# yahoo/bftkv

Measured on AMD Instinct MI355X. Metric: pgp_rsa2048_signature_verifies_per_sec, higher is better.
Workload: dtype u32; 1 GPU; 64-replica quorum, 10000 RSA-2048 signed writes per GPU (cfg2 of BASELINE.json), 534164 signature packets per GPU, 1.0% corrupt / 0.5% unknown issuer / 0.5% duplicate / 1.0% one-short; parallelism=shard-by-write x1, RCCL all-gather of verdict bitmaps on the verifier's stream, replicas=64, writes_per_gpu=10000, sigs_per_gpu=534164, batches_in_flight=3

## Files before the change

### bftkv_amd/csrc/capi.hip

```cpp
#include "../../include/bftkv_gpu.h"

#include <hip/hip_runtime.h>
#include <stdio.h>
#include <stdlib.h>
#include <string.h>

#include <limits.h>
#include <linux/futex.h>
#include <sched.h>
#include <sys/syscall.h>
#include <unistd.h>

#include <algorithm>
#include <array>
#include <atomic>
#include <memory>
#include <functional>
#include <map>
#include <set>
#include <chrono>
#include <condition_variable>
#include <mutex>
#include <shared_mutex>
#include <system_error>
#include <thread>
#include <string>
#include <unordered_map>
#include <vector>

#include "host_bignum.h"
#include "host_sha256.h"
#include "kernels.hip"
#include "threshold_kernels.hip"
#include "ec_kernels.hip"
#include "dsa_verify_kernels.hip"

using namespace bftkv;

namespace {

inline void copy_out(void* dst, const void* src, size_t n) { if (n) memcpy(dst, src, n); }

struct DevBuf {
  void* p = nullptr;
  size_t cap = 0;
  hipError_t ensure(size_t bytes) {
    if (bytes <= cap) return hipSuccess;
    if (p) { hipError_t e = hipFree(p); if (e != hipSuccess) return e; p = nullptr; cap = 0; }
    size_t want = bytes + bytes / 4 + 256;
    hipError_t e = hipMalloc(&p, want);
    if (e == hipSuccess) cap = want;
    return e;
  }
  hipError_t ensure_exact(size_t bytes) {
    if (bytes <= cap) return hipSuccess;
    if (p) { hipError_t e = hipFree(p); if (e != hipSuccess) return e; p = nullptr; cap = 0; }
    hipError_t e = hipMalloc(&p, bytes);
    if (e == hipSuccess) cap = bytes;
    return e;
  }
  void release() { if (p) (void)hipFree(p); p = nullptr; cap = 0; }
  template <typename T> T* as() const { return (T*)p; }
};

struct KeyEntry {
  uint64_t key_id = 0, entity_id = 0;
  uint8_t algo = 0, flags = 0;
  uint32_t bits = 0, e = 0, n0 = 0, qbits = 0;
  std::vector<uint32_t> nl, r2, r2w, qw, dtab, qpow, qconst;
  std::string material;
  bool cert_only = false;
  int cert_group = -1;
  uint32_t entity_index = 0;
  std::string cert_digest;
  uint64_t last_used = 0;
  bool dsa_unslotted = false;
};

struct QuorumHost {
  bool live = false;
  int n_qcs = 0;
  int32_t f[MAX_QC], mn[MAX_QC], thr[MAX_QC], suff[MAX_QC];
  std::vector<std::vector<uint64_t>> nodes;
  DevBuf member;
  uint64_t keyring_gen = ~0ull;
  DevBuf ids;
  uint32_t ids_off[MAX_QC + 1];
};

struct EcKeySet {
  bool live = false;
  int curve_id = -1;
  uint32_t bits = 0, n_keys = 0, n_refused = 0;
  uint32_t w = 0, nwin = 0;
  size_t key_words = 0;
  std::vector<uint8_t> curve;
  DevBuf tab;
  DevBuf refused;
  DevBuf mod[4];
  void release() { tab.release(); refused.release(); for (DevBuf& b : mod) b.release(); }
};

}

using ctx_lock = std::lock_guard<std::recursive_mutex>;

struct bftkv_gpu_ctx {
  int device = 0;
  hipStream_t stream = nullptr;
  hipStream_t stream_h = nullptr;
  hipStream_t stream_d = nullptr;
  std::recursive_mutex mu;
  std::string err;

  uint64_t keyring_gen = 0;
  uint32_t n_keys = 0, n_entities = 0;
  bool have_dsa_keys = false, have_rsa3072 = false, have_rsa4096 = false, have_ambiguous = false;
  std::vector<uint64_t> h_key_id, h_entity_id;
  std::vector<uint32_t> h_key_entity;
  std::vector<uint8_t> h_key_flags;
  std::vector<KeyEntry> ring, certs;
  uint32_t n_ring_entities = 0;
  std::map<std::string, bool> cert_valid;
  DevBuf k_r2w;
  DevBuf k_id, k_entity, k_algo, k_flags, k_bits, k_e, k_n, k_r2, k_n0, k_q, k_qbits, k_dsatab, k_dsaslot, k_sorted_id, k_sorted_slot;
  DevBuf dsa_comb;
  uint32_t dsa_wbits = 8, dsa_wbits_pinned = 0;
  std::map<std::string, uint32_t> dsa_comb_slot;
  std::set<std::string> dsa_cert_materials;
  uint64_t ring_epoch = 0, dsa_ring_epoch_seen = ~0ull;
  uint32_t dsa_wbits_want = 0;
  uint32_t dsa_entry_limbs = DSA_N_SMALL;
  size_t dsa_budget_bytes = 0;
  bool have_dsa3072 = false, have_dsa2048 = false;
  DevBuf dsa_idx;
  uint64_t cert_clock = 0;
  struct CertFast { uint64_t issuer_id; int group; uint64_t epoch; };
  std::shared_mutex cert_fast_mu;
  std::unordered_map<std::string, CertFast> cert_fast;
  size_t cert_fast_bytes = 0;
  uint64_t cert_epoch = 0, kt_cert_epoch = 0;
  std::vector<uint32_t> kt_group_ent;
  KeyTableDev kt{};

  std::vector<QuorumHost> quorums;
  std::vector<EcKeySet> ec_keysets;

  DevBuf txt_mid32, txt_mid64, txt_tail, txt_len;
  DevBuf forced_iss;
  DevBuf counts, base, total, item_flags, walk_scratch, cert_ent, sig_class, mid, mid64, hash_mask, recs, digests, r, xr, pk_list, pk_list3072, pk_list4096, r3072, r4096, pk_count, dsa_list, dsa_u, ids_tmp;
  DevBuf o_err, o_nver, o_verdict, o_fenced;
  DevBuf in_tbs, in_tbs_off, in_ss, in_ss_off;
  hipEvent_t seg_ev = nullptr;
  DevBuf in_prefix, in_prefix_off, in_shared, in_shared_off, in_seg;
  DevBuf st_tmp, item_tmp, bits_tmp, plan_cut;
  DevBuf chunk_arena, chunk_ctr;
  uint32_t multiexp_parts = 0;
  uint32_t ec_split = 0;
  uint32_t ec_window = 0;
  DevBuf ec_fb_tab[4];
  uint32_t ec_fb_w[4] = {};
  uint32_t multiexp_block = 0;
  uint32_t multiexp_lanes = 0;
  uint32_t dsa_inv_mode = 0;
  uint32_t n_cus = 256;
  uint32_t lagrange_x_bound = 0;
  bool early_exit = true;
  std::vector<DevBuf*> scratch_pool;
  std::unordered_map<std::string, std::vector<uint32_t>> modrow_cache;
  std::map<std::string, std::array<DevBuf, 4>> modtab_cache;
  uint32_t* h_mail = nullptr;
  uint32_t* d_mail = nullptr;
  uint32_t last_total = 0, last_rsa = 0, last_items = 0;
  bool last_total_on_dev = false;
  hipEvent_t ev[10] = {};
  hipEvent_t ev_turn = nullptr;
  bool have_timing = false;
  void* rccl_comm = nullptr;
  int n_ranks = 1, rank = 0;

  bftkv_gpu_ctx* root = nullptr;
  std::shared_mutex kt_rw;
  std::atomic<int> kt_writers{0};
  std::atomic<int> n_forks{0};
  uint64_t quorum_gen = 0;
  uint64_t seen_keyring_gen = ~0ull, seen_quorum_gen = ~0ull;
  size_t n_dsa_slots = 0;
  int kt_read_depth = 0;
  DevBuf in_pack;
  uint8_t* h_out = nullptr; uint8_t* d_out = nullptr; size_t out_cap = 0;
  uint32_t out_seq = 0;
  std::vector<bftkv_gpu_ctx*> hb_workers;
  hipStream_t stream_c = nullptr;
  hipStream_t stream_c2 = nullptr;
  std::vector<hipEvent_t> hb_ev;
  uint8_t* hb_out = nullptr; size_t hb_out_cap = 0;
  uint32_t modexp_lds_pad = 0;
  uint32_t hb_pieces = 0;
  hipEvent_t hb_ev0 = nullptr;
  bool hb_tight = false;
  uint32_t hb_copy_mode = 0;
  void* hb_ring = nullptr;
  std::vector<float> hb_trace;
  uint32_t hb_last_pieces = 0;
  std::vector<uint32_t> hb_item0;
  void* small_pin = nullptr;
  uint32_t staged_spin_us = 50000;
};

void rccl_release(bftkv_gpu_ctx* c);
void release_small_pin(bftkv_gpu_ctx* c);
extern "C" int signature_verify_entities(bftkv_gpu_ctx* c, uint32_t n_items, const uint8_t* tbs, const uint64_t* tbs_off, const uint8_t* sig,
                                         const uint64_t* sig_off, const uint32_t* ent, uint8_t* err_out, const uint8_t* sig_class = nullptr,
                                         uint8_t* fenced_out = nullptr, const uint64_t* forced_issuer = nullptr);

namespace {

int fork_refresh(bftkv_gpu_ctx* c);

struct KtWrite {
  bftkv_gpu_ctx* c;
  explicit KtWrite(bftkv_gpu_ctx* c_) : c(c_) { c->kt_writers.fetch_add(1); c->kt_rw.lock(); }
  ~KtWrite() { c->kt_rw.unlock(); c->kt_writers.fetch_sub(1); }
};
struct KtRead {
  bftkv_gpu_ctx *c, *r;
  int rc = 0;
  explicit KtRead(bftkv_gpu_ctx* c_) : c(c_), r(c_->root) {
    if (!r || c->kt_read_depth++ > 0) return;
    while (r->kt_writers.load(std::memory_order_acquire) > 0) std::this_thread::yield();
    r->kt_rw.lock_shared();
    rc = fork_refresh(c);
  }
  ~KtRead() { if (r && --c->kt_read_depth == 0) r->kt_rw.unlock_shared(); }
};

struct Turnstile { std::mutex mu; hipEvent_t last = nullptr; const void* owner = nullptr; };
Turnstile g_turnstile[16];
constexpr uint64_t HB_PIPE_MIN_BYTES = 24ull << 20;
constexpr uint32_t HB_PIPE_MAX_PIECES = 8;
std::mutex g_hb_mu[16];
constexpr size_t HB_TR = 10;
struct HbRing {
  static constexpr size_t SLOT = 16u << 20;
  static constexpr int NSLOT = 6;
  static constexpr int THREADS = 4;
  uint8_t* base = nullptr;
  hipEvent_t ev[NSLOT] = {};
  bool used[NSLOT] = {};
  ~HbRing() { if (base) (void)hipHostFree(base); for (auto e : ev) if (e) (void)hipEventDestroy(e); }
  hipError_t init() {
    if (base) return hipSuccess;
    hipError_t e = hipHostMalloc((void**)&base, SLOT * NSLOT, hipHostMallocDefault);
    if (e != hipSuccess) { base = nullptr; return e; }
    for (auto& x : ev) if ((e = hipEventCreateWithFlags(&x, hipEventDisableTiming)) != hipSuccess) return e;
    return hipSuccess;
  }
};


constexpr uint32_t TURNSTILE_MIN_PACKETS = 98304;

std::mutex g_live_mu;
std::vector<bftkv_gpu_ctx*> g_live;
bool ctx_is_live(bftkv_gpu_ctx* c) {
  std::lock_guard<std::mutex> lk(g_live_mu);
  for (auto* p : g_live) if (p == c) return true;
  return false;
}

int fail(bftkv_gpu_ctx* c, int rc, const char* what, hipError_t e = hipSuccess) {
  char buf[512];
  if (e != hipSuccess) snprintf(buf, sizeof buf, "%s: %s", what, hipGetErrorString(e));
  else snprintf(buf, sizeof buf, "%s", what);
  c->err = buf;
  return rc;
}
// ... 96 lines not shown
                 const std::function<int(hipStream_t)>* upload_tbs = nullptr, const QuorumDev* plan_q = nullptr, uint64_t ss_len = 0,
                 const uint32_t* d_mid_in = nullptr, const uint64_t* d_tbs_prefix = nullptr, uint32_t staged_cap = 0,
                 hipEvent_t ev_input = nullptr, bool mid_prelaunched = false, const uint64_t* d_forced_issuer = nullptr) {
  const bool one_stream = staged_cap != 0 && !ev_input;
  hipStream_t s = c->stream, sh = one_stream ? c->stream : c->stream_h;
  auto rec = [&](int k, hipStream_t st) -> hipError_t { return one_stream ? hipSuccess : hipEventRecord(c->ev[k], st); };
  auto join = [&](hipStream_t st, int k) -> hipError_t { return one_stream ? hipSuccess : hipStreamWaitEvent(st, c->ev[k], 0); };
  if (!c->ev[0]) for (auto& e : c->ev) HIPCHK(c, hipEventCreate(&e));
  HIPCHK(c, c->counts.ensure(sizeof(uint32_t) * (n_items + 1)));
  HIPCHK(c, c->base.ensure(sizeof(uint32_t) * (n_items + 1)));
  HIPCHK(c, c->total.ensure(16));
  HIPCHK(c, c->item_flags.ensure(n_items + 16));
  const uint32_t walk_cap = ss_len ? (uint32_t)std::min<uint64_t>(WALK_CAP_MAX, std::max<uint64_t>(WALK_CAP_MIN, ss_len / n_items / 48)) : 96u;
  HIPCHK(c, c->walk_scratch.ensure(sizeof(WalkEnt) * walk_cap * (size_t)n_items + 16));
  HIPCHK(c, c->mid.ensure(sizeof(uint32_t) * 8 * N_MID32 * (size_t)n_items + 16));
  HIPCHK(c, c->mid64.ensure(sizeof(uint64_t) * 8 * 2 * (size_t)n_items + 16));
  HIPCHK(c, c->hash_mask.ensure(sizeof(uint32_t) * (size_t)n_items + 16));
  constexpr size_t CHUNK_ARENA_MIN = 64u << 10;
  if (!c->chunk_ctr.p) { HIPCHK(c, c->chunk_ctr.ensure(16)); HIPCHK(c, hipMemsetAsync(c->chunk_ctr.p, 0, 16, c->stream)); }
  HIPCHK(c, c->chunk_arena.ensure(CHUNK_ARENA_MIN + (staged_cap ? 2 * (size_t)ss_len : 0)));
  HIPCHK(c, c->pk_count.ensure(96));
  if (plan_q) HIPCHK(c, c->plan_cut.ensure(sizeof(uint32_t) * (size_t)n_items + 16));
  TextDev txt{nullptr, nullptr, nullptr, nullptr};
  if (!d_mid_in) {
    HIPCHK(c, c->txt_mid32.ensure(sizeof(uint32_t) * 8 * N_MID32 * (size_t)n_items + 16));
    HIPCHK(c, c->txt_mid64.ensure(sizeof(uint64_t) * 8 * N_MID64 * (size_t)n_items + 16));
    HIPCHK(c, c->txt_tail.ensure((size_t)128 * N_HASHES * n_items + 16));
    HIPCHK(c, c->txt_len.ensure(sizeof(uint64_t) * N_HASHES * (size_t)n_items + 16));
    txt = TextDev{c->txt_mid32.as<uint32_t>(), c->txt_mid64.as<uint64_t>(), c->txt_tail.as<uint8_t>(), c->txt_len.as<uint64_t>()};
  }
  if (ev_input) HIPCHK(c, hipStreamWaitEvent(s, ev_input, 0));
  HIPCHK(c, rec(0, s));
  HIPCHK(c, join(sh, 0));
  HIPCHK(c, rec(5, sh));
  if (!upload_tbs && !d_mid_in)
    hipLaunchKernelGGL(k_sha256_mid, dim3((n_items + 63) / 64), dim3(64), 0, sh, d_tbs, d_tbs_off, n_items, c->mid.as<uint32_t>());
  hipLaunchKernelGGL(k_walk<false>, dim3(n_items), dim3(64), 0, s, d_ss, d_ss_off, n_items, c->counts.as<uint32_t>(),
                     (const uint32_t*)nullptr, (SigRec*)nullptr, c->item_flags.as<uint8_t>(), c->walk_scratch.as<WalkEnt>(), walk_cap,
                     c->chunk_ctr.as<uint32_t>());
  constexpr uint32_t MAIL_EMPTY = 0xFFFFFFFFu;
  if (c->h_mail && !staged_cap) __atomic_store_n(&c->h_mail[0], MAIL_EMPTY, __ATOMIC_RELEASE);
  hipLaunchKernelGGL(k_scan_counts, dim3(1), dim3(1024), 0, s, c->counts.as<uint32_t>(), n_items, c->base.as<uint32_t>(),
                     c->total.as<uint32_t>(), staged_cap ? (uint32_t*)nullptr : c->d_mail, c->pk_count.as<uint32_t>(), c->hash_mask.as<uint32_t>(),
                     staged_cap, c->chunk_ctr.as<uint32_t>());
  uint32_t total = staged_cap ? staged_cap : MAIL_EMPTY;
  const uint32_t* const n_recs_dev = staged_cap ? c->total.as<uint32_t>() : nullptr;
  if (c->h_mail && !staged_cap) {
    const auto t_spin = std::chrono::steady_clock::now();
    for (uint32_t it = 0;; ++it) {
      total = __atomic_load_n(&c->h_mail[0], __ATOMIC_ACQUIRE);
      if (total != MAIL_EMPTY) break;
      if ((it & 1023u) == 1023u && std::chrono::steady_clock::now() - t_spin > std::chrono::milliseconds(20)) break;
      __builtin_ia32_pause();
    }
  }
  uint32_t chunk_units = (c->h_mail && !staged_cap && total != MAIL_EMPTY) ? c->h_mail[2] : 0u;
  if (total == MAIL_EMPTY) {
    HIPCHK(c, hipMemcpyAsync(&total, c->total.p, sizeof(uint32_t), hipMemcpyDeviceToHost, s));
    HIPCHK(c, hipMemcpyAsync(&chunk_units, c->chunk_ctr.as<uint32_t>() + 2, sizeof(uint32_t), hipMemcpyDeviceToHost, s));
    HIPCHK(c, hipStreamSynchronize(s));
  }
  if (!staged_cap && (size_t)chunk_units * 16 > c->chunk_arena.cap) HIPCHK(c, c->chunk_arena.ensure((size_t)chunk_units * 16));
  c->last_total = staged_cap ? 0u : total;
  c->last_total_on_dev = staged_cap != 0 && ev_input != nullptr;
  c->last_items = n_items;
  c->hb_last_pieces = 0;
  const size_t tr = total ? total : 1;
  HIPCHK(c, c->recs.ensure(sizeof(SigRec) * tr));
  HIPCHK(c, c->digests.ensure(sizeof(uint32_t) * 16 * tr));
  HIPCHK(c, c->r.ensure(sizeof(uint32_t) * EM_LOW_LIMBS * tr));
  HIPCHK(c, c->xr.ensure(sizeof(uint32_t) * (c->have_rsa4096 ? MONT_NMAX : c->have_rsa3072 ? MONT_TPI_BIG * MONT_L3072 : 80) * tr));
  HIPCHK(c, c->pk_list.ensure(sizeof(uint32_t) * tr));
  HIPCHK(c, c->pk_list3072.ensure(c->have_rsa3072 ? sizeof(uint32_t) * tr : 16));
  HIPCHK(c, c->pk_list4096.ensure(c->have_rsa4096 ? sizeof(uint32_t) * tr : 16));
  if (c->have_rsa3072) HIPCHK(c, c->r3072.ensure(sizeof(uint32_t) * EM_LOW_LIMBS * tr));
  if (c->have_rsa4096) HIPCHK(c, c->r4096.ensure(sizeof(uint32_t) * EM_LOW_LIMBS * tr));
  HIPCHK(c, c->dsa_list.ensure(sizeof(uint32_t) * tr));
  if (c->have_dsa_keys) HIPCHK(c, c->dsa_u.ensure(sizeof(uint32_t) * DSA_U_WORDS * tr));
  if (c->have_dsa3072 && c->have_dsa2048) HIPCHK(c, c->dsa_idx.ensure(sizeof(uint32_t) * 4 * (size_t)tr + 16));
  hipLaunchKernelGGL(k_walk<true>, dim3(n_items), dim3(64), 0, s, d_ss, d_ss_off, n_items, c->counts.as<uint32_t>(),
                     c->base.as<uint32_t>(), c->recs.as<SigRec>(), c->item_flags.as<uint8_t>(), (WalkEnt*)nullptr, walk_cap, (uint32_t*)nullptr);
  if (total) {
    ParseArgs pa;
    pa.sig_blob = d_ss; pa.sig_off = d_ss_off; pa.rec_base = c->base.as<uint32_t>(); pa.counts = c->counts.as<uint32_t>(); pa.n_items = n_items;
    pa.scratch = c->walk_scratch.as<WalkEnt>(); pa.walk_cap = walk_cap; pa.recs = c->recs.as<SigRec>(); pa.n_recs = total; pa.cert_ent = d_cert_ent;
    pa.pk_list = c->pk_list.as<uint32_t>(); pa.pk_list3072 = c->pk_list3072.as<uint32_t>(); pa.pk_list4096 = c->pk_list4096.as<uint32_t>();
    pa.pk_count = c->pk_count.as<uint32_t>(); pa.dsa_list = c->dsa_list.as<uint32_t>(); pa.item_hash_mask = c->hash_mask.as<uint32_t>();
    pa.sig_class = d_sig_class; pa.forced_issuer = d_forced_issuer; pa.msg_slot = d_msg_slot; pa.msg_hash = d_msg_hash; pa.item_flags = c->item_flags.as<uint8_t>();
    pa.defer_queue = plan_q ? 1u : 0u;
    pa.n_recs_dev = n_recs_dev;
    pa.chunk_arena = c->chunk_arena.as<uint8_t>(); pa.chunk_cap_units = (uint32_t)std::min<size_t>(c->chunk_arena.cap / 16, 0xFFFFFFF0u);
    pa.chunk_bump = c->chunk_ctr.as<uint32_t>() + 1;
    if (!staged_cap && (uint64_t)total >= 128ull * n_items)
      hipLaunchKernelGGL(k_parse_body_items, dim3(n_items), dim3(PARSE_ITEM_BLOCK), 0, s, pa, c->kt);
    else
      hipLaunchKernelGGL(k_parse_body, dim3((total + 255) / 256), dim3(256), 0, s, pa, c->kt);
  }
  uint32_t* const cnt_p = c->pk_count.as<uint32_t>();
  const uint32_t* const start0 = cnt_p + 12;
  PlanArgs pl{};
  if (total && plan_q) {
    pl.recs = c->recs.as<SigRec>(); pl.rec_base = c->base.as<uint32_t>(); pl.counts = c->counts.as<uint32_t>(); pl.n_items = n_items;
    pl.pk_list = c->pk_list.as<uint32_t>(); pl.dsa_list = c->dsa_list.as<uint32_t>(); pl.pk_list3072 = c->pk_list3072.as<uint32_t>();
    pl.pk_list4096 = c->pk_list4096.as<uint32_t>(); pl.pk_count = cnt_p; pl.plan_cut = c->plan_cut.as<uint32_t>(); pl.verdict = nullptr;
    int min_suff = 0;
    for (int i = 0; i < plan_q->n_qcs; ++i) if (plan_q->suff[i] > 0 && (min_suff == 0 || plan_q->suff[i] < min_suff)) min_suff = plan_q->suff[i];
    pl.margin = 1u + (uint32_t)min_suff / 64u;
    pl.mail = c->d_mail ? c->d_mail + 3 : nullptr;
    if (c->h_mail) __atomic_store_n(&c->h_mail[3], 0u, __ATOMIC_RELEASE);
    hipLaunchKernelGGL(k_plan<1>, dim3((n_items + PLAN_ITEMS - 1) / PLAN_ITEMS), dim3(PLAN_BLOCK), 0, s, pl, c->kt, *plan_q);
  }
  const bool dsa_side = total && c->have_dsa_keys;
  if (one_stream && dsa_side) HIPCHK(c, hipEventRecord(c->ev[1], s)); else HIPCHK(c, rec(1, s));
  const size_t n_slots = c->root ? c->n_dsa_slots : c->dsa_comb_slot.size();
  const uint32_t inv_batch_min = c->dsa_inv_mode == 1 || n_slots > (c->dsa_inv_mode == 2 ? (size_t)INV_MAX_SLOTS : 256) ? 0xFFFFFFFFu
                                 : c->dsa_inv_mode == 2 ? 0u : (uint32_t)std::max<size_t>(4096, 64 * n_slots);
  auto launch_dsa_inv = [&](hipStream_t st, const uint32_t* start) {
    if (inv_batch_min != 0xFFFFFFFFu)
      hipLaunchKernelGGL(k_dsa_inv_batched, dim3((total + INV_TILE - 1) / INV_TILE), dim3(INV_BLOCK), 0, st, d_ss, c->recs.as<SigRec>(),
                         c->dsa_list.as<uint32_t>(), c->pk_count.as<uint32_t>(), start, c->kt, c->dsa_u.as<uint32_t>(), inv_batch_min);
    if (inv_batch_min != 0u)
      hipLaunchKernelGGL(k_dsa_inv, dim3((total + 63) / 64), dim3(64), 0, st, d_ss, c->recs.as<SigRec>(), c->dsa_list.as<uint32_t>(),
                         c->pk_count.as<uint32_t>(), start, c->kt, c->dsa_u.as<uint32_t>(), inv_batch_min);
  };
  if (total && c->have_dsa_keys) {
    HIPCHK(c, hipStreamWaitEvent(c->stream_d, c->ev[1], 0));
    launch_dsa_inv(c->stream_d, start0);
    HIPCHK(c, hipEventRecord(c->ev[7], c->stream_d));
  }
  auto hash_stream_work = [&]() -> int {
    HIPCHK(c, join(sh, 1));
    if (total) {
      if (!d_mid_in) {
        hipLaunchKernelGGL(k_hash_mid_other, dim3((n_items + 63) / 64, N_HASHES - 1), dim3(64), 0, sh, d_tbs, d_tbs_off, n_items,
                           c->hash_mask.as<uint32_t>(), c->mid.as<uint32_t>(), c->mid64.as<uint64_t>());
        hipLaunchKernelGGL(k_hash_mid_text, dim3((n_items + 63) / 64, N_HASHES), dim3(64), 0, sh, d_tbs, d_tbs_off, n_items, c->hash_mask.as<uint32_t>(), txt);
      }
      hipLaunchKernelGGL(k_digest_sha256, dim3((total + 255) / 256), dim3(256), 0, sh, d_tbs, d_tbs_off, d_ss,
                         d_mid_in ? d_mid_in : c->mid.as<uint32_t>(), c->mid64.as<uint64_t>(), n_items, c->recs.as<SigRec>(), total,
                         c->digests.as<uint32_t>(), d_tbs_prefix, n_recs_dev);
    }
    HIPCHK(c, rec(6, sh));
    return 0;
  };
  if (!upload_tbs) { int hrc = hash_stream_work(); if (hrc) return hrc; }
  const dim3 qg((total + MODEXP_BLOCK / MONT_TPI - 1) / (MODEXP_BLOCK / MONT_TPI));
  const dim3 qg8((total + MODEXP_BLOCK / MONT_TPI_BIG - 1) / (MODEXP_BLOCK / MONT_TPI_BIG));
  static const bool wide8_off = getenv("BFTKV_NO_WIDE8") != nullptr;
  const bool wide8 = staged_cap != 0 && ss_len / 256 <= 8192 && !wide8_off;
  auto launch_modexp = [&](const uint32_t* start) {
    if (wide8)
      hipLaunchKernelGGL((k_rsa_modexp<10, MONT_TPI_BIG>), qg8, dim3(MODEXP_BLOCK), 0, s, d_ss, c->recs.as<SigRec>(), c->pk_list.as<uint32_t>(),
                         cnt_p, start, c->kt, c->r.as<uint32_t>(), c->xr.as<uint32_t>(), (uint64_t*)(cnt_p + 16));
    else
    hipLaunchKernelGGL((k_rsa_modexp<MONT_L, MONT_TPI>), qg, dim3(MODEXP_BLOCK), c->modexp_lds_pad, s, d_ss, c->recs.as<SigRec>(), c->pk_list.as<uint32_t>(),
                       cnt_p, start, c->kt, c->r.as<uint32_t>(), c->xr.as<uint32_t>(), (uint64_t*)(cnt_p + 16));
    if (c->have_rsa3072)
      hipLaunchKernelGGL((k_rsa_modexp<MONT_L3072, MONT_TPI_BIG>), qg8, dim3(MODEXP_BLOCK), 0, s, d_ss, c->recs.as<SigRec>(), c->pk_list3072.as<uint32_t>(),
                         cnt_p + 2, start + 2, c->kt, c->r3072.as<uint32_t>(), c->xr.as<uint32_t>(), (uint64_t*)nullptr);
    if (c->have_rsa4096)
      hipLaunchKernelGGL((k_rsa_modexp<MONT_L4096, MONT_TPI_BIG>), qg8, dim3(MODEXP_BLOCK), 0, s, d_ss, c->recs.as<SigRec>(), c->pk_list4096.as<uint32_t>(),
                         cnt_p + 3, start + 3, c->kt, c->r4096.as<uint32_t>(), c->xr.as<uint32_t>(), (uint64_t*)nullptr);
  };
  static const bool turnstile_off = getenv("BFTKV_NO_TURNSTILE") != nullptr;
  const bool big = staged_cap ? (ev_input != nullptr && ss_len / 320 >= TURNSTILE_MIN_PACKETS) : total >= TURNSTILE_MIN_PACKETS;
  if (big && !turnstile_off) {
    Turnstile& g = g_turnstile[(unsigned)c->device & 15u];
    std::lock_guard<std::mutex> tl(g.mu);
    if (g.last && g.owner != c) HIPCHK(c, hipStreamWaitEvent(s, g.last, 0));
    HIPCHK(c, rec(9, s));
    launch_modexp(start0);
    if (!c->ev_turn) HIPCHK(c, hipEventCreateWithFlags(&c->ev_turn, hipEventDisableTiming));
    HIPCHK(c, hipEventRecord(c->ev_turn, s));
    g.last = c->ev_turn; g.owner = c;
  } else {
    HIPCHK(c, rec(9, s));
    if (total) launch_modexp(start0);
  }
  HIPCHK(c, rec(2, s));
  if (upload_tbs) {
    int hrc = (*upload_tbs)(sh);
    if (hrc) return hrc;
    if (!mid_prelaunched)
      hipLaunchKernelGGL(k_sha256_mid, dim3((n_items + 63) / 64), dim3(64), 0, sh, d_tbs, d_tbs_off, n_items, c->mid.as<uint32_t>());
    if ((hrc = hash_stream_work())) return hrc;
  }
  HIPCHK(c, join(s, 6));
  bool other_hashes = true;
  if (total && !d_mid_in && plan_q && big && c->h_mail) {
    const auto t_spin = std::chrono::steady_clock::now();
    for (uint32_t it = 0;; ++it) {
      const uint32_t v = __atomic_load_n(&c->h_mail[3], __ATOMIC_ACQUIRE);
      if (v) { other_hashes = (v & 1u) != 0; break; }
      if ((it & 255u) == 255u && std::chrono::steady_clock::now() - t_spin > std::chrono::microseconds(300) + std::chrono::nanoseconds((uint64_t)total / 2)) break;
      __builtin_ia32_pause();
    }
  }
  if (total && !d_mid_in && other_hashes)
    hipLaunchKernelGGL(k_digest_other, dim3(std::min<uint32_t>((total + 255) / 256, DIGEST_OTHER_MAX_BLOCKS)), dim3(256), 0, s,
                       d_tbs, d_tbs_off, d_ss, c->mid.as<uint32_t>(), c->mid64.as<uint64_t>(), n_items, c->recs.as<SigRec>(), total,
                       c->digests.as<uint32_t>(), c->pk_count.as<uint32_t>() + 4, txt, n_recs_dev);
  const dim3 cg(((uint64_t)total * CMP_LANES + 255) / 256);
  auto launch_compare = [&](const uint32_t* start) {
    hipLaunchKernelGGL(k_rsa_compare, cg, dim3(256), 0, s, c->recs.as<SigRec>(), c->pk_list.as<uint32_t>(),
                       cnt_p, start, c->kt, c->r.as<uint32_t>(), c->digests.as<uint32_t>());
    if (c->have_rsa3072)
      hipLaunchKernelGGL(k_rsa_compare, cg, dim3(256), 0, s, c->recs.as<SigRec>(), c->pk_list3072.as<uint32_t>(),
                         cnt_p + 2, start + 2, c->kt, c->r3072.as<uint32_t>(), c->digests.as<uint32_t>());
    if (c->have_rsa4096)
      hipLaunchKernelGGL(k_rsa_compare, cg, dim3(256), 0, s, c->recs.as<SigRec>(), c->pk_list4096.as<uint32_t>(),
                         cnt_p + 3, start + 3, c->kt, c->r4096.as<uint32_t>(), c->digests.as<uint32_t>());
  };
  auto launch_dsa = [&](const uint32_t* start) {
    hipLaunchKernelGGL(k_dsa_mul, dim3((total + 63) / 64), dim3(64), 0, s, c->recs.as<SigRec>(), c->dsa_list.as<uint32_t>(),
                       cnt_p, start, c->kt, c->digests.as<uint32_t>(), c->dsa_u.as<uint32_t>());
    const uint32_t* idx_s = nullptr; const uint32_t* idx_b = nullptr; const uint32_t* cnt_cls = nullptr;
    if (c->have_dsa3072 && c->have_dsa2048) {
      uint32_t* cc = cnt_p + (start == start0 ? 20 : 22);
      uint32_t* is = c->dsa_idx.as<uint32_t>() + (start == start0 ? 0 : 2 * (size_t)total);
      hipLaunchKernelGGL(k_dsa_split, dim3((total + 255) / 256), dim3(256), 0, s, c->recs.as<SigRec>(), c->dsa_list.as<uint32_t>(), cnt_p, start, c->kt,
                         is, is + total, cc);
      idx_s = is; idx_b = is + total; cnt_cls = cc;
    }
    if (c->have_dsa2048)
      hipLaunchKernelGGL((k_dsa_modexp<MONT_L, MONT_TPI>), dim3((total + QUADS_PER_BLOCK - 1) / QUADS_PER_BLOCK), dim3(RSA_BLOCK), 0, s,
                         c->recs.as<SigRec>(), c->dsa_list.as<uint32_t>(), cnt_p, start, c->kt, c->dsa_u.as<uint32_t>(), idx_s, cnt_cls);
    if (c->have_dsa3072)
      hipLaunchKernelGGL((k_dsa_modexp<MONT_L3072, MONT_TPI_BIG>), dim3((total + RSA_BLOCK / MONT_TPI_BIG - 1) / (RSA_BLOCK / MONT_TPI_BIG)), dim3(RSA_BLOCK), 0, s,
                         c->recs.as<SigRec>(), c->dsa_list.as<uint32_t>(), cnt_p, start, c->kt, c->dsa_u.as<uint32_t>(), idx_b, cnt_cls ? cnt_cls + 1 : nullptr);
  };
  if (total) launch_compare(start0);
  HIPCHK(c, rec(8, s));
  if (total && c->have_dsa_keys) {
    HIPCHK(c, hipStreamWaitEvent(s, c->ev[7], 0));
    launch_dsa(start0);
  }
  if (total && plan_q) {
    HIPCHK(c, c->o_nver.ensure(sizeof(uint32_t) * n_items));
    HIPCHK(c, c->o_verdict.ensure(n_items));
    hipLaunchKernelGGL(k_tally, dim3((n_items + 3) / 4), dim3(256), 0, s, c->recs.as<SigRec>(), c->base.as<uint32_t>(), c->counts.as<uint32_t>(),
                       n_items, c->kt, *plan_q, c->o_verdict.as<uint8_t>(), c->o_nver.as<uint32_t>(), (uint32_t*)nullptr);
    hipLaunchKernelGGL(k_plan_snapshot, dim3(1), dim3(64), 0, s, cnt_p);
    pl.verdict = c->o_verdict.as<uint8_t>();
    hipLaunchKernelGGL(k_plan<2>, dim3((n_items + PLAN_ITEMS - 1) / PLAN_ITEMS), dim3(PLAN_BLOCK), 0, s, pl, c->kt, *plan_q);
    const uint32_t* const start1 = cnt_p + 8;
    if (c->have_dsa_keys) launch_dsa_inv(s, start1);
    launch_modexp(start1);
    launch_compare(start1);
    if (c->have_dsa_keys) launch_dsa(start1);
  }
  if (total && c->have_ambiguous && !d_msg_slot)
    hipLaunchKernelGGL(k_candidates, dim3((total + 63) / 64), dim3(64), 0, s, d_tbs, d_tbs_off, d_ss, d_mid_in ? d_mid_in : c->mid.as<uint32_t>(),
                       c->mid64.as<uint64_t>(), n_items, c->recs.as<SigRec>(), total, n_recs_dev, d_tbs_prefix, c->kt, d_cert_ent, d_sig_class, txt,
                       c->hash_mask.as<uint32_t>());
  HIPCHK(c, rec(3, s));
  HIPCHK(c, hipGetLastError());
  return 0;
}

int make_key_entry(bftkv_gpu_ctx* c, const bftkv_gpu_pubkey& k, bool cert_only, KeyEntry* out) {
  KeyEntry& e = *out;
  e.key_id = k.key_id; e.entity_id = k.entity_id; e.algo = k.pk_algo; e.cert_only = cert_only;
  e.material.clear();
  e.material.push_back((char)k.pk_algo);
  e.material.push_back((char)k.usable_sign);
  auto app = [&](const uint8_t* p, uint32_t l) {
    uint32_t z = 0;
    while (z < l && p[z] == 0) ++z;
    if (l > z) e.material.append((const char*)p + z, l - z);
    e.material.push_back('|');
  };
  app(k.n, k.n_len); app(k.e, k.e_len); app(k.g, k.g_len); app(k.y, k.y_len);
  e.flags = 0;
  if (k.usable_sign) e.flags |= KEYF_USABLE_SIGN;
  if (k.pk_algo != PK_RSA_ENCRYPT_ONLY && k.pk_algo != PK_ELGAMAL) e.flags |= KEYF_CAN_SIGN;
  if (k.key_id == k.entity_id) e.flags |= KEYF_PRIMARY;
  if (cert_only) e.flags |= KEYF_CERT_ONLY;
  e.bits = (uint32_t)hostbn::bit_length(k.n, k.n_len);
  e.e = 0; e.n0 = 0; e.qbits = 0;
  e.r2w.clear();
  e.nl.assign(MONT_NMAX, 0); e.r2.assign(MONT_NMAX, 0); e.qw.assign(8, 0); e.dtab.assign(2 * DSA_N_BIG, 0); e.qpow.clear(); e.qconst.clear();
  if (k.pk_algo == PK_RSA || k.pk_algo == PK_RSA_SIGN_ONLY) {
    if (hostbn::bit_length(k.e, k.e_len) > 32) return fail(c, BFTKV_E_UNSUPPORTED, "RSA public exponent wider than 32 bits");
    for (uint32_t j = 0; j < k.e_len; ++j) e.e = (e.e << 8) | k.e[j];
    const int nlimbs = e.bits <= 2048 ? MONT_N : (e.bits <= 3072 ? MONT_TPI_BIG * MONT_L3072 : MONT_TPI_BIG * MONT_L4096);
    if (e.bits > 4096) e.bits = 0xFFFFFFFFu;
    else if (!hostbn::mont_setup(k.n, k.n_len, nlimbs, e.nl.data(), e.r2.data(), &e.n0)) e.bits = 0xFFFFFFFFu;
    else if (e.bits <= 2048) {
      std::vector<uint32_t> nl80(80);
      uint32_t n0b = 0;
      e.r2w.assign(80, 0);
      (void)hostbn::mont_setup(k.n, k.n_len, 80, nl80.data(), e.r2w.data(), &n0b);
    }
  } else if (k.pk_algo == PK_DSA) {
    e.qbits = (uint32_t)hostbn::bit_length(k.e, k.e_len);
    const int NLp = e.bits <= 2048 ? (int)DSA_N_SMALL : (int)DSA_N_BIG;
    const uint32_t cap_bits = e.bits <= 2048 ? 2048u : 3072u;
    const int nwords = (28 * NLp + 31) / 32 + 1;
    std::vector<uint32_t> p(nwords), g(nwords), y(nwords), q(nwords);
    hostbn::from_be(k.e, k.e_len, q.data(), nwords);
    bool ok = e.bits >= 2 && e.bits <= 3072 && e.qbits >= 32 && e.qbits <= 256 && (q[0] & 1u) &&
              hostbn::mont_setup(k.n, k.n_len, NLp, e.nl.data(), e.r2.data(), &e.n0);
    if (ok && (hostbn::bit_length(k.g, k.g_len) > cap_bits || hostbn::bit_length(k.y, k.y_len) > cap_bits)) ok = false;
    if (ok) {
      hostbn::from_be(k.n, k.n_len, p.data(), nwords);
      hostbn::from_be(k.g, k.g_len, g.data(), nwords);
      hostbn::from_be(k.y, k.y_len, y.data(), nwords);
      hostbn::reduce(g.data(), p.data(), nwords);
      hostbn::reduce(y.data(), p.data(), nwords);
      hostbn::to_mont_limbs(g.data(), p.data(), nwords, NLp, &e.dtab[0]);
      hostbn::to_mont_limbs(y.data(), p.data(), nwords, NLp, &e.dtab[DSA_N_BIG]);
      for (int j = 0; j < 8; ++j) e.qw[j] = q[j];
      e.qpow.assign((size_t)NLp * 10, 0);
      uint32_t x[9] = {1, 0, 0, 0, 0, 0, 0, 0, 0}, q9[9];
      for (int j = 0; j < 9; ++j) q9[j] = j < 8 ? q[j] : 0;
      for (int j = 0; j < NLp; ++j) {
        hostbn::to_limbs28(x, 9, &e.qpow[(size_t)j * 10], 10);
        for (int b = 0; b < MONT_W; ++b) hostbn::dbl_mod(x, q9, 9);
      }
      e.qconst.assign(12, 0);
      uint32_t r2q[9] = {1, 0, 0, 0, 0, 0, 0, 0, 0};
      for (int b = 0; b < 512; ++b) hostbn::dbl_mod(r2q, q9, 9);
      for (int j = 0; j < 8; ++j) e.qconst[j] = r2q[j];
      uint32_t inv = 1;
      for (int it = 0; it < 5; ++it) inv *= 2u - q[0] * inv;
      e.qconst[8] = 0u - inv;
    } else {
      e.bits = 0xFFFFFFFFu;
    }
  }
  return 0;
}

int sync_dsa_tables(bftkv_gpu_ctx* c, const std::vector<const KeyEntry*>& rows, const std::vector<uint8_t>& algo,
                    std::vector<uint32_t>& bits, bool* bits_changed) {
  std::vector<uint32_t> slot(rows.size() ? rows.size() : 1, 0xFFFFFFFFu);
  *bits_changed = false;
  auto stride_bytes = [&](uint32_t w, uint32_t E) -> size_t { return (size_t)dsa_slot_stride(w, E) * sizeof(uint32_t); };
  size_t ring_dsa = 0;
  bool ring_big = false;
  for (size_t i = 0; i < rows.size(); ++i)
    if (algo[i] == PK_DSA && bits[i] != 0xFFFFFFFFu && !rows[i]->cert_only) { ++ring_dsa; ring_big = ring_big || bits[i] > 2048; }
  auto assign = [&](std::vector<uint32_t>& new_slots, std::vector<uint32_t>& new_rows) {
    new_slots.clear(); new_rows.clear();
    size_t cert_cap = c->dsa_wbits > 8 ? 8 : 1024;
    if (c->dsa_budget_bytes) {
      const size_t per = stride_bytes(c->dsa_wbits, c->dsa_entry_limbs), ring_need = per * ring_dsa;
      cert_cap = std::min(cert_cap, c->dsa_budget_bytes > ring_need ? (c->dsa_budget_bytes - ring_need) / per : 0);
    }
    for (size_t i = 0; i < rows.size(); ++i) {
      if (algo[i] != PK_DSA || bits[i] == 0xFFFFFFFFu) continue;
      if (bits[i] > 2048 && c->dsa_entry_limbs != DSA_N_BIG) {
        bits[i] = 0xFFFFFFFFu; *bits_changed = true;
        const_cast<KeyEntry*>(rows[i])->dsa_unslotted = true;
        continue;
      }
      auto it = c->dsa_comb_slot.find(rows[i]->material);
      if (it == c->dsa_comb_slot.end()) {
        uint32_t id = (uint32_t)c->dsa_comb_slot.size();
        if (rows[i]->cert_only && c->dsa_cert_materials.size() >= cert_cap) {
          std::string victim;
          if (rows[i]->last_used == c->cert_clock) {
            for (const std::string& m : c->dsa_cert_materials) {
              bool in_use = false;
              for (size_t j = 0; j < rows.size() && !in_use; ++j)
                in_use = algo[j] == PK_DSA && rows[j]->material == m && (!rows[j]->cert_only || rows[j]->last_used == c->cert_clock);
              if (!in_use) { victim = m; break; }
            }
          }
          if (victim.empty()) {
            bits[i] = 0xFFFFFFFFu; *bits_changed = true;
            const_cast<KeyEntry*>(rows[i])->dsa_unslotted = true;
            continue;
          }
          for (size_t j = 0; j < rows.size(); ++j)
            if (algo[j] == PK_DSA && rows[j]->material == victim) {
              bits[j] = 0xFFFFFFFFu; slot[j] = 0xFFFFFFFFu; *bits_changed = true;
              const_cast<KeyEntry*>(rows[j])->dsa_unslotted = true;
            }
          id = c->dsa_comb_slot[victim];
          c->dsa_comb_slot.erase(victim);
          c->dsa_cert_materials.erase(victim);
        }
        it = c->dsa_comb_slot.emplace(rows[i]->material, id).first;
        if (rows[i]->cert_only) c->dsa_cert_materials.insert(rows[i]->material);
        const_cast<KeyEntry*>(rows[i])->dsa_unslotted = false;
        new_slots.push_back(it->second); new_rows.push_back((uint32_t)i);
      } else if (!rows[i]->cert_only) c->dsa_cert_materials.erase(rows[i]->material);
      slot[i] = it->second;
    }
  };
  auto policy = [&](size_t n_keys, uint32_t E) -> uint32_t {
    if (c->dsa_wbits_pinned) return c->dsa_wbits_pinned;
    if (const char* e = getenv("BFTKV_DSA_WBITS")) {
      const uint32_t b = (uint32_t)atoi(e);
      if (b == 4 || (b >= 8 && b <= 20)) return b;
    }
    if (n_keys > 4096) return 4u;
    static const uint32_t widths[] = {18, 16, 15, 14, 13, 12, 10};
    if (c->dsa_budget_bytes) {
      for (uint32_t w : widths)
        if (std::max<size_t>(n_keys, 1) * stride_bytes(w, E) <= c->dsa_budget_bytes) return w;
      return std::max<size_t>(n_keys, 1) * stride_bytes(8, E) <= c->dsa_budget_bytes ? 8u : 4u;
    }
    size_t free_b = 0, total_b = 0;
    if (hipMemGetInfo(&free_b, &total_b) == hipSuccess) {
      const size_t room = free_b + c->dsa_comb.cap;
      for (uint32_t w : widths) {
        const size_t need = (n_keys + 1) * stride_bytes(w, E) * 3 / 2;
        if (need < (w == 18 ? room / 100 * 45 : room / 4)) return w;
      }
    }
    return 8u;
  };
  uint32_t want_E = c->dsa_entry_limbs;
  if (c->dsa_ring_epoch_seen != c->ring_epoch || c->dsa_wbits_want == 0) {
    want_E = ring_big ? DSA_N_BIG : DSA_N_SMALL;
    c->dsa_wbits_want = policy(ring_dsa, want_E);
    c->dsa_ring_epoch_seen = c->ring_epoch;
  }
  const uint32_t want_wbits = c->dsa_wbits_pinned ? c->dsa_wbits_pinned : c->dsa_wbits_want;
  std::vector<uint32_t> new_slots, new_rows;
  bool restart = false;
  if (want_wbits != c->dsa_wbits || want_E != c->dsa_entry_limbs) {
    restart = true;
    c->dsa_comb_slot.clear();
    c->dsa_cert_materials.clear();
    c->dsa_wbits = want_wbits;
    c->dsa_entry_limbs = want_E;
  }
  assign(new_slots, new_rows);
  const size_t live = [&] { size_t n = 0; for (uint32_t v : slot) n += v != 0xFFFFFFFFu; return n; }();
  bool crowded = false;
  if (!restart && c->dsa_comb_slot.size() > live) {
    const size_t held = c->dsa_comb_slot.size() * stride_bytes(c->dsa_wbits, c->dsa_entry_limbs);
    size_t free_b = 0, total_b = 0;
    if (c->dsa_budget_bytes) crowded = held > c->dsa_budget_bytes;
    else if (c->dsa_wbits >= 12 && hipMemGetInfo(&free_b, &total_b) == hipSuccess) crowded = held * 3 / 2 > (free_b + c->dsa_comb.cap) / 100 * 45;
  }
  if (!restart && (c->dsa_comb_slot.size() > 2 * live + 256 || crowded)) {
    restart = true;
    c->dsa_comb_slot.clear();
    c->dsa_cert_materials.clear();
    for (size_t i = 0; i < rows.size(); ++i) slot[i] = 0xFFFFFFFFu;
    assign(new_slots, new_rows);
  }
  if (getenv("BFTKV_DEBUG_DSA")) {
    size_t n_cert_rows = 0, n_dsa = 0, n_fenced = 0;
    for (size_t i = 0; i < rows.size(); ++i) { n_cert_rows += rows[i]->cert_only; n_dsa += algo[i] == PK_DSA; n_fenced += algo[i] == PK_DSA && bits[i] == 0xFFFFFFFFu; }
    fprintf(stderr, "[dsa tables] rows %zu (cert %zu, dsa %zu, dsa without slot %zu) width %u want %u entry limbs %u slots %zu cert-slots %zu new %zu restart %d clock %llu budget %zu\n", rows.size(),
            n_cert_rows, n_dsa, n_fenced, c->dsa_wbits, want_wbits, c->dsa_entry_limbs, c->dsa_comb_slot.size(), c->dsa_cert_materials.size(), new_slots.size(), (int)restart,
            (unsigned long long)c->cert_clock, c->dsa_budget_bytes);
  }
  int rc;
  if ((rc = upload(c, c->k_dsaslot, slot))) return rc;
  c->kt.dsa_slot = c->k_dsaslot.as<uint32_t>();
  c->kt.dsa_wbits = c->dsa_wbits;
  c->kt.dsa_entry_limbs = c->dsa_entry_limbs;
  if (new_slots.empty()) return 0;
  const uint32_t E = c->dsa_entry_limbs;
  const size_t per_key = stride_bytes(c->dsa_wbits, E);
  const size_t need = per_key * c->dsa_comb_slot.size();
  if (restart && (c->dsa_comb.cap > 2 * need + (64u << 20) || (c->dsa_budget_bytes && c->dsa_comb.cap > c->dsa_budget_bytes))) c->dsa_comb.release();
  if (need > c->dsa_comb.cap) {
    DevBuf bigger;
    size_t want = need + (c->dsa_wbits > 18 ? std::min(need / 2, 2 * per_key) : need / 2);
    if (c->dsa_budget_bytes) want = std::max(need, std::min(want, c->dsa_budget_bytes));
    if (restart) c->dsa_comb.release();
    HIPCHK(c, bigger.ensure_exact(want));
    const size_t keep = restart ? 0 : std::min(need, (c->dsa_comb.cap / per_key) * per_key);
    if (keep && c->dsa_comb.p) HIPCHK(c, hipMemcpyAsync(bigger.p, c->dsa_comb.p, keep, hipMemcpyDeviceToDevice, c->stream));
    HIPCHK(c, hipStreamSynchronize(c->stream));
    c->dsa_comb.release();
    c->dsa_comb = bigger;
  }
  c->kt.dsa_comb = c->dsa_comb.as<uint32_t>();
  for (size_t k = 0; k < new_slots.size(); ++k) {
    char* tail = (char*)c->dsa_comb.p + per_key * new_slots[k] + dsa_comb_limbs_per_key(c->dsa_wbits, E) * sizeof(uint32_t);
    const KeyEntry* ke = rows[new_rows[k]];
    HIPCHK(c, hipMemcpyAsync(tail, ke->qpow.data(), ke->qpow.size() * sizeof(uint32_t), hipMemcpyHostToDevice, c->stream));
    HIPCHK(c, hipMemcpyAsync(tail + dsa_qpow_words(E) * sizeof(uint32_t), ke->qconst.data(), ke->qconst.size() * sizeof(uint32_t), hipMemcpyHostToDevice, c->stream));
  }
  hipError_t e = hipSuccess;
  for (int big = 0; big < 2 && e == hipSuccess; ++big) {
    std::vector<uint32_t> cs, cr;
    for (size_t k = 0; k < new_slots.size(); ++k)
      if ((bits[new_rows[k]] > 2048) == (big == 1)) { cs.push_back(new_slots[k]); cr.push_back(new_rows[k]); }
    if (cs.empty()) continue;
    DevBuf d_slots, d_rows;
    if ((rc = upload(c, d_slots, cs)) || (rc = upload(c, d_rows, cr))) { d_slots.release(); d_rows.release(); return rc; }
    const uint32_t parts = c->dsa_wbits > 12 ? 1u << (c->dsa_wbits - 12u) : 1u;
    const uint32_t n_groups = (uint32_t)cs.size() * 2u * dsa_nwin(c->dsa_wbits) * parts;
    if (big)
      hipLaunchKernelGGL((k_dsa_build_comb<MONT_L3072, MONT_TPI_BIG>), dim3((n_groups + RSA_BLOCK / MONT_TPI_BIG - 1) / (RSA_BLOCK / MONT_TPI_BIG)), dim3(RSA_BLOCK), 0, c->stream,
                         (uint32_t)cs.size(), d_slots.as<uint32_t>(), d_rows.as<uint32_t>(), c->kt, c->dsa_comb.as<uint32_t>(), parts);
    else
      hipLaunchKernelGGL((k_dsa_build_comb<MONT_L, MONT_TPI>), dim3((n_groups + QUADS_PER_BLOCK - 1) / QUADS_PER_BLOCK), dim3(RSA_BLOCK), 0, c->stream,
                         (uint32_t)cs.size(), d_slots.as<uint32_t>(), d_rows.as<uint32_t>(), c->kt, c->dsa_comb.as<uint32_t>(), parts);
    e = hipStreamSynchronize(c->stream);
    d_slots.release(); d_rows.release();
  }
  if (e != hipSuccess) return fail(c, BFTKV_E_DEVICE, "k_dsa_build_comb", e);
  return 0;
}

int upload_key_table(bftkv_gpu_ctx* c) {
  if (c->root) return fail(c, BFTKV_E_STATE, "a forked context cannot change the key table (use its root)");
  KtWrite kw(c);
  std::vector<uint64_t> key_id, entity_ids;
  std::vector<uint32_t> entity, bits, e32, nl, r2, r2w, n0, qw, qbits, dtab;
  std::vector<uint8_t> algo, flags;
  std::vector<const KeyEntry*> rows;
  auto add = [&](const KeyEntry& e, bool own_entity) {
    uint32_t ent = 0;
    if (own_entity) { ent = (uint32_t)entity_ids.size(); entity_ids.push_back(e.entity_id); }
    else {
      for (; ent < entity_ids.size(); ++ent) if (entity_ids[ent] == e.entity_id) break;
      if (ent == entity_ids.size()) entity_ids.push_back(e.entity_id);
    }
    key_id.push_back(e.key_id); entity.push_back(ent); algo.push_back(e.algo); flags.push_back(e.flags);
    bits.push_back(e.bits); e32.push_back(e.e); n0.push_back(e.n0); qbits.push_back(e.qbits);
    nl.insert(nl.end(), e.nl.begin(), e.nl.end()); r2.insert(r2.end(), e.r2.begin(), e.r2.end());
    r2w.insert(r2w.end(), e.r2w.begin(), e.r2w.end()); r2w.resize(key_id.size() * 80, 0);
    qw.insert(qw.end(), e.qw.begin(), e.qw.end()); dtab.insert(dtab.end(), e.dtab.begin(), e.dtab.end());
    rows.push_back(&e);
    return ent;
  };
  for (auto& e : c->ring) add(e, false);
  c->n_ring_entities = (uint32_t)entity_ids.size();
  int last_group = -1;
  uint32_t group_ent = 0;
  std::vector<uint32_t> group_ents;
  for (auto& e : c->certs) {
    if (e.cert_group != last_group) { group_ent = add(e, true); last_group = e.cert_group; }
    else {
      key_id.push_back(e.key_id); entity.push_back(group_ent); algo.push_back(e.algo); flags.push_back(e.flags);
      bits.push_back(e.bits); e32.push_back(e.e); n0.push_back(e.n0); qbits.push_back(e.qbits);
      nl.insert(nl.end(), e.nl.begin(), e.nl.end()); r2.insert(r2.end(), e.r2.begin(), e.r2.end());
      r2w.insert(r2w.end(), e.r2w.begin(), e.r2w.end()); r2w.resize(key_id.size() * 80, 0);
      qw.insert(qw.end(), e.qw.begin(), e.qw.end()); dtab.insert(dtab.end(), e.dtab.begin(), e.dtab.end());
      rows.push_back(&e);
    }
    const_cast<KeyEntry&>(e).entity_index = group_ent;
    if (e.cert_group >= 0) {
      if (group_ents.size() <= (size_t)e.cert_group) group_ents.resize((size_t)e.cert_group + 1, 0xFFFFFFFEu);
      group_ents[(size_t)e.cert_group] = group_ent;
    }
  }
  std::vector<uint32_t> sorted_slot(key_id.size());
  for (size_t i = 0; i < sorted_slot.size(); ++i) sorted_slot[i] = (uint32_t)i;
  std::stable_sort(sorted_slot.begin(), sorted_slot.end(), [&](uint32_t a, uint32_t b) { return key_id[a] < key_id[b]; });
  std::vector<uint64_t> sorted_id(key_id.size());
  for (size_t i = 0; i < sorted_slot.size(); ++i) sorted_id[i] = key_id[sorted_slot[i]];
  int rc;
  if ((rc = upload(c, c->k_sorted_id, sorted_id)) || (rc = upload(c, c->k_sorted_slot, sorted_slot))) return rc;
  if ((rc = upload(c, c->k_id, key_id)) || (rc = upload(c, c->k_entity, entity)) || (rc = upload(c, c->k_algo, algo)) ||
      (rc = upload(c, c->k_flags, flags)) || (rc = upload(c, c->k_bits, bits)) || (rc = upload(c, c->k_e, e32)) ||
      (rc = upload(c, c->k_n, nl)) || (rc = upload(c, c->k_r2, r2)) || (rc = upload(c, c->k_n0, n0)) ||
      (rc = upload(c, c->k_q, qw)) || (rc = upload(c, c->k_qbits, qbits)) || (rc = upload(c, c->k_dsatab, dtab)) || (rc = upload(c, c->k_r2w, r2w)))
    return rc;
  c->kt.r2_limbs80 = c->k_r2w.as<uint32_t>();
  c->n_keys = (uint32_t)key_id.size();
  c->kt.n_keys = c->n_keys;
  c->kt.n_limbs = c->k_n.as<uint32_t>();
  c->kt.r2_limbs = c->k_r2.as<uint32_t>();
  c->kt.n0inv = c->k_n0.as<uint32_t>();
  c->kt.dsa_tab = c->k_dsatab.as<uint32_t>();
  bool bits_changed = false;
  if ((rc = sync_dsa_tables(c, rows, algo, bits, &bits_changed))) return rc;
  if (bits_changed && (rc = upload(c, c->k_bits, bits))) return rc;
  HIPCHK(c, hipStreamSynchronize(c->stream));
  c->have_dsa_keys = c->have_dsa3072 = c->have_dsa2048 = c->have_rsa3072 = c->have_rsa4096 = c->have_ambiguous = false;
  for (size_t i = 0; i < algo.size(); ++i) {
    if (flags[i] & KEYF_AMBIGUOUS) c->have_ambiguous = true;
    if (algo[i] == PK_DSA) c->have_dsa_keys = true;
    if (algo[i] == PK_DSA && bits[i] != 0xFFFFFFFFu && bits[i] > 2048) c->have_dsa3072 = true;
    if (algo[i] == PK_DSA && (bits[i] == 0xFFFFFFFFu || bits[i] <= 2048)) c->have_dsa2048 = true;
    if ((algo[i] == PK_RSA || algo[i] == PK_RSA_SIGN_ONLY) && bits[i] != 0xFFFFFFFFu) {
      if (bits[i] > 3072) c->have_rsa4096 = true; else if (bits[i] > 2048) c->have_rsa3072 = true;
    }
  }
  c->n_entities = (uint32_t)entity_ids.size();
  c->h_key_id = key_id;
  c->h_entity_id = entity_ids;
  c->h_key_entity = entity;
  c->h_key_flags = flags;
  c->kt.n_keys = c->n_keys;
  c->kt.key_id = c->k_id.as<uint64_t>();
  c->kt.sorted_id = c->k_sorted_id.as<uint64_t>();
  c->kt.sorted_slot = c->k_sorted_slot.as<uint32_t>();
  c->kt.entity = c->k_entity.as<uint32_t>();
  c->kt.pk_algo = c->k_algo.as<uint8_t>();
  c->kt.flags = c->k_flags.as<uint8_t>();
  c->kt.mod_bits = c->k_bits.as<uint32_t>();
  c->kt.rsa_e = c->k_e.as<uint32_t>();
  c->kt.n_limbs = c->k_n.as<uint32_t>();
  c->kt.r2_limbs = c->k_r2.as<uint32_t>();
  c->kt.n0inv = c->k_n0.as<uint32_t>();
  c->kt.q_words = c->k_q.as<uint32_t>();
  c->kt.q_bits = c->k_qbits.as<uint32_t>();
  c->kt.dsa_tab = c->k_dsatab.as<uint32_t>();
  c->kt.dsa_slot = c->k_dsaslot.as<uint32_t>();
  c->kt.dsa_comb = c->dsa_comb.as<uint32_t>();
  c->kt.dsa_wbits = c->dsa_wbits;
  c->kt.dsa_entry_limbs = c->dsa_entry_limbs;
  c->kt_group_ent = std::move(group_ents);
  c->kt_cert_epoch = c->cert_epoch;
  ++c->keyring_gen;
  return 0;
}

int fork_refresh(bftkv_gpu_ctx* c) {
  bftkv_gpu_ctx* r = c->root;
  if (c->seen_keyring_gen != r->keyring_gen) {
    c->kt = r->kt;
    c->n_keys = r->n_keys; c->n_entities = r->n_entities; c->n_ring_entities = r->n_ring_entities;
    c->have_dsa_keys = r->have_dsa_keys; c->have_dsa3072 = r->have_dsa3072; c->have_dsa2048 = r->have_dsa2048; c->have_rsa3072 = r->have_rsa3072; c->have_rsa4096 = r->have_rsa4096; c->have_ambiguous = r->have_ambiguous;
    c->h_key_id = r->h_key_id; c->h_entity_id = r->h_entity_id; c->h_key_entity = r->h_key_entity; c->h_key_flags = r->h_key_flags;
    c->n_dsa_slots = r->dsa_comb_slot.size(); c->dsa_wbits = r->dsa_wbits; c->dsa_entry_limbs = r->dsa_entry_limbs;
    c->keyring_gen = r->keyring_gen;
    c->seen_keyring_gen = r->keyring_gen;
  }
  c->early_exit = r->early_exit;
  if (c->seen_quorum_gen != r->quorum_gen) {
    for (auto& q : c->quorums) { q.member.release(); q.ids.release(); }
    c->quorums.clear();
    c->quorums.resize(r->quorums.size());
    for (size_t i = 0; i < r->quorums.size(); ++i) {
      const QuorumHost& s = r->quorums[i];
      QuorumHost& d = c->quorums[i];
      d.live = s.live; d.n_qcs = s.n_qcs; d.nodes = s.nodes;
      for (int k = 0; k < MAX_QC; ++k) { d.f[k] = s.f[k]; d.mn[k] = s.mn[k]; d.thr[k] = s.thr[k]; d.suff[k] = s.suff[k]; }
      d.keyring_gen = ~0ull;
    }
    c->seen_quorum_gen = r->quorum_gen;
  }
  return 0;
}

int check_offsets(bftkv_gpu_ctx* c, const uint64_t* off, uint32_t n, const char* what) {
  if (off[0] != 0) return fail(c, BFTKV_E_INVALID, what);
  for (uint32_t i = 0; i < n; ++i) if (off[i + 1] < off[i]) return fail(c, BFTKV_E_INVALID, what);
  return 0;
}

int check_quorum(bftkv_gpu_ctx* c, int quorum) {
  if (quorum < 0 || (size_t)quorum >= c->quorums.size() || !c->quorums[quorum].live) return fail(c, BFTKV_E_INVALID, "bad quorum handle");
  return 0;
}

}

extern "C" {

int bftkv_gpu_init(int device_ordinal, bftkv_gpu_ctx** out) {
  if (!out) return BFTKV_E_INVALID;
  int n = 0;
  if (hipGetDeviceCount(&n) != hipSuccess || n <= 0) return BFTKV_E_DEVICE;
  if (device_ordinal < 0 || device_ordinal >= n) return BFTKV_E_INVALID;
  if (hipSetDevice(device_ordinal) != hipSuccess) return BFTKV_E_DEVICE;
  bftkv_gpu_ctx* c = new bftkv_gpu_ctx();
  c->device = device_ordinal;
  if (hipHostMalloc((void**)&c->h_mail, 64, hipHostMallocMapped) == hipSuccess) {
    if (hipHostGetDevicePointer((void**)&c->d_mail, c->h_mail, 0) != hipSuccess) { (void)hipHostFree(c->h_mail); c->h_mail = nullptr; c->d_mail = nullptr; }
    else memset(c->h_mail, 0, 64);
  } else c->h_mail = nullptr;
  if (hipStreamCreateWithFlags(&c->stream, hipStreamNonBlocking) != hipSuccess ||
      hipStreamCreateWithFlags(&c->stream_h, hipStreamNonBlocking) != hipSuccess ||
      hipStreamCreateWithFlags(&c->stream_d, hipStreamNonBlocking) != hipSuccess) { delete c; return BFTKV_E_DEVICE; }
  { std::lock_guard<std::mutex> lk(g_live_mu); g_live.push_back(c); }
  if (const char* e = getenv("BFTKV_STAGED_SPIN_US")) c->staged_spin_us = (uint32_t)atoi(e);
  if (const char* e = getenv("BFTKV_MODEXP_LDS_PAD")) c->modexp_lds_pad = (uint32_t)atoi(e);
  if (const char* e = getenv("BFTKV_MULTIEXP_PARTS")) c->multiexp_parts = (uint32_t)atoi(e);
  if (const char* e = getenv("BFTKV_EC_SPLIT")) c->ec_split = (uint32_t)atoi(e);
  if (const char* e = getenv("BFTKV_EC_WINDOW")) c->ec_window = (uint32_t)atoi(e);
  if (const char* e = getenv("BFTKV_MULTIEXP_LANES")) c->multiexp_lanes = (uint32_t)atoi(e);
  if (const char* e = getenv("BFTKV_MULTIEXP_BLOCK")) c->multiexp_block = (uint32_t)atoi(e);
  if (const char* e = getenv("BFTKV_DSA_INV")) c->dsa_inv_mode = !strcmp(e, "batched") ? 2u : !strcmp(e, "single") ? 1u : 0u;
  { int cus = 0; if (hipDeviceGetAttribute(&cus, hipDeviceAttributeMultiprocessorCount, device_ordinal) == hipSuccess && cus > 0) c->n_cus = (uint32_t)cus; }
  *out = c;
  return BFTKV_OK;
}

int bftkv_gpu_ctx_fork(bftkv_gpu_ctx* root, bftkv_gpu_ctx** out) {
  if (!root || !out) return BFTKV_E_INVALID;
  if (root->root) return fail(root, BFTKV_E_INVALID, "fork of a fork");
  bftkv_gpu_ctx* c = nullptr;
  int rc = bftkv_gpu_init(root->device, &c);
  if (rc) return rc;
  c->root = root;
  c->early_exit = root->early_exit;
  c->dsa_inv_mode = root->dsa_inv_mode;
  root->n_forks.fetch_add(1);
  *out = c;
  return 0;
}

void bftkv_gpu_destroy(bftkv_gpu_ctx* c) {
  if (!c) return;
  for (bftkv_gpu_ctx* w : c->hb_workers) bftkv_gpu_destroy(w);
  c->hb_workers.clear();
  if (!c->root && c->n_forks.load() > 0) {
    fprintf(stderr, "bftkv_gpu_destroy: context still has %d forked context(s); not destroyed\n", c->n_forks.load());
    return;
  }
  {
    std::lock_guard<std::mutex> lk(g_live_mu);
    for (size_t i = 0; i < g_live.size(); ++i) if (g_live[i] == c) { g_live.erase(g_live.begin() + i); break; }
  }
  (void)hipSetDevice(c->device);
  (void)hipStreamSynchronize(c->stream);
  (void)hipStreamSynchronize(c->stream_h);
  (void)hipStreamSynchronize(c->stream_d);
  for (DevBuf* b : {&c->k_id, &c->k_entity, &c->k_algo, &c->k_flags, &c->k_bits, &c->k_e, &c->k_n, &c->k_r2, &c->k_n0, &c->k_q, &c->k_qbits, &c->k_dsatab, &c->k_dsaslot, &c->dsa_comb, &c->k_sorted_id, &c->k_sorted_slot, &c->k_r2w,
                    &c->chunk_arena, &c->chunk_ctr, &c->counts, &c->base, &c->total, &c->item_flags, &c->walk_scratch, &c->cert_ent, &c->sig_class, &c->mid, &c->mid64, &c->hash_mask, &c->recs, &c->digests, &c->r, &c->xr,
                    &c->pk_list, &c->pk_list3072, &c->pk_list4096, &c->r3072, &c->r4096, &c->pk_count, &c->dsa_list, &c->dsa_u, &c->dsa_idx, &c->ids_tmp, &c->o_err, &c->o_nver, &c->o_verdict, &c->o_fenced, &c->in_tbs, &c->in_tbs_off,
                    &c->in_ss, &c->in_ss_off, &c->in_prefix, &c->in_prefix_off, &c->in_shared, &c->in_shared_off, &c->in_seg, &c->st_tmp, &c->item_tmp, &c->bits_tmp, &c->plan_cut, &c->txt_mid32, &c->txt_mid64, &c->txt_tail, &c->txt_len})
    b->release();
  for (auto& q : c->quorums) { q.member.release(); q.ids.release(); }
  for (EcKeySet& ks : c->ec_keysets) ks.release();
  c->in_pack.release();
  c->forced_iss.release();
  release_small_pin(c);
  if (c->h_out) (void)hipHostFree(c->h_out);
  if (c->root) c->root->n_forks.fetch_sub(1);
  for (DevBuf* b : c->scratch_pool) { b->release(); delete b; }
  for (auto& kv : c->modtab_cache) for (DevBuf& b : kv.second) b.release();
  for (DevBuf& b : c->ec_fb_tab) b.release();
  if (c->h_mail) (void)hipHostFree(c->h_mail);
  if (c->hb_out) (void)hipHostFree(c->hb_out);
  if (c->hb_ring) { if (c->stream_c) (void)hipStreamSynchronize(c->stream_c); delete (HbRing*)c->hb_ring; }
  for (hipEvent_t e : c->hb_ev) (void)hipEventDestroy(e);
  if (c->hb_ev0) (void)hipEventDestroy(c->hb_ev0);
  if (c->seg_ev) (void)hipEventDestroy(c->seg_ev);
  if (c->stream_c) { (void)hipStreamSynchronize(c->stream_c); (void)hipStreamDestroy(c->stream_c); }
  if (c->stream_c2) { (void)hipStreamSynchronize(c->stream_c2); (void)hipStreamDestroy(c->stream_c2); }
  rccl_release(c);
  for (auto& e : c->ev) if (e) (void)hipEventDestroy(e);
  if (c->ev_turn) {
    Turnstile& g = g_turnstile[(unsigned)c->device & 15u];
    std::lock_guard<std::mutex> tl(g.mu);
    if (g.owner == c) { g.last = nullptr; g.owner = nullptr; }
    (void)hipEventDestroy(c->ev_turn);
  }
  (void)hipStreamDestroy(c->stream);
  (void)hipStreamDestroy(c->stream_h);
  (void)hipStreamDestroy(c->stream_d);
  delete c;
}

const char* bftkv_gpu_last_error(const bftkv_gpu_ctx* c) { return c ? c->err.c_str() : "null context"; }

const char* bftkv_gpu_error_string(int e) {
  switch (e) {
    case BFTKV_ERR_NONE: return "";
    case BFTKV_ERR_INVALID_SIGNATURE: return "crypto: invalid signature";
    case BFTKV_ERR_INSUFFICIENT_SIGNATURES: return "crypto: insufficient number of signatures";
    default: return "unknown";
  }
}

void* bftkv_gpu_stream(bftkv_gpu_ctx* c) { return c ? (void*)c->stream : nullptr; }

int bftkv_gpu_sync(bftkv_gpu_ctx* c) {
  if (!c) return BFTKV_E_INVALID;
  HIPCHK(c, hipStreamSynchronize(c->stream));
  return 0;
}

int bftkv_gpu_set_host_pipeline(bftkv_gpu_ctx* c, uint32_t pieces) {
  const uint32_t mode = (pieces >> 8) & 3u, tight = (pieces >> 10) & 1u;
  if (!c || (pieces & 0xFFu) > HB_PIPE_MAX_PIECES || mode > 2 || (pieces >> 11)) return BFTKV_E_INVALID;
  pieces &= 0xFFu;
  ctx_lock lk(c->mu);
  c->hb_pieces = pieces;
  c->hb_copy_mode = mode;
  c->hb_tight = tight != 0;
  return 0;
}

int bftkv_gpu_host_pipeline_trace(bftkv_gpu_ctx* c, float* out, uint32_t cap, uint32_t* n_out) {
  if (!c || !n_out) return BFTKV_E_INVALID;
  ctx_lock lk(c->mu);
  *n_out = (uint32_t)c->hb_trace.size();
  if (out) copy_out(out, c->hb_trace.data(), sizeof(float) * std::min<size_t>(cap, c->hb_trace.size()));
  return 0;
}

int bftkv_gpu_set_early_exit(bftkv_gpu_ctx* c, int on) {
  if (!c) return BFTKV_E_INVALID;
  ctx_lock lk(c->mu);
  if (c->root) return fail(c, BFTKV_E_STATE, "set on the root context; its forks follow");
  KtWrite kw(c);
  c->early_exit = on != 0;
  return 0;
}

int bftkv_gpu_set_hash_policy(bftkv_gpu_ctx* c, int hash_id, int state) {
  if (!c || (hash_id != HASH_MD5 && hash_id != HASH_RIPEMD160) || state < 0 || state > 2) return BFTKV_E_INVALID;
  ctx_lock lk(c->mu);
  if (c->root) return fail(c, BFTKV_E_STATE, "set on the root context; its forks follow");
  KtWrite kw(c);
  const int sh = hash_id == HASH_MD5 ? 0 : 2;
  c->kt.hash_policy = (c->kt.hash_policy & ~(3u << sh)) | ((uint32_t)state << sh);
  ++c->keyring_gen;
  return 0;
}

static bool dsa_width_ok(uint32_t bits) { return bits == 4 || (bits >= 8 && bits <= 20); }

int bftkv_gpu_set_dsa_window_bits(bftkv_gpu_ctx* c, uint32_t bits) {
  if (!c || (bits != 0 && !dsa_width_ok(bits))) return BFTKV_E_INVALID;
  ctx_lock lk(c->mu);
  c->dsa_wbits_pinned = bits;
  return 0;
}

int bftkv_gpu_set_dsa_table_budget(bftkv_gpu_ctx* c, uint64_t bytes) {
  if (!c) return BFTKV_E_INVALID;
  ctx_lock lk(c->mu);
  if (c->root) return fail(c, BFTKV_E_STATE, "a forked context cannot change the key table (use its root)");
  c->dsa_budget_bytes = (size_t)bytes;
  c->dsa_wbits_want = 0;
  return 0;
}

int bftkv_gpu_dsa_table_bytes(bftkv_gpu_ctx* c, uint64_t* bytes_out, uint32_t* entry_limbs_out) {
  if (!c) return BFTKV_E_INVALID;
  ctx_lock lk(c->mu);
  const bftkv_gpu_ctx* r = c->root ? c->root : c;
  if (bytes_out) *bytes_out = (uint64_t)r->dsa_comb.cap;
  if (entry_limbs_out) *entry_limbs_out = r->dsa_entry_limbs;
  return 0;
}

int bftkv_gpu_dsa_window_bits(bftkv_gpu_ctx* c, uint32_t* bits_out) {
  if (!c || !bits_out) return BFTKV_E_INVALID;
  ctx_lock lk(c->mu);
  const bftkv_gpu_ctx* r = c->root ? c->root : c;
  *bits_out = r->dsa_comb_slot.empty() ? 0u : r->dsa_wbits;
  return 0;
}

int bftkv_gpu_keyring_set(bftkv_gpu_ctx* c, const bftkv_gpu_pubkey* keys, uint32_t n_keys) {
  if (!c || (!keys && n_keys)) return BFTKV_E_INVALID;
  ctx_lock lk(c->mu);
  if (c->root) return fail(c, BFTKV_E_STATE, "a forked context cannot change the key table (use its root)");
  HIPCHK(c, hipSetDevice(c->device));
  std::vector<KeyEntry> ring;
  for (uint32_t i = 0; i < n_keys; ++i) {
    KeyEntry e;
    int rc = make_key_entry(c, keys[i], false, &e);
    if (rc) return rc;
    bool dup = false;
    for (auto& o : ring) {
      if (o.key_id == e.key_id) {
        if (o.material == e.material) { dup = true; break; }
        o.flags |= KEYF_AMBIGUOUS; e.flags |= KEYF_AMBIGUOUS;
      }
    }
    if (!dup) ring.push_back(std::move(e));
  }
  c->ring = std::move(ring);
  c->certs.clear();
  c->cert_valid.clear();
  ++c->cert_epoch;
  { std::unique_lock<std::shared_mutex> fl(c->cert_fast_mu); c->cert_fast.clear(); c->cert_fast_bytes = 0; }
// ... 817 lines not shown
```

### bftkv_amd/csrc/device_types.h

```cpp
#pragma once
#include <stdint.h>

namespace bftkv {

enum SigStatus : uint8_t {
  ST_OK = 0,
  ST_UNKNOWN_ISSUER = 1,
  ST_PARSE_ERROR = 2,
  ST_NOT_SIGNATURE = 3,
  ST_NO_ISSUER = 4,
  ST_HASH_UNSUPPORTED = 5,
  ST_HASH_TAG = 6,
  ST_ALGO_MISMATCH = 7,
  ST_BAD_SIG = 8,
  ST_KEY_CANNOT_SIGN = 9,
  ST_UNSUPPORTED = 10,
  ST_NOT_EXAMINED = 11,
  ST_PENDING_CHUNKED = 98,
  ST_PENDING_PARSE = 99,
  ST_PENDING_HASH = 100,
  ST_PENDING_RSA = 101,
  ST_PENDING_DSA = 102,
};

constexpr int PK_RSA = 1, PK_RSA_ENCRYPT_ONLY = 2, PK_RSA_SIGN_ONLY = 3, PK_ELGAMAL = 16, PK_DSA = 17, PK_ECDSA = 19;
constexpr int HASH_MD5 = 1, HASH_SHA1 = 2, HASH_RIPEMD160 = 3, HASH_SHA256 = 8, HASH_SHA384 = 9,
              HASH_SHA512 = 10, HASH_SHA224 = 11;

struct SigRec {
  uint64_t body_off;
  uint32_t body_len;
  uint32_t item;
  int32_t key_slot;
  uint32_t mpi_off[2];
  uint16_t mpi_bits[2];
  uint16_t hashed_len;
  uint8_t hash_tag[2];
  uint8_t pk_algo, hash_id, sig_type, status;
  uint8_t after_tag;
  uint8_t flags;
  uint8_t q_kind1;
  uint8_t queued;
  uint32_t pk_idx;
};
constexpr uint8_t AFTER_TAG_PUBKEY = 0xFF;

struct KeyTableDev {
  uint32_t n_keys;
  const uint64_t* key_id;
  const uint64_t* sorted_id;
  const uint32_t* sorted_slot;
  const uint32_t* entity;
  const uint8_t* pk_algo;
  const uint8_t* flags;
  const uint32_t* mod_bits;
  const uint32_t* rsa_e;
  const uint32_t* n_limbs;
  const uint32_t* r2_limbs;
  const uint32_t* r2_limbs80;
  const uint32_t* n0inv;
  const uint32_t* q_words;
  const uint32_t* q_bits;
  const uint32_t* dsa_tab;
  const uint32_t* dsa_slot;
  const uint32_t* dsa_comb;
  uint32_t dsa_wbits;
  uint32_t dsa_entry_limbs;
  uint32_t hash_policy;
};
constexpr uint32_t dsa_nwin(uint32_t wbits) { return (256u + wbits - 1u) / wbits; }
constexpr uint32_t DSA_N_SMALL = 76, DSA_N_BIG = 112;
constexpr uint64_t dsa_comb_limbs_per_key(uint32_t wbits, uint32_t entry_limbs) {
  return 2ull * dsa_nwin(wbits) * ((1u << wbits) - 1u) * entry_limbs;
}
constexpr uint32_t dsa_qpow_words(uint32_t entry_limbs) { return entry_limbs * 10u; }
constexpr uint32_t dsa_qtail_words(uint32_t entry_limbs) { return dsa_qpow_words(entry_limbs) + 12u; }
constexpr bool dsa_plain_window(uint32_t base, uint32_t w, uint32_t nwin) { return base == 1u && w == nwin - 1u; }
constexpr uint64_t dsa_slot_stride(uint32_t wbits, uint32_t entry_limbs) { return dsa_comb_limbs_per_key(wbits, entry_limbs) + dsa_qtail_words(entry_limbs); }

constexpr uint8_t KEYF_USABLE_SIGN = 1, KEYF_CAN_SIGN = 2, KEYF_PRIMARY = 4;
constexpr uint8_t KEYF_CERT_ONLY = 8;
constexpr uint8_t KEYF_CERT_CHECK_ONLY = 16;
constexpr uint8_t KEYF_AMBIGUOUS = 32;
constexpr uint32_t ITEM_FENCED = 0x80000000u;
constexpr uint32_t ITEM_TEXT_SHIFT = 8, ITEM_NEEDS_PAYLOAD = 0x7F7Eu;

struct TextDev {
  uint32_t* mid32;
  uint64_t* mid64;
  uint8_t* tail;
  uint64_t* len;
};

constexpr int MAX_QC = 8;
struct QuorumDev {
  int32_t n_qcs;
  int32_t f[MAX_QC], min[MAX_QC], threshold[MAX_QC], suff[MAX_QC];
  const uint8_t* member;
  uint32_t n_entities;
};

constexpr uint8_t V_IS_QUORUM = 1, V_IS_THRESHOLD = 2, V_IS_SUFFICIENT = 4, V_REJECT = 8;

}
```

### bftkv_amd/csrc/host_bignum.h

```cpp
#pragma once
#include <stdint.h>
#include <string.h>

#include <vector>

namespace bftkv {
namespace hostbn {

constexpr int W28 = 28;
constexpr uint32_t MASK28 = (1u << W28) - 1;

inline void from_be(const uint8_t* be, uint32_t len, uint32_t* w, int nwords) {
  memset(w, 0, sizeof(uint32_t) * nwords);
  for (uint32_t i = 0; i < len; ++i) {
    uint32_t k = len - 1 - i;
    if ((int)(k >> 2) < nwords) w[k >> 2] |= (uint32_t)be[i] << (8 * (k & 3));
  }
}

inline int bit_length(const uint8_t* be, uint32_t len) {
  uint32_t i = 0;
  while (i < len && be[i] == 0) ++i;
  if (i == len) return 0;
  int top = 8;
  while (!((be[i] >> (top - 1)) & 1)) --top;
  return (int)(len - i - 1) * 8 + top;
}

inline int cmp(const uint32_t* a, const uint32_t* b, int n) {
  for (int i = n - 1; i >= 0; --i) {
    if (a[i] != b[i]) return a[i] < b[i] ? -1 : 1;
  }
  return 0;
}
inline void sub(uint32_t* a, const uint32_t* b, int n) {
  uint64_t borrow = 0;
  for (int i = 0; i < n; ++i) {
    uint64_t d = (uint64_t)a[i] - b[i] - borrow;
    a[i] = (uint32_t)d;
    borrow = (d >> 63) & 1;
  }
}
inline void dbl_mod(uint32_t* a, const uint32_t* m, int n) {
  uint32_t c = 0;
  for (int i = 0; i < n; ++i) {
    uint32_t nc = a[i] >> 31;
    a[i] = (a[i] << 1) | c;
    c = nc;
  }
  if (cmp(a, m, n) >= 0) sub(a, m, n);
}

inline void to_limbs28(const uint32_t* w, int nwords, uint32_t* limbs, int nlimbs) {
  for (int j = 0; j < nlimbs; ++j) {
    uint32_t bit = 28u * j, wi = bit >> 5, sh = bit & 31;
    uint64_t v = 0;
    if ((int)wi < nwords) v = w[wi];
    if ((int)wi + 1 < nwords) v |= (uint64_t)w[wi + 1] << 32;
    limbs[j] = (uint32_t)(v >> sh) & MASK28;
  }
}

inline bool mont_setup_by_doubling(const uint8_t* n_be, uint32_t n_len, int nlimbs, uint32_t* n_limbs, uint32_t* r2_limbs,
                                   uint32_t* n0inv) {
  const int nwords = (28 * nlimbs + 31) / 32 + 1;
  std::vector<uint32_t> n(nwords), r(nwords);
  from_be(n_be, n_len, n.data(), nwords);
  if ((n[0] & 1) == 0) return false;
  r.assign(nwords, 0);
  r[0] = 1;
  if (cmp(r.data(), n.data(), nwords) >= 0) { r[0] = 0; }
  for (int i = 0; i < 2 * 28 * nlimbs; ++i) dbl_mod(r.data(), n.data(), nwords);
  to_limbs28(n.data(), nwords, n_limbs, nlimbs);
  to_limbs28(r.data(), nwords, r2_limbs, nlimbs);
  uint32_t n0 = n[0], inv = n0;
  for (int i = 0; i < 5; ++i) inv *= 2u - n0 * inv;
  *n0inv = (0u - inv) & MASK28;
  return true;
}

inline void dbl_mod64(uint64_t* a, const uint64_t* m, int k) {
  uint64_t c = 0;
  for (int i = 0; i < k; ++i) { const uint64_t nc = a[i] >> 63; a[i] = (a[i] << 1) | c; c = nc; }
  bool ge = true;
  for (int i = k - 1; i >= 0; --i) if (a[i] != m[i]) { ge = a[i] > m[i]; break; }
  if (ge) {
    uint64_t borrow = 0;
    for (int i = 0; i < k; ++i) {
      const unsigned __int128 d = (unsigned __int128)a[i] - m[i] - borrow;
      a[i] = (uint64_t)d;
      borrow = (uint64_t)(d >> 64) & 1;
    }
  }
}
inline void montmul64(const uint64_t* a, const uint64_t* b, const uint64_t* m, uint64_t m0inv, int k, uint64_t* out) {
  std::vector<uint64_t> t((size_t)k + 2, 0);
  for (int i = 0; i < k; ++i) {
    unsigned __int128 c = 0;
    for (int j = 0; j < k; ++j) { c += (unsigned __int128)a[j] * b[i] + t[j]; t[j] = (uint64_t)c; c >>= 64; }
    c += t[k]; t[k] = (uint64_t)c; t[k + 1] = (uint64_t)(c >> 64);
    const uint64_t u = t[0] * m0inv;
    c = (unsigned __int128)u * m[0] + t[0];
    c >>= 64;
    for (int j = 1; j < k; ++j) { c += (unsigned __int128)u * m[j] + t[j]; t[j - 1] = (uint64_t)c; c >>= 64; }
    c += t[k]; t[k - 1] = (uint64_t)c; c >>= 64;
    t[k] = t[k + 1] + (uint64_t)c;
  }
  bool ge = t[k] != 0;
  if (!ge) { ge = true; for (int i = k - 1; i >= 0; --i) if (t[i] != m[i]) { ge = t[i] > m[i]; break; } }
  if (ge) {
    uint64_t borrow = 0;
    for (int i = 0; i < k; ++i) {
      const unsigned __int128 d = (unsigned __int128)t[i] - m[i] - borrow;
      t[i] = (uint64_t)d;
      borrow = (uint64_t)(d >> 64) & 1;
    }
  }
  memcpy(out, t.data(), sizeof(uint64_t) * (size_t)k);
}

inline bool mont_setup(const uint8_t* n_be, uint32_t n_len, int nlimbs, uint32_t* n_limbs, uint32_t* r2_limbs, uint32_t* n0inv) {
  const int nwords = (28 * nlimbs + 31) / 32 + 1;
  std::vector<uint32_t> n(nwords);
  from_be(n_be, n_len, n.data(), nwords);
  if ((n[0] & 1) == 0) return false;
  to_limbs28(n.data(), nwords, n_limbs, nlimbs);
  uint32_t n0 = n[0], inv = n0;
  for (int i = 0; i < 5; ++i) inv *= 2u - n0 * inv;
  *n0inv = (0u - inv) & MASK28;
  int top = nwords - 1;
  while (top > 0 && n[top] == 0) --top;
  int bits = 32 * top + 32;
  while (!((n[top] >> ((bits - 1) & 31)) & 1u)) --bits;
  const int k = (bits + 64) / 64;
  if (bits == 1) { for (int j = 0; j < nlimbs; ++j) r2_limbs[j] = 0; return true; }
  if (bits > 28 * nlimbs - 2) return mont_setup_by_doubling(n_be, n_len, nlimbs, n_limbs, r2_limbs, n0inv);
  std::vector<uint64_t> m(k, 0), acc(k, 0), one(k, 0);
  for (int i = 0; i < nwords && i < 2 * k; ++i) m[i >> 1] |= (uint64_t)n[i] << (32 * (i & 1));
  uint64_t m0inv = m[0];
  for (int i = 0; i < 6; ++i) m0inv *= 2ull - m[0] * m0inv;
  m0inv = 0ull - m0inv;
  acc[(bits - 1) >> 6] = 1ull << ((bits - 1) & 63);
  for (int i = bits - 1; i < 64 * k; ++i) dbl_mod64(acc.data(), m.data(), k);
  dbl_mod64(acc.data(), m.data(), k);
  const uint32_t e = 2u * 28u * (uint32_t)nlimbs;
  int hb = 31;
  while (!((e >> hb) & 1u)) --hb;
  for (int b = hb - 1; b >= 0; --b) {
    montmul64(acc.data(), acc.data(), m.data(), m0inv, k, acc.data());
    if ((e >> b) & 1u) dbl_mod64(acc.data(), m.data(), k);
  }
  one[0] = 1;
  montmul64(acc.data(), one.data(), m.data(), m0inv, k, acc.data());
  std::vector<uint32_t> r(nwords, 0);
  for (int i = 0; i < nwords && i < 2 * k; ++i) r[i] = (uint32_t)(acc[i >> 1] >> (32 * (i & 1)));
  to_limbs28(r.data(), nwords, r2_limbs, nlimbs);
  return true;
}

inline void add_mod(uint32_t* a, const uint32_t* b, const uint32_t* m, int n) {
  uint64_t c = 0;
  for (int i = 0; i < n; ++i) { c += (uint64_t)a[i] + b[i]; a[i] = (uint32_t)c; c >>= 32; }
  if (c || cmp(a, m, n) >= 0) sub(a, m, n);
}
inline void mul_mod(const uint32_t* a, const uint32_t* b, const uint32_t* m, uint32_t* r, int n) {
  std::vector<uint32_t> acc(n, 0);
  for (int i = 32 * n - 1; i >= 0; --i) {
    dbl_mod(acc.data(), m, n);
    if ((b[i >> 5] >> (i & 31)) & 1u) add_mod(acc.data(), a, m, n);
  }
  memcpy(r, acc.data(), sizeof(uint32_t) * n);
}
inline void reduce(uint32_t* a, const uint32_t* m, int n) {
  std::vector<uint32_t> r(n, 0);
  for (int i = 32 * n - 1; i >= 0; --i) {
    dbl_mod(r.data(), m, n);
    if ((a[i >> 5] >> (i & 31)) & 1u) {
      uint64_t c = 1;
      for (int k = 0; k < n && c; ++k) { c += r[k]; r[k] = (uint32_t)c; c >>= 32; }
      if (cmp(r.data(), m, n) >= 0) sub(r.data(), m, n);
    }
  }
  memcpy(a, r.data(), sizeof(uint32_t) * n);
}
inline void to_mont_limbs(const uint32_t* x_words, const uint32_t* m, int nwords, int nlimbs, uint32_t* out_limbs) {
  std::vector<uint32_t> t(x_words, x_words + nwords);
  for (int i = 0; i < 28 * nlimbs; ++i) dbl_mod(t.data(), m, nwords);
  to_limbs28(t.data(), nwords, out_limbs, nlimbs);
}

}
}
```

### bftkv_amd/csrc/kernels.hip

```cpp
#include <hip/hip_runtime.h>
#include <stdint.h>

#include "device_types.h"
#include "mont28.h"
#include "u256.h"
#include "hashes.h"

namespace bftkv {

struct ParsedPacket {
  uint64_t next;
  bool event;
  SigRec rec;
};

__host__ __device__ __forceinline__ bool known_tag(uint32_t tag) {
  return tag < 32 && ((0x00066BFEu >> tag) & 1u);
}

struct SubpacketState {
  bool have_ctime = false, have_issuer = false, have_embedded = false;
  bool too_deep = false;
  uint64_t issuer = 0;
};
constexpr uint32_t PARSE_WIN = 64;
constexpr uint32_t PARSE_WIN_STRIDE = 68;
typedef const __attribute__((address_space(3))) uint8_t* lds_bytes_t;
struct WinBytes {
  const uint8_t* g;
  lds_bytes_t l;
  uint32_t n;
  __device__ __forceinline__ uint8_t operator[](uint32_t i) const { return i < n ? l[i] : g[i]; }
  __device__ __forceinline__ WinBytes operator+(uint32_t d) const {
    return d < n ? WinBytes{g + d, l + d, n - d} : WinBytes{g + d, l, 0u};
  }
};

__host__ __device__ __forceinline__ const uint8_t* raw_bytes(const uint8_t* p) { return p; }
__device__ __forceinline__ const uint8_t* raw_bytes(const WinBytes& w) { return w.g; }
struct ChainBytes;
__host__ __device__ inline ChainBytes raw_bytes(const ChainBytes& c);

template <int DEPTH, class B = const uint8_t*>
__host__ __device__ __forceinline__ bool parse_subpackets_t(B p, uint32_t len, bool hashed, SubpacketState& st);

template <int DEPTH, class B = const uint8_t*>
__host__ __device__ __forceinline__ bool parse_sig_body_t(B body, uint32_t blen, SigRec& rec, SubpacketState& st) {
  if (blen < 1) return false;
  if (body[0] != 4) return false;
  if (blen < 6) return false;
  rec.sig_type = body[1];
  rec.pk_algo = body[2];
  rec.hash_id = body[3];
  if (!(rec.pk_algo == PK_RSA || rec.pk_algo == PK_RSA_SIGN_ONLY || rec.pk_algo == PK_DSA || rec.pk_algo == PK_ECDSA))
    return false;
  uint32_t h = rec.hash_id;
  if (!(h == 1 || h == 2 || h == 3 || (h >= 8 && h <= 11))) return false;
  uint32_t hl = ((uint32_t)body[4] << 8) | body[5];
  if (6 + hl > blen) return false;
  rec.hashed_len = (uint16_t)hl;
  if (!parse_subpackets_t<DEPTH, B>(body + 6u, hl, true, st)) return false;
  if (!st.have_ctime) return false;
  uint32_t p = 6 + hl;
  if (p + 2 > blen) return false;
  uint32_t ul = ((uint32_t)body[p] << 8) | body[p + 1];
  p += 2;
  if (p + ul > blen) return false;
  if (!parse_subpackets_t<DEPTH, B>(body + p, ul, false, st)) return false;
  p += ul;
  if (p + 2 > blen) return false;
  rec.hash_tag[0] = body[p];
  rec.hash_tag[1] = body[p + 1];
  p += 2;
  int n_mpi = (rec.pk_algo == PK_RSA || rec.pk_algo == PK_RSA_SIGN_ONLY) ? 1 : 2;
  rec.mpi_off[1] = 0;
  rec.mpi_bits[1] = 0;
  for (int i = 0; i < n_mpi; ++i) {
    if (p + 2 > blen) return false;
    uint32_t bits = ((uint32_t)body[p] << 8) | body[p + 1];
    uint32_t nb = (bits + 7) >> 3;
    p += 2;
    if (p + nb > blen) return false;
    rec.mpi_off[i] = p;
    rec.mpi_bits[i] = (uint16_t)bits;
    p += nb;
  }
  return true;
}

template <int DEPTH, class B>
__host__ __device__ __forceinline__ bool parse_subpackets_t(B a, uint32_t len, bool hashed, SubpacketState& st) {
  uint32_t p = 0;
  while (p < len) {
    uint32_t b = a[p], ln;
    if (b < 192) { ln = b; p += 1; }
    else if (b < 255) {
      if (p + 2 > len) return false;
      ln = ((b - 192) << 8) + a[p + 1] + 192; p += 2;
    } else {
      if (p + 5 > len) return false;
      ln = ((uint32_t)a[p + 1] << 24) | ((uint32_t)a[p + 2] << 16) | ((uint32_t)a[p + 3] << 8) | a[p + 4]; p += 5;
    }
    if (ln > len - p) return false;
    if (ln == 0) return false;
    uint32_t typ = a[p] & 0x7F;
    bool critical = (a[p] & 0x80) != 0;
    const B body = a + (p + 1);
    uint32_t bl = ln - 1;
    p += ln;
    switch (typ) {
      case 2:
        if (!hashed) return false;
        if (bl != 4) return false;
        st.have_ctime = true;
        break;
      case 3: case 9:
        if (!hashed) break;
        if (bl != 4) return false;
        break;
      case 11: case 21: case 22: case 30:
        break;
      case 16:
        if (bl != 8) return false;
        st.issuer = 0;
        for (int i = 0; i < 8; ++i) st.issuer = (st.issuer << 8) | body[i];
        st.have_issuer = true;
        break;
      case 25:
        if (!hashed) break;
        if (bl != 1) return false;
        break;
      case 27: case 29:
        if (!hashed) break;
        if (bl == 0) return false;
        break;
      case 32: {
        if (st.have_embedded) return false;
        st.have_embedded = true;
        if constexpr (DEPTH >= 2) { st.too_deep = true; return false; }
        else {
          SigRec tmp; SubpacketState inner;
          const bool ok = parse_sig_body_t<DEPTH + 1>(raw_bytes(body), bl, tmp, inner);
          if (inner.too_deep) st.too_deep = true;
          if (!ok) return false;
          if (tmp.sig_type != 0x19) return false;
        }
        break;
      }
      default:
        if (critical) return false;
    }
  }
  return true;
}

template <class B = const uint8_t*>
__host__ __device__ __forceinline__ bool parse_sig_body(B body, uint32_t blen, SigRec& rec, bool& have_issuer,
                                                        uint64_t& issuer, bool* too_deep = nullptr) {
  SubpacketState st;
  const bool ok = parse_sig_body_t<0, B>(body, blen, rec, st);
  have_issuer = st.have_issuer;
  issuer = st.issuer;
  if (too_deep) *too_deep = st.too_deep;
  return ok;
}

constexpr uint8_t SIGF_LONG_VALUE = 1, SIGF_V3 = 2, SIGF_MORE_CANDIDATES = 4, SIGF_TEXT = 8;
template <class B = const uint8_t*>
__host__ __device__ __forceinline__ bool parse_sig_body_v3(B body, uint32_t blen, SigRec& rec, uint64_t& issuer) {
  if (blen < 1 || body[0] < 2 || body[0] > 3) return false;
  if (blen < 19) return false;
  if (body[1] != 5) return false;
  rec.sig_type = body[2];
  issuer = 0;
  for (int i = 0; i < 8; ++i) issuer = (issuer << 8) | body[7 + i];
  rec.pk_algo = body[15];
  rec.hash_id = body[16];
  if (!(rec.pk_algo == PK_RSA || rec.pk_algo == PK_RSA_SIGN_ONLY || rec.pk_algo == PK_DSA)) return false;
  const uint32_t h = rec.hash_id;
  if (!(h == 1 || h == 2 || h == 3 || (h >= 8 && h <= 11))) return false;
  rec.hashed_len = 0;
  rec.hash_tag[0] = body[17];
  rec.hash_tag[1] = body[18];
  uint32_t p = 19;
  const int n_mpi = (rec.pk_algo == PK_DSA) ? 2 : 1;
  rec.mpi_off[1] = 0;
  rec.mpi_bits[1] = 0;
  for (int i = 0; i < n_mpi; ++i) {
    if (p + 2 > blen) return false;
    const uint32_t bits = ((uint32_t)body[p] << 8) | body[p + 1];
    const uint32_t nb = (bits + 7) >> 3;
    p += 2;
    if (p + nb > blen) return false;
    rec.mpi_off[i] = p;
    rec.mpi_bits[i] = (uint16_t)bits;
    p += nb;
  }
  return true;
}

constexpr uint8_t BODY_DEFINITE = 0, BODY_PARTIAL = 1, BODY_INDETERMINATE = 2;
constexpr uint32_t BUFIO_SIZE = 4096;
constexpr uint32_t CHAIN_MAX_HOPS = 1024;
constexpr uint32_t CHUNKED_SIG_MAX_BODY = 16384;

struct ChunkCursor { uint64_t pos; uint64_t rem; bool partial; };

__host__ __device__ inline bool cursor_next_chunk(const uint8_t* base, ChunkCursor& c, uint64_t end) {
  while (c.rem == 0) {
    if (!c.partial) return true;
    if (c.pos >= end) return false;
    const uint32_t b = base[c.pos];
    if (b < 192) { c.rem = b; c.pos += 1; c.partial = false; }
    else if (b < 224) {
      if (c.pos + 2 > end) { c.pos = end; return false; }
      c.rem = ((uint64_t)(b - 192) << 8) + base[c.pos + 1] + 192; c.pos += 2; c.partial = false;
    } else if (b == 255) {
      if (c.pos + 5 > end) { c.pos = end; return false; }
      c.rem = ((uint64_t)base[c.pos + 1] << 24) | ((uint64_t)base[c.pos + 2] << 16) | ((uint64_t)base[c.pos + 3] << 8) | base[c.pos + 4];
      c.pos += 5; c.partial = false;
    } else { c.rem = 1ull << (b & 31u); c.pos += 1; }
  }
  return true;
}

struct BodyExtent { uint64_t next, avail; bool truncated, gave_up; };
__host__ __device__ inline BodyExtent chain_extent(const uint8_t* base, ChunkCursor c, uint64_t end, uint32_t max_hops) {
  BodyExtent e{end, 0, false, false};
  for (uint32_t hop = 0;; ++hop) {
    const uint64_t room = end - c.pos, take = c.rem < room ? c.rem : room;
    e.avail += take; c.pos += take;
    if (take < c.rem) { e.truncated = true; return e; }
    c.rem = 0;
    if (!c.partial) { e.next = c.pos; return e; }
    if (hop >= max_hops) { e.gave_up = true; return e; }
    if (!cursor_next_chunk(base, c, end)) { e.truncated = true; return e; }
  }
}

__host__ __device__ inline void chain_copy(const uint8_t* base, ChunkCursor c, uint64_t end, uint8_t* dst, uint64_t n) {
  uint64_t done = 0;
  while (done < n) {
    if (c.rem == 0 && !cursor_next_chunk(base, c, end)) return;
    if (c.rem == 0) return;
    uint64_t take = c.rem < end - c.pos ? c.rem : end - c.pos;
    if (take > n - done) take = n - done;
    if (take == 0) return;
    for (uint64_t i = 0; i < take; ++i) dst[done + i] = base[c.pos + i];
    done += take; c.pos += take; c.rem -= take;
  }
}

struct ChainBytes {
  const uint8_t* base; ChunkCursor c0; uint64_t end; uint32_t skip;
  mutable ChunkCursor cur; mutable uint64_t cur_at; mutable bool cur_ok;
  __host__ __device__ inline ChainBytes(const uint8_t* b, ChunkCursor c, uint64_t e, uint32_t s)
      : base(b), c0(c), end(e), skip(s), cur(c), cur_at(0), cur_ok(true) {}
  __host__ __device__ inline uint8_t operator[](uint32_t i) const {
    const uint64_t want = (uint64_t)skip + i;
    if (!cur_ok || want < cur_at) { cur = c0; cur_at = 0; cur_ok = true; }
    for (;;) {
      if (cur.rem == 0 && (!cursor_next_chunk(base, cur, end) || cur.rem == 0)) { cur_ok = false; return 0; }
      const uint64_t off = want - cur_at;
      if (off < cur.rem) return cur.pos + off < end ? base[cur.pos + off] : 0;
      cur_at += cur.rem; cur.pos += cur.rem; cur.rem = 0;
      if (cur.pos >= end) { cur_ok = false; return 0; }
    }
  }
  __host__ __device__ inline ChainBytes operator+(uint32_t d) const { ChainBytes r(*this); r.skip = skip + d; return r; }
};
__host__ __device__ inline ChainBytes raw_bytes(const ChainBytes& c) { return c; }

struct FetchSim {
  ChunkCursor c; uint64_t end; uint64_t buffered; bool dry;
  __host__ __device__ inline uint64_t fetch(const uint8_t* base, uint64_t req) {
    if (c.rem == 0 && !cursor_next_chunk(base, c, end)) { dry = true; return 0; }
    uint64_t take = c.rem < end - c.pos ? c.rem : end - c.pos;
    if (take > req) take = req;
    if (take == 0) { dry = true; return 0; }
    c.pos += take; c.rem -= take;
    return take;
  }
  __host__ __device__ inline void read_full(const uint8_t* base, uint64_t n) {
    while (n > 0 && !dry) {
      if (buffered == 0) {
        if (n >= BUFIO_SIZE) { n -= fetch(base, n); continue; }
        buffered = fetch(base, BUFIO_SIZE);
        if (buffered == 0) return;
      }
      const uint64_t take = n < buffered ? n : buffered;
      n -= take; buffered -= take;
    }
  }
};

__host__ __device__ inline uint64_t reader_position_after_parse(const uint8_t* base, ChunkCursor body, uint64_t end, const SigRec& rec, bool v3) {
  FetchSim f{body, end, 0, false};
  f.buffered = f.fetch(base, BUFIO_SIZE);
  const int n_mpi = rec.mpi_bits[1] || rec.mpi_off[1] ? 2 : 1;
  if (v3) f.read_full(base, 19);
  else {
    const uint64_t hl = rec.hashed_len, ul = (uint64_t)rec.mpi_off[0] - hl - 12;
    f.read_full(base, 6); f.read_full(base, hl); f.read_full(base, 2); f.read_full(base, ul); f.read_full(base, 2);
  }
  f.read_full(base, 2); f.read_full(base, ((uint64_t)rec.mpi_bits[0] + 7) >> 3);
  if (n_mpi == 2) { f.read_full(base, 2); f.read_full(base, ((uint64_t)rec.mpi_bits[1] + 7) >> 3); }
  return f.dry ? ~0ull : f.c.pos;
}

struct WalkStep {
  uint64_t next;
  uint64_t body_off;
  uint32_t body_len;
  bool event;
  bool reads_to_end;
  bool gave_up;
  uint8_t status;
  uint8_t kind;
};

// ... 182 lines not shown
  const bool usable = (kt.flags[k] & KEYF_USABLE_SIGN) || (cls != 0 && (kt.flags[k] & KEYF_CERT_CHECK_ONLY));
  return usable && (only_ent == 0xFFFFFFFFu ? !(kt.flags[k] & KEYF_CERT_ONLY) : kt.entity[k] == only_ent);
}

struct ParseArgs {
  const uint8_t* sig_blob; const uint64_t* sig_off; const uint32_t* rec_base; const uint32_t* counts; uint32_t n_items;
  const WalkEnt* scratch; uint32_t walk_cap; SigRec* recs; uint32_t n_recs; const uint32_t* cert_ent;
  uint32_t *pk_list, *pk_list3072, *pk_list4096;
  uint32_t* pk_count;
  uint32_t* dsa_list; uint32_t* item_hash_mask;
  const uint8_t* sig_class;
  const uint64_t* forced_issuer;
  const uint32_t* msg_slot;
  const uint8_t* msg_hash;
  const uint8_t* item_flags;
  uint32_t defer_queue;
  const uint32_t* n_recs_dev;
  uint8_t* chunk_arena; uint32_t chunk_cap_units; uint32_t* chunk_bump;
};

__device__ __forceinline__ void parse_one(const ParseArgs& a, const KeyTableDev& kt, uint32_t ri, uint32_t item, uint32_t* win) {
  const uint8_t* __restrict__ sig_blob = a.sig_blob; const uint64_t* __restrict__ sig_off = a.sig_off;
  const uint32_t* __restrict__ rec_base = a.rec_base; const uint32_t* __restrict__ counts = a.counts;
  const WalkEnt* __restrict__ scratch = a.scratch; SigRec* __restrict__ recs = a.recs;
  const uint32_t* __restrict__ cert_ent = a.cert_ent;
  uint32_t* __restrict__ pk_list = a.pk_list; uint32_t* __restrict__ pk_list3072 = a.pk_list3072; uint32_t* __restrict__ pk_list4096 = a.pk_list4096;
  uint32_t* __restrict__ pk_count = a.pk_count; uint32_t* __restrict__ dsa_list = a.dsa_list; uint32_t* __restrict__ item_hash_mask = a.item_hash_mask;
  const uint8_t* __restrict__ sig_class = a.sig_class; const uint32_t* __restrict__ msg_slot = a.msg_slot;
  const uint8_t* __restrict__ msg_hash = a.msg_hash; const uint8_t* __restrict__ item_flags = a.item_flags;
  SigRec rec;
  const uint32_t WALK_CAP = a.walk_cap;
  if (counts[item] <= WALK_CAP && !(item_flags[item] & 2)) {
    const WalkEnt e = scratch[(uint64_t)item * WALK_CAP + (ri - rec_base[item])];
    rec.body_off = sig_off[item] + e.body_rel; rec.body_len = e.body_len_status & 0xFFFFFFu; rec.item = item; rec.key_slot = -1;
    rec.mpi_off[0] = rec.mpi_off[1] = 0; rec.mpi_bits[0] = rec.mpi_bits[1] = 0;
    rec.hashed_len = 0; rec.hash_tag[0] = rec.hash_tag[1] = 0;
    rec.pk_algo = rec.hash_id = rec.sig_type = 0; rec.status = (uint8_t)(e.body_len_status >> 24);
    rec.after_tag = 0; rec.flags = 0; rec.q_kind1 = rec.queued = 0; rec.pk_idx = 0xFFFFFFFFu;
    if (rec.status != ST_PENDING_PARSE && rec.status != ST_PENDING_CHUNKED) { recs[ri] = rec; return; }
  } else {
    rec = recs[ri];
    if (rec.status != ST_PENDING_PARSE && rec.status != ST_PENDING_CHUNKED) return;
  }
  const uint64_t item_end = sig_off[item + 1];
  const bool chunked = rec.status == ST_PENDING_CHUNKED;
  ChunkCursor body_cur{rec.body_off, rec.body_len, false};
  uint64_t body_next = rec.body_off + rec.body_len;
  if (chunked) {
    body_cur = ChunkCursor{rec.body_off, 1ull << (sig_blob[rec.body_off - 1] & 31u), true};
    body_next = chain_extent(sig_blob, body_cur, item_end, 0xFFFFFFFFu).next;
    const uint32_t units = chunk_arena_units(rec.body_len);
    const uint32_t at = a.chunk_arena ? atomicAdd(a.chunk_bump, units) : 0xFFFFFFFFu;
    if (!a.chunk_arena || at > a.chunk_cap_units || units > a.chunk_cap_units - at) {
      rec.status = ST_UNSUPPORTED;
      atomicOr(&item_hash_mask[item], ITEM_FENCED);
      recs[ri] = rec;
      return;
    }
    uint8_t* const lin = a.chunk_arena + 16ull * at;
    chain_copy(sig_blob, body_cur, item_end, lin, rec.body_len);
    rec.body_off = (uint64_t)((uintptr_t)lin - (uintptr_t)sig_blob);
    rec.status = ST_PENDING_PARSE;
  }
  const uint8_t* gbody = sig_blob + rec.body_off;
  const uint64_t room = chunked ? PARSE_WIN : sig_off[a.n_items] - rec.body_off;
  const uint32_t nwin = (room < PARSE_WIN ? (uint32_t)room : PARSE_WIN) & ~15u;
#pragma unroll
  for (uint32_t j = 0; j < PARSE_WIN / 16; ++j) {
    if (16 * j < nwin) {
      uint32_t v[4];
      __builtin_memcpy(v, gbody + 16 * j, 16);
      win[4 * j] = v[0]; win[4 * j + 1] = v[1]; win[4 * j + 2] = v[2]; win[4 * j + 3] = v[3];
    }
  }
  const WinBytes body{gbody, (lds_bytes_t)win, nwin};
  uint8_t st;
  int q_kind = -1;
  bool fence = false;
  const bool v3 = rec.body_len >= 1 && body[0] < 4;
  if (v3 && msg_slot) { st = ST_UNSUPPORTED; fence = true; }
  else {
    bool have_issuer = false, too_deep = false;
    uint64_t issuer = 0;
    bool parsed;
    if (v3) { parsed = parse_sig_body_v3(body, rec.body_len, rec, issuer); have_issuer = parsed; }
    else parsed = parse_sig_body(body, rec.body_len, rec, have_issuer, issuer, &too_deep);
    if (parsed && (chunked || rec.body_len > BUFIO_SIZE) && reader_position_after_parse(sig_blob, body_cur, item_end, rec, v3) != body_next)
      fence = true;
    if (parsed && a.forced_issuer && sig_class && sig_class[rec.item] != 0 && a.forced_issuer[rec.item] != 0) {
      issuer = a.forced_issuer[rec.item];
      have_issuer = true;
    }
    if (!parsed) { st = ST_PARSE_ERROR; fence = too_deep; }
    else if (!have_issuer && !msg_slot) st = ST_NO_ISSUER;
    else {
      const uint32_t only_ent = cert_ent ? cert_ent[rec.item] : 0xFFFFFFFFu;
      int32_t slot = -1;
      const uint32_t cls = sig_class ? sig_class[rec.item] : 0;
      const uint8_t sig_hash_id = rec.hash_id;
      if (msg_slot) { slot = (int32_t)msg_slot[rec.item]; rec.hash_id = msg_hash[rec.item]; }
      if (!msg_slot) {
        uint32_t lo_i = 0, hi_i = kt.n_keys;
        while (lo_i < hi_i) {
          const uint32_t mid = (lo_i + hi_i) >> 1;
          if (kt.sorted_id[mid] < issuer) lo_i = mid + 1; else hi_i = mid;
        }
        int32_t first_any = -1;
        for (uint32_t i = lo_i; i < kt.n_keys && kt.sorted_id[i] == issuer; ++i) {
          const uint32_t k = kt.sorted_slot[i];
          if (!key_is_candidate(kt, k, only_ent, cls)) continue;
          if (first_any < 0) first_any = (int32_t)k;
          if (kt.flags[k] & KEYF_CAN_SIGN) { slot = (int32_t)k; break; }
        }
        if (slot < 0) slot = first_any;
      }
      rec.key_slot = slot;
      const HashInfo hi = hash_info(rec.hash_id);
      const uint32_t hlen = hi.dlen, plen = hi.plen;
      if (slot >= 0 && !msg_slot && (kt.flags[slot] & KEYF_AMBIGUOUS)) rec.flags |= SIGF_MORE_CANDIDATES;
      if (slot < 0) st = ST_UNKNOWN_ISSUER;
      else if (!msg_slot && !sig_class_ok(cls, rec.sig_type) && !(cls == 0 && rec.sig_type == 0x01)) st = ST_HASH_UNSUPPORTED;
      else if (hi.family == 0) st = ST_HASH_UNSUPPORTED;
      else if (hi.le && ((kt.hash_policy >> (hi.idx == 5 ? 0 : 2)) & 3u) != 1u) {
        st = ST_HASH_UNSUPPORTED;
        fence = ((kt.hash_policy >> (hi.idx == 5 ? 0 : 2)) & 3u) == 0u;
      }
      else if (!(kt.flags[slot] & KEYF_CAN_SIGN)) st = ST_KEY_CANNOT_SIGN;
      else {
        st = ST_PENDING_HASH;
        if (!msg_slot && cls == 0 && rec.sig_type == 0x01) {
          rec.flags |= SIGF_TEXT;
          atomicOr(&item_hash_mask[rec.item], 1u << (ITEM_TEXT_SHIFT + hi.idx));
          pk_count[4] = 1u;
        } else if (rec.hash_id != HASH_SHA256) { atomicOr(&item_hash_mask[rec.item], 1u << hi.idx); pk_count[4] = 1u; }
        if (kt.pk_algo[slot] != rec.pk_algo) rec.after_tag = ST_ALGO_MISMATCH;
        else if ((rec.pk_algo == PK_RSA || rec.pk_algo == PK_RSA_SIGN_ONLY) && sig_hash_id != rec.hash_id)
          rec.after_tag = ST_BAD_SIG;
        else if (rec.pk_algo == PK_RSA || rec.pk_algo == PK_RSA_SIGN_ONLY) {
          const uint32_t mod_bits = kt.mod_bits[slot];
          const uint32_t kbytes = (mod_bits + 7) >> 3;
          const uint32_t nb = (rec.mpi_bits[0] + 7u) >> 3;
          const WinBytes mp = body + (uint32_t)rec.mpi_off[0];
          uint32_t lead = 0;
          while (lead < nb && mp[lead] == 0) ++lead;
          const uint32_t vbytes = nb - lead;
          const uint32_t cls_sz = mod_bits <= 2048 ? 0u : (mod_bits <= 3072 ? 1u : 2u);
          const uint32_t cap_bytes = (cls_sz == 0 ? MONT_N : cls_sz == 1 ? MONT_TPI_BIG * MONT_L3072 : MONT_TPI_BIG * MONT_L4096) * MONT_W / 8;
          if (mod_bits == 0xFFFFFFFFu) { rec.after_tag = ST_UNSUPPORTED; fence = true; }
          else if (kbytes < hlen + plen + 11) rec.after_tag = ST_BAD_SIG;
          else if (vbytes > cap_bytes) { rec.after_tag = ST_BAD_SIG; fence = true; }
          else {
            rec.after_tag = AFTER_TAG_PUBKEY;
            rec.flags |= (vbytes > kbytes) ? SIGF_LONG_VALUE : 0;
            q_kind = cls_sz == 0 ? 0 : (int)cls_sz + 1;
          }
        } else if (rec.pk_algo == PK_DSA) {
          if (kt.mod_bits[slot] == 0xFFFFFFFFu) { rec.after_tag = ST_UNSUPPORTED; fence = true; }
          else {
            rec.after_tag = AFTER_TAG_PUBKEY;
            q_kind = 1;
          }
        } else { rec.after_tag = ST_UNSUPPORTED; fence = true; }
      }
    }
  }
  if (fence) atomicOr(&item_hash_mask[rec.item], ITEM_FENCED);
  if (v3) rec.flags |= SIGF_V3;
  rec.q_kind1 = (uint8_t)(q_kind + 1);
  if (!a.defer_queue) {
    uint32_t* const lists[4] = {pk_list, dsa_list, pk_list3072, pk_list4096};
#pragma unroll
    for (int k = 0; k < 4; ++k) {
      const uint32_t idx = wave_alloc(pk_count + k, q_kind == k);
      if (q_kind == k) { rec.pk_idx = idx; rec.queued = 1; lists[k][idx] = ri; }
    }
  }
  rec.status = st;
  recs[ri] = rec;
}

__global__ void __launch_bounds__(256) k_parse_body(ParseArgs a, KeyTableDev kt) {
  const uint32_t ri = blockIdx.x * blockDim.x + threadIdx.x;
  if (ri >= (a.n_recs_dev ? *a.n_recs_dev : a.n_recs)) return;
  uint32_t lo = 0, hi = a.n_items;
  while (hi - lo > 1) {
    const uint32_t mid = (lo + hi) >> 1;
    if (a.rec_base[mid] <= ri) lo = mid; else hi = mid;
  }
  __shared__ uint32_t win_sh[256 * (PARSE_WIN_STRIDE / 4)];
  parse_one(a, kt, ri, lo, win_sh + threadIdx.x * (PARSE_WIN_STRIDE / 4));
}

constexpr int PARSE_ITEM_BLOCK = 128;
__global__ void __launch_bounds__(PARSE_ITEM_BLOCK) k_parse_body_items(ParseArgs a, KeyTableDev kt) {
  const uint32_t item = blockIdx.x;
  const uint32_t cnt = a.counts[item], base = a.rec_base[item];
  __shared__ uint32_t win_sh[PARSE_ITEM_BLOCK * (PARSE_WIN_STRIDE / 4)];
  for (uint32_t j = threadIdx.x; j < cnt; j += PARSE_ITEM_BLOCK) parse_one(a, kt, base + j, item, win_sh + threadIdx.x * (PARSE_WIN_STRIDE / 4));
}

template <bool FILL>
__global__ void __launch_bounds__(64) k_signers(const uint8_t* __restrict__ sig_blob, const uint64_t* __restrict__ sig_off,
                                                uint32_t n_items, uint32_t* __restrict__ counts,
                                                const uint32_t* __restrict__ out_base, uint64_t* __restrict__ ids_out,
                                                KeyTableDev kt, uint8_t* __restrict__ fenced ) {
  uint32_t item = blockIdx.x * blockDim.x + threadIdx.x;
  if (item >= n_items) return;
  uint64_t pos = sig_off[item], end = sig_off[item + 1];
  uint32_t n = 0;
  uint32_t base = FILL ? out_base[item] : 0;
  bool fence = false;
  while (pos < end) {
    WalkStep w = walk_next_dev(sig_blob, pos, end);
    pos = w.next;
    if (!w.event) continue;
    if (w.status == ST_UNSUPPORTED || (w.status == ST_NOT_SIGNATURE && !w.reads_to_end)) fence = true;
    if (w.status == ST_NOT_SIGNATURE) continue;
    if (w.status != ST_PENDING_PARSE && w.status != ST_PENDING_CHUNKED) break;
    SigRec tmp;
    bool have_issuer = false, too_deep = false, parsed, v3;
    uint64_t issuer = 0;
    ChunkCursor cur{w.body_off, w.body_len, false};
    if (w.status == ST_PENDING_CHUNKED) {
      cur = ChunkCursor{w.body_off, 1ull << (sig_blob[w.body_off - 1] & 31u), true};
      const ChainBytes body(sig_blob, cur, end, 0u);
      v3 = w.body_len >= 1 && body[0] < 4;
      parsed = v3 ? parse_sig_body_v3(body, w.body_len, tmp, issuer) : parse_sig_body(body, w.body_len, tmp, have_issuer, issuer, &too_deep);
    } else {
      const uint8_t* body = sig_blob + w.body_off;
      v3 = w.body_len >= 1 && body[0] < 4;
      parsed = v3 ? parse_sig_body_v3(body, w.body_len, tmp, issuer) : parse_sig_body(body, w.body_len, tmp, have_issuer, issuer, &too_deep);
    }
    if (!parsed) { fence |= too_deep; break; }
    if ((w.status == ST_PENDING_CHUNKED || w.body_len > BUFIO_SIZE) && reader_position_after_parse(sig_blob, cur, end, tmp, v3) != w.next)
      fence = true;
    if (v3) continue;
    if (!have_issuer) { fence = true; break; }
    for (uint32_t k = 0; k < kt.n_keys; ++k) {
      if (kt.key_id[k] == issuer && (kt.flags[k] & KEYF_PRIMARY) && !(kt.flags[k] & KEYF_CERT_ONLY)) {
        if (FILL) ids_out[base + n] = issuer;
        ++n;
        break;
      }
    }
  }
  if (!FILL) { counts[item] = n; if (fenced) fenced[item] = fence ? 1 : 0; }
}

__global__ void __launch_bounds__(1024) k_scan_counts(uint32_t* __restrict__ counts, uint32_t n,
                                                      uint32_t* __restrict__ base, uint32_t* __restrict__ total,
                                                      uint32_t* __restrict__ host_total, uint32_t* __restrict__ pk_count ,
                                                      uint32_t* __restrict__ item_hash_mask , uint32_t cap,
                                                      uint32_t* __restrict__ chunk_ctr ) {
  __shared__ uint32_t part[1024];
  uint32_t t = threadIdx.x;
  uint32_t chunk = (n + 1023) / 1024;
  uint32_t lo = t * chunk, hi = min(n, lo + chunk);
  uint32_t s = 0;
  for (uint32_t i = lo; i < hi; ++i) s += counts[i];
  part[t] = s;
  if (pk_count && t < 24) pk_count[t] = 0;
  if (item_hash_mask) for (uint32_t i = lo; i < hi; ++i) item_hash_mask[i] = 0;
  __syncthreads();
  for (uint32_t off = 1; off < 1024; off <<= 1) {
    uint32_t v = (t >= off) ? part[t - off] : 0;
    __syncthreads();
    part[t] += v;
    __syncthreads();
  }
  const uint32_t all = part[1023];
  if (cap && all > cap) {
    for (uint32_t i = lo; i < hi; ++i) { base[i] = 0; counts[i] = 0; }
    if (t == 1023) { total[0] = 0; total[1] = all; if (chunk_ctr) { chunk_ctr[0] = 0; chunk_ctr[1] = 0; chunk_ctr[2] = 0; } }
    return;
  }
  uint32_t run = (t == 0) ? 0 : part[t - 1];
  for (uint32_t i = lo; i < hi; ++i) { base[i] = run; run += counts[i]; }
  if (t == 1023) {
    total[0] = all; total[1] = 0;
    uint32_t units = 0;
    if (chunk_ctr) { units = chunk_ctr[0]; chunk_ctr[0] = 0; chunk_ctr[1] = 0; chunk_ctr[2] = units; }
    if (host_total) {
      host_total[2] = units;
      __hip_atomic_store(host_total, all, __ATOMIC_RELEASE, __HIP_MEMORY_SCOPE_SYSTEM);
    }
  }
}

__device__ __forceinline__ void load_block_raw(const uint8_t* p, uint32_t (&t)[17]) {
  const uint32_t mis = (uint32_t)((uintptr_t)p & 3);
  const uint32_t* ap = (const uint32_t*)((uintptr_t)p & ~(uintptr_t)3);
#pragma unroll
  for (int i = 0; i < 16; ++i) t[i] = ap[i];
  t[16] = mis ? ap[16] : 0;
}
__device__ __forceinline__ void block_raw_to_be(const uint8_t* p, const uint32_t (&t)[17], uint32_t (&w)[16]) {
  const uint32_t mis = (uint32_t)((uintptr_t)p & 3);
#pragma unroll
  for (int i = 0; i < 16; ++i) w[i] = __builtin_bswap32(__builtin_amdgcn_alignbyte(t[i + 1], t[i], mis));
}
__device__ __forceinline__ void load_block_be(const uint8_t* p, uint32_t (&w)[16]) {
  uint32_t t[17];
  load_block_raw(p, t);
  block_raw_to_be(p, t, w);
}

// ... 2 lines not shown
  uint32_t item = blockIdx.x * blockDim.x + threadIdx.x;
  if (item >= n_items) return;
  const uint8_t* p = tbs_blob + tbs_off[item];
  const uint64_t nblk = (tbs_off[item + 1] - tbs_off[item]) >> 6;
  uint32_t s[8];
  sha256_init(s);
  uint32_t ta[17], tb[17], w[16];
  if (nblk) load_block_raw(p, ta);
  uint64_t blk = 0;
  for (; blk + 1 < nblk; blk += 2) {
    load_block_raw(p + (blk + 1) * 64, tb);
    block_raw_to_be(p + blk * 64, ta, w);
    sha256_compress(s, w);
    if (blk + 2 < nblk) load_block_raw(p + (blk + 2) * 64, ta);
    block_raw_to_be(p + (blk + 1) * 64, tb, w);
    sha256_compress(s, w);
  }
  if (blk < nblk) {
    block_raw_to_be(p + blk * 64, ta, w);
    sha256_compress(s, w);
  }
#pragma unroll
  for (int i = 0; i < 8; ++i) mid[(uint64_t)item * 8 + i] = s[i];
}

__device__ __forceinline__ void load_block_le(const uint8_t* p, uint32_t (&w)[16]) {
  uint32_t t[17];
  load_block_raw(p, t);
  const uint32_t mis = (uint32_t)((uintptr_t)p & 3);
#pragma unroll
  for (int i = 0; i < 16; ++i) w[i] = __builtin_amdgcn_alignbyte(t[i + 1], t[i], mis);
}
__global__ void __launch_bounds__(64) k_hash_mid_other(const uint8_t* __restrict__ tbs_blob, const uint64_t* __restrict__ tbs_off,
                                                       uint32_t n_items, const uint32_t* __restrict__ item_hash_mask,
                                                       uint32_t* __restrict__ mid32 , uint64_t* __restrict__ mid64 ) {
  const uint32_t item = blockIdx.x * blockDim.x + threadIdx.x;
  const uint32_t which = blockIdx.y;
  if (item >= n_items) return;
  if (!((item_hash_mask[item] >> (which + 1)) & 1u)) return;
  const uint8_t* p = tbs_blob + tbs_off[item];
  const uint64_t len = tbs_off[item + 1] - tbs_off[item];
  if (which < 2 || which >= 4) {
    uint32_t s[8];
    if (which == 0) sha224_init(s); else if (which == 1) sha1_init(s); else if (which == 4) md5_init(s); else ripemd160_init(s);
    for (uint64_t blk = 0; blk < (len >> 6); ++blk) {
      uint32_t w[16];
      if (which >= 4) { load_block_le(p + blk * 64, w); if (which == 4) md5_compress(s, w); else ripemd160_compress(s, w); }
      else { load_block_be(p + blk * 64, w); if (which == 0) sha256_compress(s, w); else sha1_compress(s, w); }
    }
    const uint32_t slot32 = which < 2 ? which + 1 : which - 1;
    uint32_t* o = mid32 + ((uint64_t)slot32 * n_items + item) * 8;
#pragma unroll
    for (int i = 0; i < 8; ++i) o[i] = s[i];
  } else {
    uint64_t s[8];
    if (which == 2) sha512_init(s); else sha384_init(s);
    for (uint64_t blk = 0; blk < (len >> 7); ++blk) {
      uint32_t lo[16], hi[16];
      load_block_be(p + blk * 128, lo);
      load_block_be(p + blk * 128 + 64, hi);
      uint64_t w[16];
#pragma unroll
      for (int i = 0; i < 8; ++i) { w[i] = ((uint64_t)lo[2 * i] << 32) | lo[2 * i + 1]; w[8 + i] = ((uint64_t)hi[2 * i] << 32) | hi[2 * i + 1]; }
      sha512_compress(s, w);
    }
    uint64_t* o = mid64 + ((uint64_t)(which - 2) * n_items + item) * 8;
#pragma unroll
    for (int i = 0; i < 8; ++i) o[i] = s[i];
  }
}

__global__ void __launch_bounds__(64) k_hash_mid_text(const uint8_t* __restrict__ tbs_blob, const uint64_t* __restrict__ tbs_off,
                                                      uint32_t n_items, const uint32_t* __restrict__ item_hash_mask, TextDev txt) {
  const uint32_t item = blockIdx.x * blockDim.x + threadIdx.x;
  const uint32_t which = blockIdx.y;
  if (item >= n_items) return;
  if (!((item_hash_mask[item] >> (ITEM_TEXT_SHIFT + which)) & 1u)) return;
  const uint8_t* p = tbs_blob + tbs_off[item];
  const uint64_t len = tbs_off[item + 1] - tbs_off[item];
  const bool wide = which == 3 || which == 4;
  const uint32_t B = wide ? 128u : 64u;
  uint32_t s32[8];
  uint64_t s64[8];
  if (which == 0) sha256_init(s32); else if (which == 1) sha224_init(s32); else if (which == 2) sha1_init(s32);
  else if (which == 3) sha512_init(s64); else if (which == 4) sha384_init(s64); else if (which == 5) md5_init(s32); else ripemd160_init(s32);
  uint8_t buf[128];
  uint32_t fill = 0;
  uint64_t total = 0;
  auto put = [&](uint8_t c) {
    buf[fill++] = c;
    ++total;
    if (fill == B) {
      if (which >= 5) {
        uint32_t w[16];
#pragma unroll
        for (int i = 0; i < 16; ++i) w[i] = (uint32_t)buf[4 * i] | ((uint32_t)buf[4 * i + 1] << 8) | ((uint32_t)buf[4 * i + 2] << 16) | ((uint32_t)buf[4 * i + 3] << 24);
        if (which == 5) md5_compress(s32, w); else ripemd160_compress(s32, w);
      } else if (!wide) {
        uint32_t w[16];
#pragma unroll
        for (int i = 0; i < 16; ++i) w[i] = ((uint32_t)buf[4 * i] << 24) | ((uint32_t)buf[4 * i + 1] << 16) | ((uint32_t)buf[4 * i + 2] << 8) | buf[4 * i + 3];
        if (which == 2) sha1_compress(s32, w); else sha256_compress(s32, w);
      } else {
        uint64_t w[16];
#pragma unroll
        for (int i = 0; i < 16; ++i) {
          uint64_t v = 0;
#pragma unroll
          for (int t = 0; t < 8; ++t) v = (v << 8) | buf[8 * i + t];
          w[i] = v;
        }
        sha512_compress(s64, w);
      }
      fill = 0;
    }
  };
  int st = 0;
  for (uint64_t i = 0; i < len; ++i) {
    const uint8_t c = p[i];
    if (st == 0) {
      if (c == 0x0D) { st = 1; put(c); }
      else if (c == 0x0A) { put(0x0D); put(0x0A); }
      else put(c);
    } else { st = 0; put(c); }
  }
  const uint64_t slot = (uint64_t)which * n_items + item;
  if (!wide) {
    const uint32_t slot32 = which < 3 ? which : which - 2;
    for (int i = 0; i < 8; ++i) txt.mid32[((uint64_t)slot32 * n_items + item) * 8 + i] = s32[i];
  } else { for (int i = 0; i < 8; ++i) txt.mid64[((uint64_t)(which - 3) * n_items + item) * 8 + i] = s64[i]; }
  for (uint32_t i = 0; i < fill; ++i) txt.tail[slot * 128 + i] = buf[i];
  txt.len[slot] = total;
}

struct TailSrc {
  const uint8_t* tail; uint32_t tail_len;
  const uint8_t* body; uint32_t pre_len;
  uint32_t tr_len;
  uint32_t rep;
};
__device__ __forceinline__ uint32_t tail_byte(const TailSrc& t, uint32_t j) {
  if (j < t.tail_len) return t.tail[j];
  j -= t.tail_len;
  const uint32_t unit = t.pre_len + t.tr_len;
  if (j >= unit * t.rep) return (j == unit * t.rep) ? 0x80 : 0;
  if (t.rep > 1) j %= unit;
  if (j < t.pre_len) return t.body[j];
  j -= t.pre_len;
  if (j == 0) return 0x04;
  if (j == 1) return 0xFF;
  return (t.pre_len >> (8 * (5 - j))) & 0xFF;
}

template <typename F>
__device__ __forceinline__ uint32_t limb28(F byte_from_lsb, int j) {
  uint32_t bit = 28u * (uint32_t)j;
  uint32_t b0 = bit >> 3, sh = bit & 7;
  uint64_t v = 0;
#pragma unroll
  for (int t = 0; t < 5; ++t) v |= (uint64_t)byte_from_lsb(b0 + t) << (8 * t);
  return (uint32_t)(v >> sh) & MONT_MASK;
}

template <bool OTHERS>
__device__ __forceinline__ void digest_body(const uint8_t* __restrict__ tbs_blob, const uint64_t* __restrict__ tbs_off,
                                            const uint8_t* __restrict__ sig_blob, const uint32_t* __restrict__ mid32,
                                            const uint64_t* __restrict__ mid64, uint32_t n_items,
                                            SigRec* __restrict__ recs, uint32_t n_recs, uint32_t* __restrict__ digests ,
                                            uint32_t ri_in, const uint64_t* __restrict__ tbs_prefix = nullptr, uint32_t rep = 1,
                                            uint32_t* __restrict__ tag_only = nullptr, TextDev txt = TextDev{nullptr, nullptr, nullptr, nullptr}) {
  const uint32_t ri = ri_in;
  if (ri >= n_recs) return;
  const SigRec rec = recs[ri];
  if (!tag_only && rec.status != ST_PENDING_HASH) return;
  const bool text = OTHERS && (rec.flags & SIGF_TEXT) != 0;
  if (!tag_only && ((rec.hash_id != HASH_SHA256) || (rec.flags & SIGF_TEXT) != 0) != OTHERS) return;
  if (OTHERS && text && !txt.len) return;
  const HashInfo hi = OTHERS ? hash_info(rec.hash_id) : HashInfo{32, 0, 32, 19};
  const uint64_t seg = tbs_off[rec.item + 1] - tbs_off[rec.item];
  const uint32_t bmask = (OTHERS && hi.family == 64) ? 127u : 63u;
  const uint64_t tslot = (uint64_t)hi.idx * n_items + rec.item;
  const uint64_t tlen = text ? txt.len[tslot] : (tbs_prefix ? tbs_prefix[rec.item] + seg : seg);
  TailSrc ts;
  ts.tail_len = text ? (uint32_t)(tlen & bmask) : (tbs_prefix ? (uint32_t)seg : (uint32_t)(tlen & bmask));
  ts.tail = text ? txt.tail + tslot * 128 : tbs_blob + tbs_off[rec.item] + (seg - ts.tail_len);
  const bool v3 = (rec.flags & SIGF_V3) != 0;
  ts.body = sig_blob + rec.body_off + (v3 ? 2 : 0);
  ts.pre_len = v3 ? 5u : 6u + rec.hashed_len;
  ts.tr_len = v3 ? 0u : 6u;
  ts.rep = rep;
  const uint32_t rem = ts.tail_len + (ts.pre_len + ts.tr_len) * rep;
  const uint64_t bits = (tlen + (uint64_t)(ts.pre_len + ts.tr_len) * rep) * 8;
  uint32_t dg_dummy[16];
  uint32_t* dg = tag_only ? dg_dummy : digests + (uint64_t)ri * 16;
  uint32_t tag_hi;
  if (!OTHERS || hi.family == 32) {
    const uint32_t nblk = (rem + 9 + 63) >> 6;
    uint32_t s[8];
    const uint32_t* m = (text ? txt.mid32 : mid32) + ((uint64_t)hi.slot * n_items + rec.item) * 8;
#pragma unroll
    for (int i = 0; i < 8; ++i) s[i] = m[i];
    const bool le = OTHERS && hi.le;
    for (uint32_t blk = 0; blk < nblk; ++blk) {
      uint32_t w[16];
#pragma unroll
      for (int i = 0; i < 16; ++i) {
        uint32_t j = blk * 64 + i * 4;
        const uint32_t be = (tail_byte(ts, j) << 24) | (tail_byte(ts, j + 1) << 16) | (tail_byte(ts, j + 2) << 8) | tail_byte(ts, j + 3);
        w[i] = le ? __builtin_bswap32(be) : be;
      }
      if (blk == nblk - 1) { w[14] = le ? (uint32_t)bits : (uint32_t)(bits >> 32); w[15] = le ? (uint32_t)(bits >> 32) : (uint32_t)bits; }
      if (OTHERS && hi.slot == 2) sha1_compress(s, w);
      else if (OTHERS && hi.slot == 3) md5_compress(s, w);
      else if (OTHERS && hi.slot == 4) ripemd160_compress(s, w);
      else sha256_compress(s, w);
    }
#pragma unroll
    for (int i = 0; i < 8; ++i) dg[i] = le ? s[i] : __builtin_bswap32(s[i]);
    tag_hi = le ? __builtin_bswap32(s[0]) : s[0];
  } else if (OTHERS) {
    const uint32_t nblk = (rem + 17 + 127) >> 7;
    uint64_t s[8];
    const uint64_t* m = (text ? txt.mid64 : mid64) + ((uint64_t)hi.slot * n_items + rec.item) * 8;
#pragma unroll
    for (int i = 0; i < 8; ++i) s[i] = m[i];
    for (uint32_t blk = 0; blk < nblk; ++blk) {
      uint64_t w[16];
#pragma unroll
      for (int i = 0; i < 16; ++i) {
        uint32_t j = blk * 128 + i * 8;
        uint64_t v = 0;
#pragma unroll
        for (int t = 0; t < 8; ++t) v = (v << 8) | tail_byte(ts, j + t);
        w[i] = v;
      }
      if (blk == nblk - 1) { w[14] = 0; w[15] = bits; }
      sha512_compress(s, w);
    }
#pragma unroll
    for (int i = 0; i < 8; ++i) { dg[2 * i] = __builtin_bswap32((uint32_t)(s[i] >> 32)); dg[2 * i + 1] = __builtin_bswap32((uint32_t)s[i]); }
    tag_hi = (uint32_t)(s[0] >> 32);
  } else {
    tag_hi = 0;
  }
  if (tag_only) { *tag_only = tag_hi >> 16; return; }
  uint8_t st;
  if ((uint8_t)(tag_hi >> 24) != rec.hash_tag[0] || (uint8_t)(tag_hi >> 16) != rec.hash_tag[1]) st = ST_HASH_TAG;
  else st = (rec.after_tag == AFTER_TAG_PUBKEY) ? (uint8_t)ST_PENDING_RSA : rec.after_tag;
  recs[ri].status = st;
}

__global__ void __launch_bounds__(256) k_digest_sha256(const uint8_t* __restrict__ tbs_blob, const uint64_t* __restrict__ tbs_off,
                                                       const uint8_t* __restrict__ sig_blob, const uint32_t* __restrict__ mid32,
                                                       const uint64_t* __restrict__ mid64, uint32_t n_items, SigRec* __restrict__ recs,
                                                       uint32_t n_recs, uint32_t* __restrict__ digests,
                                                       const uint64_t* __restrict__ tbs_prefix, const uint32_t* __restrict__ n_recs_dev) {
  digest_body<false>(tbs_blob, tbs_off, sig_blob, mid32, mid64, n_items, recs, n_recs_dev ? *n_recs_dev : n_recs, digests,
                     blockIdx.x * blockDim.x + threadIdx.x, tbs_prefix);
}
__global__ void __launch_bounds__(256) k_digest_other(const uint8_t* __restrict__ tbs_blob, const uint64_t* __restrict__ tbs_off,
                                                         const uint8_t* __restrict__ sig_blob, const uint32_t* __restrict__ mid32,
                                                         const uint64_t* __restrict__ mid64, uint32_t n_items, SigRec* __restrict__ recs,
                                                         uint32_t n_recs, uint32_t* __restrict__ digests,
                                                         const uint32_t* __restrict__ any_other , TextDev txt,
                                                         const uint32_t* __restrict__ n_recs_dev ) {
  if (*any_other == 0) return;
  if (n_recs_dev) n_recs = *n_recs_dev;
  for (uint64_t ri = (uint64_t)blockIdx.x * blockDim.x + threadIdx.x; ri < n_recs; ri += (uint64_t)gridDim.x * blockDim.x)
    digest_body<true>(tbs_blob, tbs_off, sig_blob, mid32, mid64, n_items, recs, n_recs, digests, (uint32_t)ri, nullptr, 1, nullptr, txt);
}

__global__ void __launch_bounds__(64) k_candidates(const uint8_t* __restrict__ tbs_blob, const uint64_t* __restrict__ tbs_off,
                                                   const uint8_t* __restrict__ sig_blob, const uint32_t* __restrict__ mid32,
                                                   const uint64_t* __restrict__ mid64, uint32_t n_items, SigRec* __restrict__ recs,
                                                   uint32_t n_recs, const uint32_t* __restrict__ n_recs_dev, const uint64_t* __restrict__ tbs_prefix,
                                                   KeyTableDev kt, const uint32_t* __restrict__ cert_ent, const uint8_t* __restrict__ sig_class,
                                                   TextDev txt, uint32_t* __restrict__ item_hash_mask) {
  const uint32_t ri = blockIdx.x * blockDim.x + threadIdx.x;
  const uint32_t nr = n_recs_dev ? *n_recs_dev : n_recs;
  if (ri >= nr) return;
  const SigRec rec = recs[ri];
  if (!(rec.flags & SIGF_MORE_CANDIDATES)) return;
  uint8_t st = rec.status;
  if (!(st == ST_KEY_CANNOT_SIGN || st == ST_HASH_TAG || st == ST_ALGO_MISMATCH || st == ST_BAD_SIG)) return;
  if (tbs_prefix && (rec.hash_id != HASH_SHA256 || (rec.flags & SIGF_TEXT))) return;
  const uint32_t slot = (uint32_t)rec.key_slot;
  const uint64_t issuer = kt.key_id[slot];
  const uint32_t only_ent = cert_ent ? cert_ent[rec.item] : 0xFFFFFFFFu;
  const uint32_t cls = sig_class ? sig_class[rec.item] : 0;
  uint32_t lo_i = 0, hi_i = kt.n_keys;
  while (lo_i < hi_i) {
    const uint32_t mid = (lo_i + hi_i) >> 1;
    if (kt.sorted_id[mid] < issuer) lo_i = mid + 1; else hi_i = mid;
  }
  bool behind = false;
  uint32_t writes = (kt.flags[slot] & KEYF_CAN_SIGN) ? 1u : 0u;
  for (uint32_t i = lo_i; i < kt.n_keys && kt.sorted_id[i] == issuer; ++i) {
    const uint32_t k = kt.sorted_slot[i];
    if (!key_is_candidate(kt, k, only_ent, cls)) continue;
    if (k == slot) { behind = true; continue; }
    if (!behind) continue;
    if (!(kt.flags[k] & KEYF_CAN_SIGN)) { st = ST_KEY_CANNOT_SIGN; continue; }
    ++writes;
    uint32_t tag = 0;
    if (rec.hash_id == HASH_SHA256 && !(rec.flags & SIGF_TEXT))
      digest_body<false>(tbs_blob, tbs_off, sig_blob, mid32, mid64, n_items, recs, nr, nullptr, ri, tbs_prefix, writes, &tag);
    else digest_body<true>(tbs_blob, tbs_off, sig_blob, mid32, mid64, n_items, recs, nr, nullptr, ri, tbs_prefix, writes, &tag, txt);
    if ((uint8_t)(tag >> 8) != rec.hash_tag[0] || (uint8_t)tag != rec.hash_tag[1]) st = ST_HASH_TAG;
    else if (kt.pk_algo[k] != rec.pk_algo) st = ST_ALGO_MISMATCH;
    else {
      st = ST_BAD_SIG;
      atomicOr(&item_hash_mask[rec.item], ITEM_FENCED);
    }
  }
  recs[ri].status = st;
}

constexpr int RSA_BLOCK = 256;
constexpr int QUADS_PER_BLOCK = RSA_BLOCK / MONT_TPI;
#ifndef BFTKV_MODEXP_BLOCK
#define BFTKV_MODEXP_BLOCK 256
#endif
constexpr int MODEXP_BLOCK = BFTKV_MODEXP_BLOCK;

enum : int { OP_TO_MONT = 0, OP_SQR = 1, OP_MULX = 2, OP_MULP = 3, OP_MUL1 = 4 };

constexpr int EM_LOW_BYTES = 84;
constexpr int EM_LOW_LIMBS = EM_LOW_BYTES * 8 / MONT_W;
static_assert(EM_LOW_LIMBS * MONT_W == EM_LOW_BYTES * 8, "the EM split must fall on a limb boundary");
constexpr uint32_t EM_HEAD_BAD = 0xFFFFFFFFu;

__device__ __forceinline__ uint32_t em_head_limb(uint32_t gi, uint32_t kbytes) {
  const int32_t top = 8 * ((int32_t)kbytes - 2), lo = (int32_t)gi * MONT_W;
  if (top < lo) return 0u;
  if (top >= lo + MONT_W - 1) return MONT_MASK;
  return (1u << (top - lo + 1)) - 1u;
}

template <int L, int TPI>
__global__ void __launch_bounds__(MODEXP_BLOCK, 3) k_rsa_modexp(const uint8_t* __restrict__ sig_blob, const SigRec* __restrict__ recs,
                                                          const uint32_t* __restrict__ pk_list, const uint32_t* __restrict__ pk_count_ptr,
                                                          const uint32_t* __restrict__ pk_start_ptr,
                                                          KeyTableDev kt, uint32_t* __restrict__ r_low,
                                                          uint32_t* __restrict__ xr_scratch, uint64_t* __restrict__ clk) {
  constexpr int NL = TPI * L;
  constexpr int GROUPS = MODEXP_BLOCK / TPI;
  const bool stamp = clk && blockIdx.x == 0 && threadIdx.x == 0;
  uint64_t t0 = 0, r0 = 0;
  if (stamp) { t0 = __builtin_readcyclecounter(); r0 = __builtin_amdgcn_s_memrealtime(); }
  __shared__ uint32_t a_sh[GROUPS * NL];
  __shared__ uint32_t x_sh[GROUPS * NL];
  const uint32_t count = *pk_count_ptr, start = *pk_start_ptr;
  if (start + blockIdx.x * GROUPS >= count) return;
  const uint32_t quad = threadIdx.x / TPI;
  const int qlane = threadIdx.x % TPI;
  const uint32_t gq = start + blockIdx.x * GROUPS + quad;
  const bool active = gq < count;
  const uint32_t pi = active ? gq : (count - 1);
  const uint32_t ri = pk_list[pi];
  const SigRec rec = recs[ri];
  const uint32_t key = (uint32_t)rec.key_slot;
  uint32_t* a_lds = a_sh + quad * NL + qlane * L;
  const uint32_t* a_rd = a_sh + quad * NL;
  uint32_t* x_lds = x_sh + quad * NL + qlane * L;

  uint32_t n[L], b[L], y[L];
  const uint32_t* np = kt.n_limbs + (uint64_t)key * MONT_NMAX + qlane * L;
  const uint32_t* rp = (L == 10 && TPI == 8) ? kt.r2_limbs80 + (uint64_t)key * 80 + qlane * L
                                              : kt.r2_limbs + (uint64_t)key * MONT_NMAX + qlane * L;
  uint32_t* xrp = xr_scratch + (uint64_t)pi * NL + qlane * L;
#pragma unroll
  for (int k = 0; k < L; ++k) n[k] = np[k];
  {
    const uint32_t nb = (rec.mpi_bits[0] + 7u) >> 3;
    const uint8_t* mp = sig_blob + rec.body_off + rec.mpi_off[0];
    auto sig_b = [&](uint32_t i) -> uint32_t { return i < nb ? mp[nb - 1 - i] : 0u; };
#pragma unroll
    for (int k = 0; k < L; ++k) x_lds[k] = limb28(sig_b, qlane * L + k);
  }
  const uint32_t n0inv = kt.n0inv[key];
  const uint32_t e = kt.rsa_e[key];
  const uint32_t kbytes = (kt.mod_bits[key] + 7) >> 3;
  const uint32_t cls = (e << 1) | (((e & 1u) && e > 1u && !(rec.flags & 1u)) ? 1u : 0u);

  uint64_t todo = __builtin_amdgcn_ballot_w64(true);
  while (todo) {
    const int lead = __builtin_ctzll(todo);
    const uint32_t cls_u = (uint32_t)__builtin_amdgcn_readlane((int)cls, lead);
    const bool live = (cls == cls_u);
    const uint32_t e_u = cls_u >> 1;
    const bool sc_u = cls_u & 1u;
    const int top = 31 - __builtin_clz(e_u | 1u);
    int kind = OP_TO_MONT, bitpos = top;
    while (true) {
      if (kind == OP_TO_MONT) {
#pragma unroll
        for (int k = 0; k < L; ++k) { b[k] = rp[k]; a_lds[k] = x_lds[k]; }
      } else {
#pragma unroll
        for (int k = 0; k < L; ++k) b[k] = y[k];
        if (kind == OP_SQR) {
#pragma unroll
          for (int k = 0; k < L; ++k) a_lds[k] = y[k];
        } else if (kind == OP_MULX) {
#pragma unroll
          for (int k = 0; k < L; ++k) a_lds[k] = xrp[k];
        } else if (kind == OP_MULP) {
#pragma unroll
          for (int k = 0; k < L; ++k) a_lds[k] = x_lds[k];
        } else {
#pragma unroll
          for (int k = 0; k < L; ++k) a_lds[k] = (qlane == 0 && k == 0) ? 1u : 0u;
        }
      }
      __builtin_amdgcn_fence(__ATOMIC_ACQ_REL, "wavefront");
      if (kind == OP_SQR) mont_mul<L, TPI, true>(y, a_rd, b, n, n0inv, qlane);
      else mont_mul<L, TPI, false>(y, a_rd, b, n, n0inv, qlane);
      __builtin_amdgcn_fence(__ATOMIC_ACQ_REL, "wavefront");
      if (kind == OP_TO_MONT && (e_u & (e_u - 1u)) != 0 && !(sc_u && __builtin_popcount(e_u) == 2)) {
#pragma unroll
        for (int k = 0; k < L; ++k) xrp[k] = y[k];
      }
      if (kind == OP_MULP || kind == OP_MUL1) break;
      if (kind == OP_SQR && ((e_u >> bitpos) & 1u)) { kind = (bitpos == 0 && sc_u) ? OP_MULP : OP_MULX; continue; }
      --bitpos;
      kind = (bitpos >= 0) ? OP_SQR : OP_MUL1;
    }
    canonicalize<L, TPI>(y, qlane);
    if (e_u == 0) {
#pragma unroll
      for (int k = 0; k < L; ++k) y[k] = (qlane == 0 && k == 0) ? 1u : 0u;
    }
    uint32_t head = 0;
#pragma unroll
    for (int k = 0; k < L; ++k) {
      const uint32_t gi = (uint32_t)qlane * L + k;
      if (gi >= (uint32_t)EM_LOW_LIMBS) head |= y[k] ^ em_head_limb(gi, kbytes);
    }
    head = grp_or<TPI>(head);
    if (head != 0 && qlane == 0) y[0] = EM_HEAD_BAD;
#pragma unroll
    for (int k = 0; k < L; ++k) a_lds[k] = y[k];
    __builtin_amdgcn_fence(__ATOMIC_ACQ_REL, "wavefront");
    if (live && active && qlane < 4) {
      uint32_t* out = r_low + (uint64_t)pi * EM_LOW_LIMBS + qlane * (EM_LOW_LIMBS / 4);
      const uint32_t* src = a_rd + qlane * (EM_LOW_LIMBS / 4);
#pragma unroll
      for (int k = 0; k < EM_LOW_LIMBS / 4; ++k) out[k] = src[k];
    }
    __builtin_amdgcn_fence(__ATOMIC_ACQ_REL, "wavefront");
    todo &= ~__builtin_amdgcn_ballot_w64(live);
  }
  if (stamp && *pk_start_ptr == 0) { clk[0] = __builtin_readcyclecounter() - t0; clk[1] = __builtin_amdgcn_s_memrealtime() - r0; }
}

constexpr int CMP_LANES = 4;
constexpr int CMP_L = EM_LOW_LIMBS / CMP_LANES;
static_assert(CMP_L * CMP_LANES == EM_LOW_LIMBS, "the low limbs divide over the quad");
__global__ void __launch_bounds__(256) k_rsa_compare(SigRec* __restrict__ recs, const uint32_t* __restrict__ pk_list,
                                                     const uint32_t* __restrict__ pk_count_ptr, const uint32_t* __restrict__ pk_start_ptr,
                                                     KeyTableDev kt,
                                                     const uint32_t* __restrict__ r_low, const uint32_t* __restrict__ digests) {
  constexpr int GROUPS = 256 / CMP_LANES;
  const uint32_t count = *pk_count_ptr, start = *pk_start_ptr;
  const uint32_t q0 = start + blockIdx.x * GROUPS;
  if (q0 >= count) return;
  const uint32_t gq = q0 + threadIdx.x / CMP_LANES;
  const int qlane = threadIdx.x % CMP_LANES;
  const bool active = gq < count;
  const uint32_t pi = active ? gq : (count - 1);
  const uint32_t ri = pk_list[pi];
  const SigRec rec = recs[ri];
  const bool pending = rec.status == ST_PENDING_RSA;
  const uint32_t key = (uint32_t)rec.key_slot;
  const uint32_t kbytes = (kt.mod_bits[key] + 7) >> 3;
  const HashInfo hi = hash_info(rec.hash_id);
  const uint32_t hlen = hi.dlen, plen = hi.plen, tl = hlen + plen;
  constexpr int EM_TAIL_W = 24;
  __shared__ uint32_t tail_sh[GROUPS * EM_TAIL_W];
  uint32_t* tail = tail_sh + (threadIdx.x / CMP_LANES) * EM_TAIL_W;
  const uint32_t* dgw = digests + (uint64_t)ri * 16;
  const uint32_t hw = hlen >> 2;
#pragma unroll
  for (int t = 0; t < EM_TAIL_W / CMP_LANES; ++t) {
    const uint32_t w = (uint32_t)qlane * (EM_TAIL_W / CMP_LANES) + t;
    uint32_t v = 0;
    if (w < hw) v = __builtin_bswap32(dgw[hw - 1 - w]);
    else {
#pragma unroll
      for (uint32_t bq = 0; bq < 4; ++bq) {
        const uint32_t i = 4 * w + bq;
        if (i >= hlen && i < tl) v |= digestinfo_byte(rec.hash_id, plen - 1 - (i - hlen)) << (8 * bq);
      }
    }
    tail[w] = v;
  }
  __builtin_amdgcn_fence(__ATOMIC_ACQ_REL, "wavefront");
  auto em_word = [&](uint32_t w) -> uint32_t {
    if (4 * w + 3 <= tl) return tail[w];
    if (4 * w > tl && 4 * w + 3 + 2 < kbytes) return 0xFFFFFFFFu;
    uint32_t v = 0;
#pragma unroll
    for (uint32_t bq = 0; bq < 4; ++bq) {
      const uint32_t i = 4 * w + bq;
      uint32_t byte;
      if (i <= tl) byte = (tail[i >> 2] >> (8 * (i & 3))) & 0xFFu;
      else if (i + 2 < kbytes) byte = 0xFF;
      else byte = (i + 2 == kbytes) ? 1u : 0u;
      v |= byte << (8 * bq);
    }
    return v;
  };
  constexpr int NW = (CMP_L * MONT_W + 31) / 32 + 1;
  const uint32_t bit0 = (uint32_t)qlane * CMP_L * MONT_W, w0 = bit0 >> 5, s0 = bit0 & 31u;
  uint32_t Wd[NW + 1], Wn[NW];
#pragma unroll
  for (int i = 0; i <= NW; ++i) Wd[i] = em_word(w0 + i);
#pragma unroll
  for (int i = 0; i < NW; ++i) Wn[i] = __builtin_amdgcn_alignbit(Wd[i + 1], Wd[i], s0);
  __shared__ uint32_t r_sh[GROUPS * EM_LOW_LIMBS];
  {
    const uint32_t n_valid = min((uint32_t)GROUPS, count - q0) * EM_LOW_LIMBS;
    const uint32_t* src = r_low + (uint64_t)q0 * EM_LOW_LIMBS;
    for (uint32_t t = threadIdx.x; t < GROUPS * EM_LOW_LIMBS; t += 256) r_sh[t] = t < n_valid ? src[t] : 0u;
    __syncthreads();
  }
  const uint32_t* rp = r_sh + (threadIdx.x / CMP_LANES) * EM_LOW_LIMBS + qlane * CMP_L;
  uint32_t diff = 0;
#pragma unroll
  for (int k = 0; k < CMP_L; ++k) {
    const int bit = MONT_W * k, wi = bit >> 5, sh = bit & 31;
    const uint32_t em = (sh == 0 ? Wn[wi] : __builtin_amdgcn_alignbit(Wn[wi + 1], Wn[wi], sh)) & MONT_MASK;
    diff |= em ^ rp[k];
  }
  diff = quad_or(diff);
  if (active && pending && qlane == 0) recs[ri].status = (diff == 0) ? ST_OK : ST_BAD_SIG;
}

constexpr int DSA_U_WORDS = 24;
__device__ __forceinline__ const uint32_t* dsa_slot_base(const KeyTableDev& kt, uint32_t key) {
  return kt.dsa_comb + (uint64_t)kt.dsa_slot[key] * dsa_slot_stride(kt.dsa_wbits, kt.dsa_entry_limbs);
}
__device__ __forceinline__ const uint32_t* dsa_qconst(const KeyTableDev& kt, uint32_t key) {
  return dsa_slot_base(kt, key) + dsa_comb_limbs_per_key(kt.dsa_wbits, kt.dsa_entry_limbs) + dsa_qpow_words(kt.dsa_entry_limbs);
}
__global__ void __launch_bounds__(64) k_dsa_inv(const uint8_t* __restrict__ sig_blob, const SigRec* __restrict__ recs,
                                                const uint32_t* __restrict__ dsa_list, const uint32_t* __restrict__ pk_count,
                                                const uint32_t* __restrict__ pk_start,
                                                KeyTableDev kt, uint32_t* __restrict__ dsa_u , uint32_t batch_min) {
  if (pk_count[1] - pk_start[1] >= batch_min) return;
  const uint32_t di = pk_start[1] + blockIdx.x * blockDim.x + threadIdx.x;
  if (di >= pk_count[1]) return;
  const uint32_t ri = dsa_list[di];
  const uint32_t key = (uint32_t)recs[ri].key_slot;
  const uint64_t body_off = recs[ri].body_off;
  const uint32_t off0 = recs[ri].mpi_off[0], off1 = recs[ri].mpi_off[1], bits0 = recs[ri].mpi_bits[0], bits1 = recs[ri].mpi_bits[1];
  U256 q, r, s_, w;
  for (int i = 0; i < 8; ++i) q.w[i] = kt.q_words[(uint64_t)key * 8 + i];
  const uint32_t qbits = kt.q_bits[key];
  const uint8_t* body = sig_blob + body_off;
  bool ok = u256_from_be(body + off0, (bits0 + 7u) >> 3, r);
  ok = u256_from_be(body + off1, (bits1 + 7u) >> 3, s_) && ok;
  ok = ok && !u256_is_zero(r) && u256_cmp(r, q) < 0 && !u256_is_zero(s_) && u256_cmp(s_, q) < 0;
  ok = ok && (qbits & 7u) == 0;
  ok = ok && u256_modinv_odd(s_, q, w);
  U256 u2 = u256_zero();
  if (ok) {
    const uint32_t* qc = dsa_qconst(kt, key);
    U256 r2;
    for (int i = 0; i < 8; ++i) r2.w[i] = qc[i];
    u2 = u256_mulmod_mont(w, r, q, qc[8], r2);
  } else w = u256_zero();
  uint32_t* o = dsa_u + (uint64_t)di * DSA_U_WORDS;
  for (int i = 0; i < 8; ++i) { o[i] = w.w[i]; o[8 + i] = u2.w[i]; o[16 + i] = r.w[i]; }
}

constexpr int INV_BLOCK = 256, INV_PER_THREAD = 16, INV_TILE = INV_BLOCK * INV_PER_THREAD, INV_MAX_SLOTS = 4096;
__global__ void __launch_bounds__(INV_BLOCK) k_dsa_inv_batched(const uint8_t* __restrict__ sig_blob, const SigRec* __restrict__ recs,
                                                               const uint32_t* __restrict__ dsa_list, const uint32_t* __restrict__ pk_count,
                                                               const uint32_t* __restrict__ pk_start,
                                                               KeyTableDev kt, uint32_t* __restrict__ dsa_u , uint32_t batch_min) {
  if (pk_count[1] - pk_start[1] < batch_min) return;
  __shared__ uint32_t bins[INV_MAX_SLOTS];
  __shared__ uint32_t tsum[INV_BLOCK];
  __shared__ uint16_t order[INV_TILE], slot_of[INV_TILE];
  const uint32_t count = pk_count[1], start = pk_start[1];
  const uint32_t tile0 = start + blockIdx.x * INV_TILE;
  if (tile0 >= count) return;
  const uint32_t n = min((uint32_t)INV_TILE, count - tile0);
  const uint32_t t = threadIdx.x;
#pragma unroll
  for (int j = 0; j < INV_MAX_SLOTS / INV_BLOCK; ++j) bins[t + INV_BLOCK * j] = 0;
  __syncthreads();
  for (int j = 0; j < INV_PER_THREAD; ++j) {
    const uint32_t e = t + INV_BLOCK * j;
    if (e < n) {
      const uint32_t sl = kt.dsa_slot[(uint32_t)recs[dsa_list[tile0 + e]].key_slot] & (INV_MAX_SLOTS - 1);
      slot_of[e] = (uint16_t)sl;
      atomicAdd(&bins[sl], 1u);
    }
  }
// ... 296 lines not shown
        for (int k = 0; k < L; ++k) a_lds[k] = (qlane == 0 && k == 0) ? 1u : 0u;
      }
    }
    __builtin_amdgcn_fence(__ATOMIC_ACQ_REL, "wavefront");
    if (__any(need && started)) {
#pragma unroll
      for (int k = 0; k < L; ++k) b[k] = y[k];
      mont_mul<L, TPI>(t, a_rd, b, n, n0inv, qlane);
      __builtin_amdgcn_fence(__ATOMIC_ACQ_REL, "wavefront");
    }
    if (__any(need && !started)) {
      if (need) {
#pragma unroll
        for (int k = 0; k < L; ++k) y[k] = started ? t[k] : a_lds[k];
      }
      __builtin_amdgcn_fence(__ATOMIC_ACQ_REL, "wavefront");
    } else if (need) {
#pragma unroll
      for (int k = 0; k < L; ++k) y[k] = t[k];
    }
    started = started || need;
  }
#pragma unroll
  for (int k = 0; k < L; ++k) t[k] = y[k];
  canonicalize<L, TPI>(t, qlane);
  reduce_once<L, TPI>(t, n, qlane);
  uint32_t diff = 0;
#pragma unroll
  for (int k = 0; k < L; ++k) diff |= t[k];
  diff = grp_or<TPI>(diff);
  uint64_t col[10];
#pragma unroll
  for (int j = 0; j < 10; ++j) col[j] = 0;
  const uint32_t* pw = slot_base + dsa_comb_limbs_per_key(wbits, E) + (qlane * L) * 10;
  if (mine) {
#pragma unroll
    for (int k = 0; k < L; ++k) {
#pragma unroll
      for (int j = 0; j < 10; ++j) col[j] = mad64(t[k], pw[k * 10 + j], col[j]);
    }
  }
#pragma unroll
  for (int j = 0; j < 10; ++j) col[j] = grp_sum64<TPI>(col[j]);
  uint32_t W[12];
#pragma unroll
  for (int i = 0; i < 12; ++i) W[i] = 0;
  uint64_t carry = 0;
#pragma unroll
  for (int j = 0; j < 12; ++j) {
    const uint64_t sacc = (j < 10 ? col[j] : 0ull) + carry;
    const uint32_t limb = (uint32_t)sacc & MONT_MASK;
    carry = sacc >> MONT_W;
    const int bit = MONT_W * j, wi = bit >> 5, sh = bit & 31;
    W[wi] |= limb << sh;
    if (sh > 4 && wi + 1 < 12) W[wi + 1] |= limb >> (32 - sh);
  }
  U256 q, rr, acc;
#pragma unroll
  for (int i = 0; i < 8; ++i) { q.w[i] = kt.q_words[(uint64_t)key * 8 + i]; rr.w[i] = up[16 + i]; }
#pragma unroll
  for (int i = 0; i < 8; ++i) acc.w[i] = (W[i + 1] >> 3) | (W[i + 2] << 29);
  if (u256_cmp(acc, q) >= 0) u256_sub(acc, q);
  const uint64_t low = ((uint64_t)(W[1] & 7u) << 32) | W[0];
#pragma unroll 1
  for (int bit = 34; bit >= 0; --bit) {
    uint32_t cbit = u256_shl1(acc);
    acc.w[0] |= (uint32_t)(low >> bit) & 1u;
    if (cbit || u256_cmp(acc, q) >= 0) u256_sub(acc, q);
  }
  if (live && qlane == 0) recs[ri].status = (diff != 0 && u256_cmp(acc, rr) == 0) ? ST_OK : ST_BAD_SIG;
}


__global__ void __launch_bounds__(RSA_BLOCK) k_modexp(uint32_t n_ops, const uint32_t* __restrict__ base_limbs ,
                                                      const uint32_t* __restrict__ mod_idx, const uint32_t* __restrict__ n_limbs,
                                                      const uint32_t* __restrict__ r2_limbs, const uint32_t* __restrict__ n0inv_tab,
                                                      const uint32_t* __restrict__ exp_words ,
                                                      uint32_t exp_nwords, uint32_t exp_per_op, uint32_t* __restrict__ out_limbs) {
  __shared__ uint32_t a_sh[QUADS_PER_BLOCK * MONT_N];
  __shared__ uint32_t x_sh[QUADS_PER_BLOCK * MONT_N];
  constexpr int L = MONT_L;
  const uint32_t quad = threadIdx.x >> 2;
  const int qlane = threadIdx.x & 3;
  const uint32_t gq = blockIdx.x * QUADS_PER_BLOCK + quad;
  const bool active = gq < n_ops;
  const uint32_t op = active ? gq : (n_ops - 1);
  const uint32_t mi = mod_idx[op];
  uint32_t* a_lds = a_sh + quad * MONT_N + qlane * L;
  uint32_t* x_lds = x_sh + quad * MONT_N + qlane * L;
  const uint32_t* a_rd = a_sh + quad * MONT_N;
  const uint32_t* x_rd = x_sh + quad * MONT_N;
  uint32_t n[L], b[L], y[L], t[L];
#pragma unroll
  for (int k = 0; k < L; ++k) n[k] = n_limbs[(uint64_t)mi * MONT_N + qlane * L + k];
  const uint32_t n0inv = n0inv_tab[mi];
  const uint32_t* ew = exp_words + (uint64_t)(exp_per_op ? op : mi) * exp_nwords;
  const int nbits = (int)exp_nwords * 32;
  for (int step = -2; step <= 2 * nbits; ++step) {
    const uint32_t* ard = a_rd;
    if (step == -2) {
#pragma unroll
      for (int k = 0; k < L; ++k) { b[k] = r2_limbs[(uint64_t)mi * MONT_N + qlane * L + k]; a_lds[k] = base_limbs[(uint64_t)op * MONT_N + qlane * L + k]; }
    } else if (step == -1 || step == 2 * nbits) {
#pragma unroll
      for (int k = 0; k < L; ++k) a_lds[k] = (qlane == 0 && k == 0) ? 1u : 0u;
      if (step >= 0) {
#pragma unroll
        for (int k = 0; k < L; ++k) b[k] = y[k];
      }
    } else if ((step & 1) == 0) {
#pragma unroll
      for (int k = 0; k < L; ++k) { a_lds[k] = y[k]; b[k] = y[k]; }
    } else {
#pragma unroll
      for (int k = 0; k < L; ++k) b[k] = y[k];
      ard = x_rd;
    }
    __builtin_amdgcn_fence(__ATOMIC_ACQ_REL, "wavefront");
    if (step >= 0 && step < 2 * nbits && (step & 1) == 0) mont_mul<L, MONT_TPI, true>(t, ard, b, n, n0inv, qlane);
    else mont_mul(t, ard, b, n, n0inv, qlane);
    __builtin_amdgcn_fence(__ATOMIC_ACQ_REL, "wavefront");
    if (step == -2) {
#pragma unroll
      for (int k = 0; k < L; ++k) x_lds[k] = t[k];
    } else if (step >= 0 && step < 2 * nbits && (step & 1)) {
      const int bi = nbits - 1 - (step >> 1);
      const bool bit = (ew[bi >> 5] >> (bi & 31)) & 1u;
      if (bit) {
#pragma unroll
        for (int k = 0; k < L; ++k) y[k] = t[k];
      }
    } else {
#pragma unroll
      for (int k = 0; k < L; ++k) y[k] = t[k];
    }
  }
  canonicalize(y, qlane);
  uint32_t diff = 0;
#pragma unroll
  for (int k = 0; k < L; ++k) diff |= y[k] ^ n[k];
  diff = quad_or(diff);
  if (active) {
#pragma unroll
    for (int k = 0; k < L; ++k) out_limbs[(uint64_t)op * MONT_N + qlane * L + k] = (diff == 0) ? 0u : y[k];
  }
}

__global__ void k_bytes_to_limbs(const uint8_t* __restrict__ src, uint32_t nbytes, uint32_t n_nums, uint32_t* __restrict__ dst) {
  uint32_t i = blockIdx.x * blockDim.x + threadIdx.x;
  if (i >= n_nums * MONT_N) return;
  uint32_t num = i / MONT_N, j = i % MONT_N;
  const uint8_t* p = src + (uint64_t)num * nbytes;
  auto bf = [&](uint32_t k) -> uint32_t { return k < nbytes ? p[nbytes - 1 - k] : 0u; };
  dst[i] = limb28(bf, (int)j);
}
__global__ void k_limbs_to_bytes(const uint32_t* __restrict__ src, uint32_t nbytes, uint32_t n_nums, uint8_t* __restrict__ dst) {
  uint32_t i = blockIdx.x * blockDim.x + threadIdx.x;
  if (i >= n_nums * nbytes) return;
  uint32_t num = i / nbytes, k = i % nbytes;
  uint32_t bit = k * 8, j = bit / 28, sh = bit % 28;
  const uint32_t* l = src + (uint64_t)num * MONT_N;
  uint64_t v = (j < MONT_N ? l[j] : 0u);
  if (j + 1 < MONT_N) v |= (uint64_t)l[j + 1] << 28;
  dst[(uint64_t)num * nbytes + (nbytes - 1 - k)] = (uint8_t)(v >> sh);
}

__global__ void __launch_bounds__(256) k_tally(const SigRec* __restrict__ recs, const uint32_t* __restrict__ rec_base,
                                               const uint32_t* __restrict__ counts, uint32_t n_items, KeyTableDev kt,
                                               QuorumDev q, uint8_t* __restrict__ verdict, uint32_t* __restrict__ n_verified,
                                               uint32_t* __restrict__ clique_counts ) {
  const uint32_t wave = (blockIdx.x * blockDim.x + threadIdx.x) >> 6;
  const uint32_t lane = threadIdx.x & 63;
  if (wave >= n_items) return;
  const uint32_t base = rec_base[wave], cnt = counts[wave];
  uint32_t cq[MAX_QC];
#pragma unroll
  for (int c = 0; c < MAX_QC; ++c) cq[c] = 0;
  uint32_t total_ok = 0;
  uint32_t first_suff = 0xFFFFFFFFu;
  for (uint32_t off = 0; off < cnt; off += 64) {
    const uint32_t i = off + lane;
    bool ok = false;
    uint32_t ent = 0;
    if (i < cnt) {
      const SigRec r = recs[base + i];
      ok = (r.status == ST_OK);
      if (ok) ent = kt.entity[r.key_slot];
    }
    const uint64_t okm = __builtin_amdgcn_ballot_w64(ok);
    const uint64_t below = (lane == 0) ? 0ull : (~0ull >> (64 - lane));
    bool reached = false;
#pragma unroll
    for (int c = 0; c < MAX_QC; ++c) {
      if (c < q.n_qcs) {
        const bool mem = ok && q.member[(uint64_t)c * q.n_entities + ent];
        const uint64_t mm = __builtin_amdgcn_ballot_w64(mem);
        const uint32_t run = cq[c] + (uint32_t)__builtin_popcountll(mm & below) + (mem ? 1u : 0u);
        if (ok && q.suff[c] > 0 && run >= (uint32_t)q.suff[c]) reached = true;
        cq[c] += (uint32_t)__builtin_popcountll(mm);
      }
    }
    const uint64_t rm = __builtin_amdgcn_ballot_w64(reached);
    if (rm != 0 && first_suff == 0xFFFFFFFFu) {
      const uint32_t fl = (uint32_t)__builtin_ctzll(rm);
      first_suff = total_ok + (uint32_t)__builtin_popcountll(okm & ((fl == 63) ? ~0ull : ((1ull << (fl + 1)) - 1)));
    }
    total_ok += (uint32_t)__builtin_popcountll(okm);
  }
  if (lane == 0) {
    bool is_quorum = q.n_qcs > 0, is_thr = q.n_qcs > 0, is_suff = false, reject = true;
    for (int c = 0; c < q.n_qcs; ++c) {
      if (q.f[c] > 0 && (int32_t)cq[c] < q.min[c]) is_quorum = false;
      if (q.threshold[c] > 0 && (int32_t)cq[c] < q.threshold[c]) is_thr = false;
      if (q.suff[c] > 0 && (int32_t)cq[c] >= q.suff[c]) is_suff = true;
      if (q.f[c] == 0 || (int32_t)cq[c] <= q.f[c]) reject = false;
    }
    verdict[wave] = (is_quorum ? V_IS_QUORUM : 0) | (is_thr ? V_IS_THRESHOLD : 0) | (is_suff ? V_IS_SUFFICIENT : 0) |
                    (reject ? V_REJECT : 0);
    n_verified[wave] = is_suff ? first_suff : total_ok;
    if (clique_counts)
      for (int c = 0; c < MAX_QC; ++c) clique_counts[(uint64_t)wave * MAX_QC + c] = cq[c];
  }
}

struct PlanArgs {
  SigRec* recs; const uint32_t* rec_base; const uint32_t* counts; uint32_t n_items;
  uint32_t *pk_list, *dsa_list, *pk_list3072, *pk_list4096;
  uint32_t* pk_count;
  uint32_t* plan_cut;
  const uint8_t* verdict;
  uint32_t margin;
  uint32_t* mail;
};

constexpr int PLAN_BLOCK = 1024, PLAN_ITEMS = PLAN_BLOCK / 64;
template <int PHASE>
__global__ void __launch_bounds__(PLAN_BLOCK) k_plan(PlanArgs a, KeyTableDev kt, QuorumDev q) {
  __shared__ uint32_t cnt_sh[PLAN_ITEMS][4];
  const uint32_t wib = threadIdx.x >> 6, lane = threadIdx.x & 63;
  const uint32_t item = blockIdx.x * PLAN_ITEMS + wib;
  if (PHASE == 1 && a.mail && blockIdx.x == 0 && threadIdx.x == 0)
    __hip_atomic_store(a.mail, 0x80000000u | (a.pk_count[4] ? 1u : 0u), __ATOMIC_RELEASE, __HIP_MEMORY_SCOPE_SYSTEM);
  const bool have = item < a.n_items;
  const uint32_t base = have ? a.rec_base[item] : 0, cnt = have ? a.counts[item] : 0;
  uint32_t* const lists[4] = {a.pk_list, a.dsa_list, a.pk_list3072, a.pk_list4096};
  const uint64_t below = (lane == 0) ? 0ull : (~0ull >> (64 - lane));
  uint32_t from = 0, covered = cnt;
  if (PHASE == 1) {
    uint32_t cq[MAX_QC];
#pragma unroll
    for (int c = 0; c < MAX_QC; ++c) cq[c] = 0;
    bool done = false;
    for (uint32_t off = 0; off < cnt && !done; off += 64) {
      const uint32_t i = off + lane;
      uint32_t kind = 0, ent = 0;
      if (i < cnt) {
        kind = a.recs[base + i].q_kind1;
        if (kind) ent = kt.entity[a.recs[base + i].key_slot];
      }
      bool reached = false;
#pragma unroll
      for (int c = 0; c < MAX_QC; ++c) {
        if (c < q.n_qcs) {
          const bool mem = kind != 0 && q.member[(uint64_t)c * q.n_entities + ent];
          const uint64_t mm = __builtin_amdgcn_ballot_w64(mem);
          const uint32_t run = cq[c] + (uint32_t)__builtin_popcountll(mm & below) + (mem ? 1u : 0u);
          if (mem && q.suff[c] > 0 && run >= (uint32_t)q.suff[c] + a.margin) reached = true;
          cq[c] += (uint32_t)__builtin_popcountll(mm);
        }
      }
      const uint64_t rm = __builtin_amdgcn_ballot_w64(reached);
      if (rm) { done = true; covered = off + (uint32_t)__builtin_ctzll(rm) + 1; }
    }
  } else {
    from = have ? a.plan_cut[item] : 0;
    if (!have || (a.verdict[item] & V_IS_SUFFICIENT)) from = covered;
  }
  auto wants = [&](uint32_t i, uint32_t& kind) -> bool {
    kind = 0;
    if (i >= covered) return false;
    if (PHASE == 1) { kind = a.recs[base + i].q_kind1; return kind != 0; }
    const SigRec r = a.recs[base + i];
    kind = r.q_kind1;
    return kind != 0 && !r.queued && r.status == ST_PENDING_RSA;
  };
  uint32_t n_k[4] = {0, 0, 0, 0};
  for (uint32_t off = from; off < covered; off += 64) {
    uint32_t kind;
    const bool w = wants(off + lane, kind);
#pragma unroll
    for (int k = 0; k < 4; ++k) n_k[k] += (uint32_t)__builtin_popcountll(__builtin_amdgcn_ballot_w64(w && kind == (uint32_t)k + 1));
  }
  if (lane == 0) {
#pragma unroll
    for (int k = 0; k < 4; ++k) cnt_sh[wib][k] = n_k[k];
  }
  __syncthreads();
  if (threadIdx.x < 4) {
    uint32_t tot = 0;
    for (int w = 0; w < PLAN_ITEMS; ++w) { const uint32_t v = cnt_sh[w][threadIdx.x]; cnt_sh[w][threadIdx.x] = tot; tot += v; }
    const uint32_t b0 = tot ? atomicAdd(a.pk_count + threadIdx.x, tot) : 0u;
    for (int w = 0; w < PLAN_ITEMS; ++w) cnt_sh[w][threadIdx.x] += b0;
  }
  __syncthreads();
  uint32_t run_k[4];
#pragma unroll
  for (int k = 0; k < 4; ++k) run_k[k] = cnt_sh[wib][k];
// ... 88 lines not shown
```

### bftkv_amd/csrc/mont28.h

```cpp
#pragma once
#include <hip/hip_runtime.h>
#include <stdint.h>

namespace bftkv {

constexpr int MONT_W = 28;
constexpr uint32_t MONT_MASK = (1u << MONT_W) - 1;
constexpr int MONT_TPI = 4;
constexpr int MONT_L = 19;
constexpr int MONT_N = MONT_TPI * MONT_L;
constexpr int MONT_TPI_BIG = 8;
constexpr int MONT_L3072 = 14, MONT_L4096 = 19;
constexpr int MONT_NMAX = MONT_TPI_BIG * MONT_L4096;

constexpr int DPP_QUAD_BCAST0 = 0x00;
constexpr int DPP_QUAD_SHR1 = 0x90;
constexpr int DPP_QUAD_SWAP1 = 0xB1;
constexpr int DPP_QUAD_SWAP2 = 0x4E;
constexpr int DPP_ROW_SHL1 = 0x101;

__device__ __forceinline__ uint32_t dpp_quad_bcast0(uint32_t v) {
  return (uint32_t)__builtin_amdgcn_update_dpp(0, (int)v, DPP_QUAD_BCAST0, 0xF, 0xF, true);
}
__device__ __forceinline__ uint32_t dpp_quad_shr1(uint32_t v) {
  return (uint32_t)__builtin_amdgcn_update_dpp(0, (int)v, DPP_QUAD_SHR1, 0xF, 0xF, false);
}
__device__ __forceinline__ uint32_t dpp_row_shl1(uint32_t v) {
  return (uint32_t)__builtin_amdgcn_update_dpp(0, (int)v, DPP_ROW_SHL1, 0xF, 0xF, true);
}
constexpr int DPP_ROW_SHR1 = 0x111;
constexpr int DPP_ROW_SHR4 = 0x114;
__device__ __forceinline__ uint32_t dpp_row_shr1(uint32_t v) {
  return (uint32_t)__builtin_amdgcn_update_dpp(0, (int)v, DPP_ROW_SHR1, 0xF, 0xF, true);
}
__device__ __forceinline__ uint32_t dpp_row_shr4(uint32_t v) {
  return (uint32_t)__builtin_amdgcn_update_dpp(0, (int)v, DPP_ROW_SHR4, 0xF, 0xF, true);
}
__device__ __forceinline__ uint32_t quad_or(uint32_t v) {
  v |= (uint32_t)__builtin_amdgcn_update_dpp(0, (int)v, DPP_QUAD_SWAP1, 0xF, 0xF, false);
  v |= (uint32_t)__builtin_amdgcn_update_dpp(0, (int)v, DPP_QUAD_SWAP2, 0xF, 0xF, false);
  return v;
}

template <int TPI>
__device__ __forceinline__ uint32_t grp_bcast0(uint32_t v, int glane) {
  const uint32_t q = dpp_quad_bcast0(v);
  if constexpr (TPI == 4) return q;
  else { const uint32_t u = dpp_row_shr4(q); return (glane & 4) ? u : q; }
}
template <int TPI>
__device__ __forceinline__ uint32_t grp_shr1(uint32_t v) {
  if constexpr (TPI == 4) return dpp_quad_shr1(v);
  else return dpp_row_shr1(v);
}
template <int TPI>
__device__ __forceinline__ uint32_t grp_or(uint32_t v) {
  v = quad_or(v);
  if constexpr (TPI == 8) v |= (uint32_t)__shfl_xor((int)v, 4);
  return v;
}

__device__ __forceinline__ uint64_t mad64(uint32_t a, uint32_t b, uint64_t c) {
  return (uint64_t)a * (uint64_t)b + c;
}

template <int L, int TPI, bool SQR, int O>
__device__ __forceinline__ void mont_block_ring(uint64_t (&Q)[2 * L], const uint32_t* ap, const uint32_t (&b)[L],
                                                const uint32_t (&n)[L], uint32_t n0inv, int qlane, uint32_t mask_v) {
  constexpr int M = 2 * L;
#pragma unroll
  for (int r = 0; r < L; ++r) {
    const uint32_t ai = ap[r];
    const uint32_t ai2 = ai << 1;
    uint64_t in = 0;
    if (r > 0) in = dpp_row_shl1((uint32_t)Q[(O + r - 1) % M]) & mask_v;
#pragma unroll
    for (int k = SQR ? r : 0; k < L; ++k) {
      const uint32_t av = (SQR && k > r) ? ai2 : ai;
      if (k == L - 1 && r > 0) Q[(O + r + k) % M] = mad64(av, b[k], in);
      else Q[(O + r + k) % M] = mad64(av, b[k], Q[(O + r + k) % M]);
    }
    const uint32_t m = grp_bcast0<TPI>((uint32_t)Q[(O + r) % M] * n0inv, qlane) & mask_v;
#pragma unroll
    for (int k = 0; k < L; ++k) Q[(O + r + k) % M] = mad64(m, n[k], Q[(O + r + k) % M]);
    Q[(O + r + 1) % M] += Q[(O + r) % M] >> MONT_W;
  }
  Q[(O + M - 1) % M] = dpp_row_shl1((uint32_t)Q[(O + L - 1) % M]) & mask_v;
}

template <int L, int TPI = MONT_TPI, bool SQR = false>
__device__ __forceinline__ void mont_mul(uint32_t (&out)[L], const uint32_t* a_lds,
                                         const uint32_t (&b)[L], const uint32_t (&n)[L],
                                         uint32_t n0inv, int qlane) {
  constexpr bool NORM = 2 * TPI * L > 255;
  static_assert(TPI % 2 == 0, "the ring window runs two blocks per loop iteration");
  uint32_t mask_v;
  asm("v_mov_b32 %0, 0xfffffff" : "=v"(mask_v));
  uint64_t Q[NORM ? 2 * L - 1 : 2 * L];
#pragma unroll
  for (int k = 0; k < L + (NORM ? 1 : 0); ++k) Q[k] = 0;

  if constexpr (!NORM) {
#pragma unroll 1
    for (int blk = 0; blk < TPI; blk += 2) {
      mont_block_ring<L, TPI, SQR, 0>(Q, a_lds + blk * L, b, n, n0inv, qlane, mask_v);
      mont_block_ring<L, TPI, SQR, L>(Q, a_lds + (blk + 1) * L, b, n, n0inv, qlane, mask_v);
    }
  } else {
#pragma unroll 1
    for (int blk = 0; blk < TPI; ++blk) {
      const uint32_t* ap = a_lds + blk * L;
#pragma unroll
      for (int r = 0; r < L; ++r) {
        const uint32_t ai = ap[r];
        const uint32_t ai2 = ai << 1;
#pragma unroll
        for (int k = SQR ? r : 0; k < L; ++k) {
          const uint32_t av = (SQR && k > r) ? ai2 : ai;
          if (k == L - 1 && r > 0) Q[r + k] = mad64(av, b[k], (r == 1) ? Q[r + k] : 0);
          else Q[r + k] = mad64(av, b[k], Q[r + k]);
        }
        const uint32_t m = grp_bcast0<TPI>((uint32_t)Q[r] * n0inv, qlane) & mask_v;
#pragma unroll
        for (int k = 0; k < L; ++k) Q[r + k] = mad64(m, n[k], Q[r + k]);
        Q[r + 1] += Q[r] >> MONT_W;
      }
#pragma unroll
      for (int k = 0; k < L; ++k) {
        const uint64_t nx = dpp_row_shl1((uint32_t)Q[k]) & mask_v;
        Q[k] = (k < L - 1) ? Q[L + k] + nx : nx;
      }
#pragma unroll
      for (int k = 0; k < L; ++k) {
        const uint64_t c = Q[k] >> MONT_W;
        Q[k] &= MONT_MASK;
        if (k < L - 1) Q[k + 1] += c; else Q[L] = c;
      }
    }
  }

  uint64_t c = 0;
#pragma unroll
  for (int k = 0; k < L; ++k) {
    uint64_t v = Q[k] + c;
    out[k] = (uint32_t)v & MONT_MASK;
    c = v >> MONT_W;
  }
  if (NORM) c += Q[L];
  uint32_t clo = grp_shr1<TPI>((uint32_t)c), chi = grp_shr1<TPI>((uint32_t)(c >> 32));
  uint64_t cin = (qlane == 0) ? 0 : (((uint64_t)chi << 32) | clo);
  uint64_t v0 = (uint64_t)out[0] + cin;
  out[0] = (uint32_t)v0 & MONT_MASK;
  uint32_t v1 = out[1] + (uint32_t)(v0 >> MONT_W);
  out[1] = v1 & MONT_MASK;
  out[2] += v1 >> MONT_W;
}

template <int L, int TPI = MONT_TPI>
__device__ __forceinline__ void canonicalize(uint32_t (&x)[L], int qlane) {
  uint32_t cout = 0;
#pragma unroll
  for (int step = 0; step < TPI; ++step) {
    uint32_t c = grp_shr1<TPI>(cout);
    if (qlane == 0) c = 0;
#pragma unroll
    for (int k = 0; k < L; ++k) {
      uint32_t v = x[k] + c;
      x[k] = v & MONT_MASK;
      c = v >> MONT_W;
    }
    cout = c;
  }
}

template <int L, int TPI = MONT_TPI>
__device__ __forceinline__ void reduce_once(uint32_t (&y)[L], const uint32_t (&n)[L], int qlane) {
  uint32_t ge = 1;
#pragma unroll
  for (int k = 0; k < L; ++k) ge = (y[k] > n[k]) ? 1u : ((y[k] < n[k]) ? 0u : ge);
  if (!__any(ge != 0 && qlane == TPI - 1)) return;
  uint32_t d[L];
#pragma unroll
  for (int k = 0; k < L; ++k) d[k] = y[k] - n[k];
  int32_t cout = 0, top = 0;
#pragma unroll
  for (int step = 0; step < TPI; ++step) {
    int32_t c = (int32_t)grp_shr1<TPI>((uint32_t)cout);
    if (qlane == 0) c = 0;
#pragma unroll
    for (int k = 0; k < L; ++k) {
      const int32_t v = (int32_t)d[k] + c;
      d[k] = (uint32_t)v & MONT_MASK;
      c = v >> MONT_W;
    }
    cout = c;
    top += c;
  }
  uint32_t keep = (top == 0) ? 1u : 0u;
  if constexpr (TPI == 4) keep = (uint32_t)__builtin_amdgcn_update_dpp(0, (int)keep, 0xFF, 0xF, 0xF, true);
  else keep = (uint32_t)__shfl((int)keep, (int)((threadIdx.x & 63u) | (uint32_t)(TPI - 1)));
  if (keep) {
#pragma unroll
    for (int k = 0; k < L; ++k) y[k] = d[k];
  }
}

}
```

Before: 151.9 million verifies/s.

## Switch RSA-2048 Montgomery modexp to 29-bit limbs with wide-value fallback kernel

Adds a 29-bit-radix Montgomery form for RSA-2048 (18 limbs per lane × 4 lanes = 72 limbs instead of the 28-bit layout), with host-side precomputed n, R^2 and n0inv at the new radix. Fewer limbs per lane mean fewer multiply-accumulates per Montgomery product. Signatures whose value exceeds the 29-bit capacity are flagged during parsing and handled by a second launch of the old 28-bit kernel that early-exits when no such records exist. The output is repacked into 28-bit limbs for the EM check. The cost is an extra kernel launch, a per-record flag read, and tighter column headroom in the 64-bit accumulators.

```diff
diff --git a/bftkv_amd/csrc/capi.hip b/bftkv_amd/csrc/capi.hip
--- a/bftkv_amd/csrc/capi.hip
+++ b/bftkv_amd/csrc/capi.hip
@@ -66,7 +66,8 @@
 struct KeyEntry {
   uint64_t key_id = 0, entity_id = 0;
   uint8_t algo = 0, flags = 0;
-  uint32_t bits = 0, e = 0, n0 = 0, qbits = 0;
+  uint32_t bits = 0, e = 0, n0 = 0, qbits = 0, n0_29 = 0;
+  std::vector<uint32_t> nl29, r2_29;
   std::vector<uint32_t> nl, r2, r2w, qw, dtab, qpow, qconst;
   std::string material;
   bool cert_only = false;
@@ -123,6 +124,7 @@
   uint32_t n_ring_entities = 0;
   std::map<std::string, bool> cert_valid;
   DevBuf k_r2w;
+  DevBuf k_n29, k_r2_29, k_n0_29;
   DevBuf k_id, k_entity, k_algo, k_flags, k_bits, k_e, k_n, k_r2, k_n0, k_q, k_qbits, k_dsatab, k_dsaslot, k_sorted_id, k_sorted_slot;
   DevBuf dsa_comb;
   uint32_t dsa_wbits = 8, dsa_wbits_pinned = 0;
@@ -525,9 +527,17 @@
     if (wide8)
       hipLaunchKernelGGL((k_rsa_modexp<10, MONT_TPI_BIG>), qg8, dim3(MODEXP_BLOCK), 0, s, d_ss, c->recs.as<SigRec>(), c->pk_list.as<uint32_t>(),
                          cnt_p, start, c->kt, c->r.as<uint32_t>(), c->xr.as<uint32_t>(), (uint64_t*)(cnt_p + 16));
-    else
-    hipLaunchKernelGGL((k_rsa_modexp<MONT_L, MONT_TPI>), qg, dim3(MODEXP_BLOCK), c->modexp_lds_pad, s, d_ss, c->recs.as<SigRec>(), c->pk_list.as<uint32_t>(),
-                       cnt_p, start, c->kt, c->r.as<uint32_t>(), c->xr.as<uint32_t>(), (uint64_t*)(cnt_p + 16));
+    else {
+#if BFTKV_RSA_FORM == 29
+      hipLaunchKernelGGL((k_rsa_modexp<RSA29_L, MONT_TPI, RSA29_W>), qg, dim3(MODEXP_BLOCK), c->modexp_lds_pad, s, d_ss, c->recs.as<SigRec>(), c->pk_list.as<uint32_t>(),
+                         cnt_p, start, c->kt, c->r.as<uint32_t>(), c->xr.as<uint32_t>(), (uint64_t*)(cnt_p + 16), (const uint32_t*)(cnt_p + 5));
+      hipLaunchKernelGGL((k_rsa_modexp<MONT_L, MONT_TPI, MONT_W, true>), qg, dim3(MODEXP_BLOCK), c->modexp_lds_pad, s, d_ss, c->recs.as<SigRec>(), c->pk_list.as<uint32_t>(),
+                         cnt_p, start, c->kt, c->r.as<uint32_t>(), c->xr.as<uint32_t>(), (uint64_t*)nullptr, (const uint32_t*)(cnt_p + 5));
+#else
+      hipLaunchKernelGGL((k_rsa_modexp<MONT_L, MONT_TPI>), qg, dim3(MODEXP_BLOCK), c->modexp_lds_pad, s, d_ss, c->recs.as<SigRec>(), c->pk_list.as<uint32_t>(),
+                         cnt_p, start, c->kt, c->r.as<uint32_t>(), c->xr.as<uint32_t>(), (uint64_t*)(cnt_p + 16));
+#endif
+    }
     if (c->have_rsa3072)
       hipLaunchKernelGGL((k_rsa_modexp<MONT_L3072, MONT_TPI_BIG>), qg8, dim3(MODEXP_BLOCK), 0, s, d_ss, c->recs.as<SigRec>(), c->pk_list3072.as<uint32_t>(),
                          cnt_p + 2, start + 2, c->kt, c->r3072.as<uint32_t>(), c->xr.as<uint32_t>(), (uint64_t*)nullptr);
@@ -651,7 +661,7 @@
   if (cert_only) e.flags |= KEYF_CERT_ONLY;
   e.bits = (uint32_t)hostbn::bit_length(k.n, k.n_len);
   e.e = 0; e.n0 = 0; e.qbits = 0;
-  e.r2w.clear();
+  e.r2w.clear(); e.nl29.clear(); e.r2_29.clear(); e.n0_29 = 0;
   e.nl.assign(MONT_NMAX, 0); e.r2.assign(MONT_NMAX, 0); e.qw.assign(8, 0); e.dtab.assign(2 * DSA_N_BIG, 0); e.qpow.clear(); e.qconst.clear();
   if (k.pk_algo == PK_RSA || k.pk_algo == PK_RSA_SIGN_ONLY) {
     if (hostbn::bit_length(k.e, k.e_len) > 32) return fail(c, BFTKV_E_UNSUPPORTED, "RSA public exponent wider than 32 bits");
@@ -664,6 +674,8 @@
       uint32_t n0b = 0;
       e.r2w.assign(80, 0);
       (void)hostbn::mont_setup(k.n, k.n_len, 80, nl80.data(), e.r2w.data(), &n0b);
+      e.nl29.assign(RSA29_N, 0); e.r2_29.assign(RSA29_N, 0);
+      (void)hostbn::mont_setup(k.n, k.n_len, RSA29_N, e.nl29.data(), e.r2_29.data(), &e.n0_29, RSA29_W);
     }
   } else if (k.pk_algo == PK_DSA) {
     e.qbits = (uint32_t)hostbn::bit_length(k.e, k.e_len);
@@ -881,8 +893,13 @@
   if (c->root) return fail(c, BFTKV_E_STATE, "a forked context cannot change the key table (use its root)");
   KtWrite kw(c);
   std::vector<uint64_t> key_id, entity_ids;
-  std::vector<uint32_t> entity, bits, e32, nl, r2, r2w, n0, qw, qbits, dtab;
+  std::vector<uint32_t> entity, bits, e32, nl, r2, r2w, n0, qw, qbits, dtab, nl29, r2_29, n0_29;
   std::vector<uint8_t> algo, flags;
+  auto add29 = [&](const KeyEntry& e) {
+    nl29.insert(nl29.end(), e.nl29.begin(), e.nl29.end()); nl29.resize(key_id.size() * RSA29_N, 0);
+    r2_29.insert(r2_29.end(), e.r2_29.begin(), e.r2_29.end()); r2_29.resize(key_id.size() * RSA29_N, 0);
+    n0_29.push_back(e.n0_29);
+  };
   std::vector<const KeyEntry*> rows;
   auto add = [&](const KeyEntry& e, bool own_entity) {
     uint32_t ent = 0;
@@ -895,6 +912,7 @@
     bits.push_back(e.bits); e32.push_back(e.e); n0.push_back(e.n0); qbits.push_back(e.qbits);
     nl.insert(nl.end(), e.nl.begin(), e.nl.end()); r2.insert(r2.end(), e.r2.begin(), e.r2.end());
     r2w.insert(r2w.end(), e.r2w.begin(), e.r2w.end()); r2w.resize(key_id.size() * 80, 0);
+    add29(e);
     qw.insert(qw.end(), e.qw.begin(), e.qw.end()); dtab.insert(dtab.end(), e.dtab.begin(), e.dtab.end());
     rows.push_back(&e);
     return ent;
@@ -911,6 +929,7 @@
       bits.push_back(e.bits); e32.push_back(e.e); n0.push_back(e.n0); qbits.push_back(e.qbits);
       nl.insert(nl.end(), e.nl.begin(), e.nl.end()); r2.insert(r2.end(), e.r2.begin(), e.r2.end());
       r2w.insert(r2w.end(), e.r2w.begin(), e.r2w.end()); r2w.resize(key_id.size() * 80, 0);
+      add29(e);
       qw.insert(qw.end(), e.qw.begin(), e.qw.end()); dtab.insert(dtab.end(), e.dtab.begin(), e.dtab.end());
       rows.push_back(&e);
     }
@@ -930,9 +949,11 @@
   if ((rc = upload(c, c->k_id, key_id)) || (rc = upload(c, c->k_entity, entity)) || (rc = upload(c, c->k_algo, algo)) ||
       (rc = upload(c, c->k_flags, flags)) || (rc = upload(c, c->k_bits, bits)) || (rc = upload(c, c->k_e, e32)) ||
       (rc = upload(c, c->k_n, nl)) || (rc = upload(c, c->k_r2, r2)) || (rc = upload(c, c->k_n0, n0)) ||
-      (rc = upload(c, c->k_q, qw)) || (rc = upload(c, c->k_qbits, qbits)) || (rc = upload(c, c->k_dsatab, dtab)) || (rc = upload(c, c->k_r2w, r2w)))
+      (rc = upload(c, c->k_q, qw)) || (rc = upload(c, c->k_qbits, qbits)) || (rc = upload(c, c->k_dsatab, dtab)) || (rc = upload(c, c->k_r2w, r2w)) ||
+      (rc = upload(c, c->k_n29, nl29)) || (rc = upload(c, c->k_r2_29, r2_29)) || (rc = upload(c, c->k_n0_29, n0_29)))
     return rc;
   c->kt.r2_limbs80 = c->k_r2w.as<uint32_t>();
+  c->kt.n_limbs29 = c->k_n29.as<uint32_t>(); c->kt.r2_limbs29 = c->k_r2_29.as<uint32_t>(); c->kt.n0inv29 = c->k_n0_29.as<uint32_t>();
   c->n_keys = (uint32_t)key_id.size();
   c->kt.n_keys = c->n_keys;
   c->kt.n_limbs = c->k_n.as<uint32_t>();
@@ -1085,7 +1106,7 @@
   (void)hipStreamSynchronize(c->stream);
   (void)hipStreamSynchronize(c->stream_h);
   (void)hipStreamSynchronize(c->stream_d);
-  for (DevBuf* b : {&c->k_id, &c->k_entity, &c->k_algo, &c->k_flags, &c->k_bits, &c->k_e, &c->k_n, &c->k_r2, &c->k_n0, &c->k_q, &c->k_qbits, &c->k_dsatab, &c->k_dsaslot, &c->dsa_comb, &c->k_sorted_id, &c->k_sorted_slot, &c->k_r2w,
+  for (DevBuf* b : {&c->k_id, &c->k_entity, &c->k_algo, &c->k_flags, &c->k_bits, &c->k_e, &c->k_n, &c->k_r2, &c->k_n0, &c->k_q, &c->k_qbits, &c->k_dsatab, &c->k_dsaslot, &c->dsa_comb, &c->k_sorted_id, &c->k_sorted_slot, &c->k_r2w, &c->k_n29, &c->k_r2_29, &c->k_n0_29,
                     &c->chunk_arena, &c->chunk_ctr, &c->counts, &c->base, &c->total, &c->item_flags, &c->walk_scratch, &c->cert_ent, &c->sig_class, &c->mid, &c->mid64, &c->hash_mask, &c->recs, &c->digests, &c->r, &c->xr,
                     &c->pk_list, &c->pk_list3072, &c->pk_list4096, &c->r3072, &c->r4096, &c->pk_count, &c->dsa_list, &c->dsa_u, &c->dsa_idx, &c->ids_tmp, &c->o_err, &c->o_nver, &c->o_verdict, &c->o_fenced, &c->in_tbs, &c->in_tbs_off,
                     &c->in_ss, &c->in_ss_off, &c->in_prefix, &c->in_prefix_off, &c->in_shared, &c->in_shared_off, &c->in_seg, &c->st_tmp, &c->item_tmp, &c->bits_tmp, &c->plan_cut, &c->txt_mid32, &c->txt_mid64, &c->txt_tail, &c->txt_len})
diff --git a/bftkv_amd/csrc/device_types.h b/bftkv_amd/csrc/device_types.h
--- a/bftkv_amd/csrc/device_types.h
+++ b/bftkv_amd/csrc/device_types.h
@@ -59,6 +59,9 @@
   const uint32_t* r2_limbs;
   const uint32_t* r2_limbs80;
   const uint32_t* n0inv;
+  const uint32_t* n_limbs29;
+  const uint32_t* r2_limbs29;
+  const uint32_t* n0inv29;
   const uint32_t* q_words;
   const uint32_t* q_bits;
   const uint32_t* dsa_tab;
diff --git a/bftkv_amd/csrc/host_bignum.h b/bftkv_amd/csrc/host_bignum.h
--- a/bftkv_amd/csrc/host_bignum.h
+++ b/bftkv_amd/csrc/host_bignum.h
@@ -51,31 +51,32 @@
   if (cmp(a, m, n) >= 0) sub(a, m, n);
 }
 
-inline void to_limbs28(const uint32_t* w, int nwords, uint32_t* limbs, int nlimbs) {
+inline void to_limbs(const uint32_t* w, int nwords, uint32_t* limbs, int nlimbs, int W) {
   for (int j = 0; j < nlimbs; ++j) {
-    uint32_t bit = 28u * j, wi = bit >> 5, sh = bit & 31;
+    uint32_t bit = (uint32_t)W * j, wi = bit >> 5, sh = bit & 31;
     uint64_t v = 0;
     if ((int)wi < nwords) v = w[wi];
     if ((int)wi + 1 < nwords) v |= (uint64_t)w[wi + 1] << 32;
-    limbs[j] = (uint32_t)(v >> sh) & MASK28;
+    limbs[j] = (uint32_t)(v >> sh) & ((1u << W) - 1);
   }
 }
+inline void to_limbs28(const uint32_t* w, int nwords, uint32_t* limbs, int nlimbs) { to_limbs(w, nwords, limbs, nlimbs, W28); }
 
 inline bool mont_setup_by_doubling(const uint8_t* n_be, uint32_t n_len, int nlimbs, uint32_t* n_limbs, uint32_t* r2_limbs,
-                                   uint32_t* n0inv) {
-  const int nwords = (28 * nlimbs + 31) / 32 + 1;
+                                   uint32_t* n0inv, int W = W28) {
+  const int nwords = (W * nlimbs + 31) / 32 + 1;
   std::vector<uint32_t> n(nwords), r(nwords);
   from_be(n_be, n_len, n.data(), nwords);
   if ((n[0] & 1) == 0) return false;
   r.assign(nwords, 0);
   r[0] = 1;
   if (cmp(r.data(), n.data(), nwords) >= 0) { r[0] = 0; }
-  for (int i = 0; i < 2 * 28 * nlimbs; ++i) dbl_mod(r.data(), n.data(), nwords);
-  to_limbs28(n.data(), nwords, n_limbs, nlimbs);
-  to_limbs28(r.data(), nwords, r2_limbs, nlimbs);
+  for (int i = 0; i < 2 * W * nlimbs; ++i) dbl_mod(r.data(), n.data(), nwords);
+  to_limbs(n.data(), nwords, n_limbs, nlimbs, W);
+  to_limbs(r.data(), nwords, r2_limbs, nlimbs, W);
   uint32_t n0 = n[0], inv = n0;
   for (int i = 0; i < 5; ++i) inv *= 2u - n0 * inv;
-  *n0inv = (0u - inv) & MASK28;
+  *n0inv = (0u - inv) & ((1u << W) - 1);
   return true;
 }
 
@@ -119,22 +120,23 @@
   memcpy(out, t.data(), sizeof(uint64_t) * (size_t)k);
 }
 
-inline bool mont_setup(const uint8_t* n_be, uint32_t n_len, int nlimbs, uint32_t* n_limbs, uint32_t* r2_limbs, uint32_t* n0inv) {
-  const int nwords = (28 * nlimbs + 31) / 32 + 1;
+inline bool mont_setup(const uint8_t* n_be, uint32_t n_len, int nlimbs, uint32_t* n_limbs, uint32_t* r2_limbs, uint32_t* n0inv,
+                       int W = W28) {
+  const int nwords = (W * nlimbs + 31) / 32 + 1;
   std::vector<uint32_t> n(nwords);
   from_be(n_be, n_len, n.data(), nwords);
   if ((n[0] & 1) == 0) return false;
-  to_limbs28(n.data(), nwords, n_limbs, nlimbs);
+  to_limbs(n.data(), nwords, n_limbs, nlimbs, W);
   uint32_t n0 = n[0], inv = n0;
   for (int i = 0; i < 5; ++i) inv *= 2u - n0 * inv;
-  *n0inv = (0u - inv) & MASK28;
+  *n0inv = (0u - inv) & ((1u << W) - 1);
   int top = nwords - 1;
   while (top > 0 && n[top] == 0) --top;
   int bits = 32 * top + 32;
   while (!((n[top] >> ((bits - 1) & 31)) & 1u)) --bits;
   const int k = (bits + 64) / 64;
   if (bits == 1) { for (int j = 0; j < nlimbs; ++j) r2_limbs[j] = 0; return true; }
-  if (bits > 28 * nlimbs - 2) return mont_setup_by_doubling(n_be, n_len, nlimbs, n_limbs, r2_limbs, n0inv);
+  if (bits > W * nlimbs - 2) return mont_setup_by_doubling(n_be, n_len, nlimbs, n_limbs, r2_limbs, n0inv, W);
   std::vector<uint64_t> m(k, 0), acc(k, 0), one(k, 0);
   for (int i = 0; i < nwords && i < 2 * k; ++i) m[i >> 1] |= (uint64_t)n[i] << (32 * (i & 1));
   uint64_t m0inv = m[0];
@@ -143,7 +145,7 @@
   acc[(bits - 1) >> 6] = 1ull << ((bits - 1) & 63);
   for (int i = bits - 1; i < 64 * k; ++i) dbl_mod64(acc.data(), m.data(), k);
   dbl_mod64(acc.data(), m.data(), k);
-  const uint32_t e = 2u * 28u * (uint32_t)nlimbs;
+  const uint32_t e = 2u * (uint32_t)W * (uint32_t)nlimbs;
   int hb = 31;
   while (!((e >> hb) & 1u)) --hb;
   for (int b = hb - 1; b >= 0; --b) {
@@ -154,7 +156,7 @@
   montmul64(acc.data(), one.data(), m.data(), m0inv, k, acc.data());
   std::vector<uint32_t> r(nwords, 0);
   for (int i = 0; i < nwords && i < 2 * k; ++i) r[i] = (uint32_t)(acc[i >> 1] >> (32 * (i & 1)));
-  to_limbs28(r.data(), nwords, r2_limbs, nlimbs);
+  to_limbs(r.data(), nwords, r2_limbs, nlimbs, W);
   return true;
 }
 
diff --git a/bftkv_amd/csrc/kernels.hip b/bftkv_amd/csrc/kernels.hip
--- a/bftkv_amd/csrc/kernels.hip
+++ b/bftkv_amd/csrc/kernels.hip
@@ -166,6 +166,9 @@
 }
 
 constexpr uint8_t SIGF_LONG_VALUE = 1, SIGF_V3 = 2, SIGF_MORE_CANDIDATES = 4, SIGF_TEXT = 8;
+constexpr uint8_t SIGF_WIDE_VALUE = 16;
+constexpr int RSA29_W = 29, RSA29_L = 18, RSA29_N = RSA29_L * MONT_TPI;
+constexpr uint32_t RSA29_CAP_BYTES = RSA29_N * RSA29_W / 8;
 template <class B = const uint8_t*>
 __host__ __device__ __forceinline__ bool parse_sig_body_v3(B body, uint32_t blen, SigRec& rec, uint64_t& issuer) {
   if (blen < 1 || body[0] < 2 || body[0] > 3) return false;
@@ -654,6 +657,7 @@
           else {
             rec.after_tag = AFTER_TAG_PUBKEY;
             rec.flags |= (vbytes > kbytes) ? SIGF_LONG_VALUE : 0;
+            if (cls_sz == 0 && vbytes > RSA29_CAP_BYTES) { rec.flags |= SIGF_WIDE_VALUE; pk_count[5] = 1u; }
             q_kind = cls_sz == 0 ? 0 : (int)cls_sz + 1;
           }
         } else if (rec.pk_algo == PK_DSA) {
@@ -962,14 +966,14 @@
   return (t.pre_len >> (8 * (5 - j))) & 0xFF;
 }
 
-template <typename F>
-__device__ __forceinline__ uint32_t limb28(F byte_from_lsb, int j) {
-  uint32_t bit = 28u * (uint32_t)j;
+template <int W = MONT_W, typename F>
+__device__ __forceinline__ uint32_t limb_of(F byte_from_lsb, int j) {
+  uint32_t bit = (uint32_t)W * (uint32_t)j;
   uint32_t b0 = bit >> 3, sh = bit & 7;
   uint64_t v = 0;
 #pragma unroll
   for (int t = 0; t < 5; ++t) v |= (uint64_t)byte_from_lsb(b0 + t) << (8 * t);
-  return (uint32_t)(v >> sh) & MONT_MASK;
+  return (uint32_t)(v >> sh) & ((1u << W) - 1);
 }
 
 template <bool OTHERS>
@@ -1132,6 +1136,10 @@
 #define BFTKV_MODEXP_BLOCK 256
 #endif
 constexpr int MODEXP_BLOCK = BFTKV_MODEXP_BLOCK;
+#ifndef BFTKV_RSA_FORM
+#define BFTKV_RSA_FORM 29
+#endif
+static_assert(BFTKV_RSA_FORM == 28 || BFTKV_RSA_FORM == 29, "BFTKV_RSA_FORM: 28 or 29");
 
 enum : int { OP_TO_MONT = 0, OP_SQR = 1, OP_MULX = 2, OP_MULP = 3, OP_MUL1 = 4 };
 
@@ -1140,19 +1148,22 @@
 static_assert(EM_LOW_LIMBS * MONT_W == EM_LOW_BYTES * 8, "the EM split must fall on a limb boundary");
 constexpr uint32_t EM_HEAD_BAD = 0xFFFFFFFFu;
 
+template <int W = MONT_W>
 __device__ __forceinline__ uint32_t em_head_limb(uint32_t gi, uint32_t kbytes) {
-  const int32_t top = 8 * ((int32_t)kbytes - 2), lo = (int32_t)gi * MONT_W;
+  const int32_t top = 8 * ((int32_t)kbytes - 2), lo = (int32_t)gi * W;
   if (top < lo) return 0u;
-  if (top >= lo + MONT_W - 1) return MONT_MASK;
+  if (top >= lo + W - 1) return (1u << W) - 1u;
   return (1u << (top - lo + 1)) - 1u;
 }
 
-template <int L, int TPI>
+template <int L, int TPI, int W = MONT_W, bool WIDE_ONLY = false>
 __global__ void __launch_bounds__(MODEXP_BLOCK, 3) k_rsa_modexp(const uint8_t* __restrict__ sig_blob, const SigRec* __restrict__ recs,
                                                           const uint32_t* __restrict__ pk_list, const uint32_t* __restrict__ pk_count_ptr,
                                                           const uint32_t* __restrict__ pk_start_ptr,
                                                           KeyTableDev kt, uint32_t* __restrict__ r_low,
-                                                          uint32_t* __restrict__ xr_scratch, uint64_t* __restrict__ clk) {
+                                                          uint32_t* __restrict__ xr_scratch, uint64_t* __restrict__ clk,
+                                                          const uint32_t* __restrict__ wide_word = nullptr) {
+  static_assert(W == MONT_W || (W == 29 && L == 18 && TPI == 4 && !WIDE_ONLY), "the only form at another radix is 18 x 4 at 2^29");
   constexpr int NL = TPI * L;
   constexpr int GROUPS = MODEXP_BLOCK / TPI;
   const bool stamp = clk && blockIdx.x == 0 && threadIdx.x == 0;
@@ -1162,10 +1173,16 @@
   __shared__ uint32_t x_sh[GROUPS * NL];
   const uint32_t count = *pk_count_ptr, start = *pk_start_ptr;
   if (start + blockIdx.x * GROUPS >= count) return;
+  if constexpr (WIDE_ONLY) { if (*wide_word == 0u) return; }
   const uint32_t quad = threadIdx.x / TPI;
   const int qlane = threadIdx.x % TPI;
   const uint32_t gq = start + blockIdx.x * GROUPS + quad;
-  const bool active = gq < count;
+  bool active = gq < count;
+  if constexpr (W != MONT_W || WIDE_ONLY) {
+    const bool wide = active && (recs[pk_list[gq]].flags & SIGF_WIDE_VALUE) != 0;
+    active = active && (wide == WIDE_ONLY);
+    if (WIDE_ONLY && !__any(active)) return;
+  }
   const uint32_t pi = active ? gq : (count - 1);
   const uint32_t ri = pk_list[pi];
   const SigRec rec = recs[ri];
@@ -1175,9 +1192,10 @@
   uint32_t* x_lds = x_sh + quad * NL + qlane * L;
 
   uint32_t n[L], b[L], y[L];
-  const uint32_t* np = kt.n_limbs + (uint64_t)key * MONT_NMAX + qlane * L;
-  const uint32_t* rp = (L == 10 && TPI == 8) ? kt.r2_limbs80 + (uint64_t)key * 80 + qlane * L
-                                              : kt.r2_limbs + (uint64_t)key * MONT_NMAX + qlane * L;
+  const uint32_t* np = W == 29 ? kt.n_limbs29 + (uint64_t)key * NL + qlane * L : kt.n_limbs + (uint64_t)key * MONT_NMAX + qlane * L;
+  const uint32_t* rp = W == 29                 ? kt.r2_limbs29 + (uint64_t)key * NL + qlane * L
+                       : (L == 10 && TPI == 8) ? kt.r2_limbs80 + (uint64_t)key * 80 + qlane * L
+                                               : kt.r2_limbs + (uint64_t)key * MONT_NMAX + qlane * L;
   uint32_t* xrp = xr_scratch + (uint64_t)pi * NL + qlane * L;
 #pragma unroll
   for (int k = 0; k < L; ++k) n[k] = np[k];
@@ -1186,9 +1204,9 @@
     const uint8_t* mp = sig_blob + rec.body_off + rec.mpi_off[0];
     auto sig_b = [&](uint32_t i) -> uint32_t { return i < nb ? mp[nb - 1 - i] : 0u; };
 #pragma unroll
-    for (int k = 0; k < L; ++k) x_lds[k] = limb28(sig_b, qlane * L + k);
-  }
-  const uint32_t n0inv = kt.n0inv[key];
+    for (int k = 0; k < L; ++k) x_lds[k] = limb_of<W>(sig_b, qlane * L + k);
+  }
+  const uint32_t n0inv = W == 29 ? kt.n0inv29[key] : kt.n0inv[key];
   const uint32_t e = kt.rsa_e[key];
   const uint32_t kbytes = (kt.mod_bits[key] + 7) >> 3;
   const uint32_t cls = (e << 1) | (((e & 1u) && e > 1u && !(rec.flags & 1u)) ? 1u : 0u);
@@ -1224,8 +1242,8 @@
         }
       }
       __builtin_amdgcn_fence(__ATOMIC_ACQ_REL, "wavefront");
-      if (kind == OP_SQR) mont_mul<L, TPI, true>(y, a_rd, b, n, n0inv, qlane);
-      else mont_mul<L, TPI, false>(y, a_rd, b, n, n0inv, qlane);
+      if (kind == OP_SQR) mont_mul<L, TPI, true, W>(y, a_rd, b, n, n0inv, qlane);
+      else mont_mul<L, TPI, false, W>(y, a_rd, b, n, n0inv, qlane);
       __builtin_amdgcn_fence(__ATOMIC_ACQ_REL, "wavefront");
       if (kind == OP_TO_MONT && (e_u & (e_u - 1u)) != 0 && !(sc_u && __builtin_popcount(e_u) == 2)) {
 #pragma unroll
@@ -1236,27 +1254,47 @@
       --bitpos;
       kind = (bitpos >= 0) ? OP_SQR : OP_MUL1;
     }
-    canonicalize<L, TPI>(y, qlane);
+    canonicalize<L, TPI, W>(y, qlane);
     if (e_u == 0) {
 #pragma unroll
       for (int k = 0; k < L; ++k) y[k] = (qlane == 0 && k == 0) ? 1u : 0u;
     }
     uint32_t head = 0;
-#pragma unroll
-    for (int k = 0; k < L; ++k) {
-      const uint32_t gi = (uint32_t)qlane * L + k;
-      if (gi >= (uint32_t)EM_LOW_LIMBS) head |= y[k] ^ em_head_limb(gi, kbytes);
+    if constexpr (W == MONT_W) {
+#pragma unroll
+      for (int k = 0; k < L; ++k) {
+        const uint32_t gi = (uint32_t)qlane * L + k;
+        if (gi >= (uint32_t)EM_LOW_LIMBS) head |= y[k] ^ em_head_limb(gi, kbytes);
+      }
+    } else {
+#pragma unroll
+      for (int k = 0; k < L; ++k) {
+        const int32_t lo = ((int32_t)qlane * L + k) * W, cut = 8 * EM_LOW_BYTES;
+        if (lo + W > cut) {
+          const uint32_t d = y[k] ^ em_head_limb<W>((uint32_t)qlane * L + k, kbytes);
+          head |= (lo < cut) ? d >> (cut - lo) : d;
+        }
+      }
     }
     head = grp_or<TPI>(head);
-    if (head != 0 && qlane == 0) y[0] = EM_HEAD_BAD;
+    if (W == MONT_W && head != 0 && qlane == 0) y[0] = EM_HEAD_BAD;
 #pragma unroll
     for (int k = 0; k < L; ++k) a_lds[k] = y[k];
     __builtin_amdgcn_fence(__ATOMIC_ACQ_REL, "wavefront");
     if (live && active && qlane < 4) {
       uint32_t* out = r_low + (uint64_t)pi * EM_LOW_LIMBS + qlane * (EM_LOW_LIMBS / 4);
-      const uint32_t* src = a_rd + qlane * (EM_LOW_LIMBS / 4);
-#pragma unroll
-      for (int k = 0; k < EM_LOW_LIMBS / 4; ++k) out[k] = src[k];
+      if constexpr (W == MONT_W) {
+        const uint32_t* src = a_rd + qlane * (EM_LOW_LIMBS / 4);
+#pragma unroll
+        for (int k = 0; k < EM_LOW_LIMBS / 4; ++k) out[k] = src[k];
+      } else {
+#pragma unroll
+        for (int k = 0; k < EM_LOW_LIMBS / 4; ++k) {
+          const uint32_t bit = (uint32_t)MONT_W * ((uint32_t)qlane * (EM_LOW_LIMBS / 4) + k), i = bit / W, sh = bit % W;
+          const uint32_t v = ((a_rd[i] >> sh) | (a_rd[i + 1] << (W - sh))) & MONT_MASK;
+          out[k] = (head != 0 && qlane == 0 && k == 0) ? EM_HEAD_BAD : v;
+        }
+      }
     }
     __builtin_amdgcn_fence(__ATOMIC_ACQ_REL, "wavefront");
     todo &= ~__builtin_amdgcn_ballot_w64(live);
@@ -1859,7 +1897,7 @@
   uint32_t num = i / MONT_N, j = i % MONT_N;
   const uint8_t* p = src + (uint64_t)num * nbytes;
   auto bf = [&](uint32_t k) -> uint32_t { return k < nbytes ? p[nbytes - 1 - k] : 0u; };
-  dst[i] = limb28(bf, (int)j);
+  dst[i] = limb_of(bf, (int)j);
 }
 __global__ void k_limbs_to_bytes(const uint32_t* __restrict__ src, uint32_t nbytes, uint32_t n_nums, uint8_t* __restrict__ dst) {
   uint32_t i = blockIdx.x * blockDim.x + threadIdx.x;
diff --git a/bftkv_amd/csrc/mont28.h b/bftkv_amd/csrc/mont28.h
--- a/bftkv_amd/csrc/mont28.h
+++ b/bftkv_amd/csrc/mont28.h
@@ -64,7 +64,7 @@
   return (uint64_t)a * (uint64_t)b + c;
 }
 
-template <int L, int TPI, bool SQR, int O>
+template <int L, int TPI, bool SQR, int O, int W = MONT_W>
 __device__ __forceinline__ void mont_block_ring(uint64_t (&Q)[2 * L], const uint32_t* ap, const uint32_t (&b)[L],
                                                 const uint32_t (&n)[L], uint32_t n0inv, int qlane, uint32_t mask_v) {
   constexpr int M = 2 * L;
@@ -83,19 +83,22 @@
     const uint32_t m = grp_bcast0<TPI>((uint32_t)Q[(O + r) % M] * n0inv, qlane) & mask_v;
 #pragma unroll
     for (int k = 0; k < L; ++k) Q[(O + r + k) % M] = mad64(m, n[k], Q[(O + r + k) % M]);
-    Q[(O + r + 1) % M] += Q[(O + r) % M] >> MONT_W;
+    Q[(O + r + 1) % M] += Q[(O + r) % M] >> W;
   }
   Q[(O + M - 1) % M] = dpp_row_shl1((uint32_t)Q[(O + L - 1) % M]) & mask_v;
 }
 
-template <int L, int TPI = MONT_TPI, bool SQR = false>
+template <int L, int TPI = MONT_TPI, bool SQR = false, int W = MONT_W>
 __device__ __forceinline__ void mont_mul(uint32_t (&out)[L], const uint32_t* a_lds,
                                          const uint32_t (&b)[L], const uint32_t (&n)[L],
                                          uint32_t n0inv, int qlane) {
   constexpr bool NORM = 2 * TPI * L > 255;
   static_assert(TPI % 2 == 0, "the ring window runs two blocks per loop iteration");
+  static_assert(W == 28 || (W == 29 && !NORM && L <= 18), "a 29-bit limb fits the column only in a ring form of at most 18 rows per block");
+  constexpr uint32_t MASK = (1u << W) - 1;
   uint32_t mask_v;
-  asm("v_mov_b32 %0, 0xfffffff" : "=v"(mask_v));
+  if constexpr (W == 28) asm("v_mov_b32 %0, 0xfffffff" : "=v"(mask_v));
+  else asm("v_mov_b32 %0, 0x1fffffff" : "=v"(mask_v));
   uint64_t Q[NORM ? 2 * L - 1 : 2 * L];
 #pragma unroll
   for (int k = 0; k < L + (NORM ? 1 : 0); ++k) Q[k] = 0;
@@ -103,8 +106,8 @@
   if constexpr (!NORM) {
 #pragma unroll 1
     for (int blk = 0; blk < TPI; blk += 2) {
-      mont_block_ring<L, TPI, SQR, 0>(Q, a_lds + blk * L, b, n, n0inv, qlane, mask_v);
-      mont_block_ring<L, TPI, SQR, L>(Q, a_lds + (blk + 1) * L, b, n, n0inv, qlane, mask_v);
+      mont_block_ring<L, TPI, SQR, 0, W>(Q, a_lds + blk * L, b, n, n0inv, qlane, mask_v);
+      mont_block_ring<L, TPI, SQR, L, W>(Q, a_lds + (blk + 1) * L, b, n, n0inv, qlane, mask_v);
     }
   } else {
 #pragma unroll 1
@@ -123,7 +126,7 @@
         const uint32_t m = grp_bcast0<TPI>((uint32_t)Q[r] * n0inv, qlane) & mask_v;
 #pragma unroll
         for (int k = 0; k < L; ++k) Q[r + k] = mad64(m, n[k], Q[r + k]);
-        Q[r + 1] += Q[r] >> MONT_W;
+        Q[r + 1] += Q[r] >> W;
       }
 #pragma unroll
       for (int k = 0; k < L; ++k) {
@@ -132,8 +135,8 @@
       }
 #pragma unroll
       for (int k = 0; k < L; ++k) {
-        const uint64_t c = Q[k] >> MONT_W;
-        Q[k] &= MONT_MASK;
+        const uint64_t c = Q[k] >> W;
+        Q[k] &= MASK;
         if (k < L - 1) Q[k + 1] += c; else Q[L] = c;
       }
     }
@@ -143,20 +146,20 @@
 #pragma unroll
   for (int k = 0; k < L; ++k) {
     uint64_t v = Q[k] + c;
-    out[k] = (uint32_t)v & MONT_MASK;
-    c = v >> MONT_W;
+    out[k] = (uint32_t)v & MASK;
+    c = v >> W;
   }
   if (NORM) c += Q[L];
   uint32_t clo = grp_shr1<TPI>((uint32_t)c), chi = grp_shr1<TPI>((uint32_t)(c >> 32));
   uint64_t cin = (qlane == 0) ? 0 : (((uint64_t)chi << 32) | clo);
   uint64_t v0 = (uint64_t)out[0] + cin;
-  out[0] = (uint32_t)v0 & MONT_MASK;
-  uint32_t v1 = out[1] + (uint32_t)(v0 >> MONT_W);
-  out[1] = v1 & MONT_MASK;
-  out[2] += v1 >> MONT_W;
-}
-
-template <int L, int TPI = MONT_TPI>
+  out[0] = (uint32_t)v0 & MASK;
+  uint32_t v1 = out[1] + (uint32_t)(v0 >> W);
+  out[1] = v1 & MASK;
+  out[2] += v1 >> W;
+}
+
+template <int L, int TPI = MONT_TPI, int W = MONT_W>
 __device__ __forceinline__ void canonicalize(uint32_t (&x)[L], int qlane) {
   uint32_t cout = 0;
 #pragma unroll
@@ -166,14 +169,14 @@
 #pragma unroll
     for (int k = 0; k < L; ++k) {
       uint32_t v = x[k] + c;
-      x[k] = v & MONT_MASK;
-      c = v >> MONT_W;
+      x[k] = v & ((1u << W) - 1);
+      c = v >> W;
     }
     cout = c;
   }
 }
 
-template <int L, int TPI = MONT_TPI>
+template <int L, int TPI = MONT_TPI, int W = MONT_W>
 __device__ __forceinline__ void reduce_once(uint32_t (&y)[L], const uint32_t (&n)[L], int qlane) {
   uint32_t ge = 1;
 #pragma unroll
@@ -190,8 +193,8 @@
 #pragma unroll
     for (int k = 0; k < L; ++k) {
       const int32_t v = (int32_t)d[k] + c;
-      d[k] = (uint32_t)v & MONT_MASK;
-      c = v >> MONT_W;
+      d[k] = (uint32_t)v & ((1u << W) - 1);
+      c = v >> W;
     }
     cout = c;
     top += c;
```

After: 161.3 million verifies/s, median of 6. +6.2%, better.
